# marcomistretta/incremental_multimodal_medical_learning_II

Measured on AMD Instinct MI355X. Metric: contrastive train-step images/sec at global batch 1024; 1/2/4/8-GPU scaling, higher is better.
Workload: dtype bf16x3

## Files before the change

### include/cxrk.h

```cpp
#ifndef CXRK_H
#define CXRK_H

#include <stddef.h>
#include <hip/hip_runtime_api.h>

#ifdef __cplusplus
extern "C" {
#endif

size_t cxrk_gemm_splitk_ws_bytes(int M, int N, int splitk);
int cxrk_gemm_wgrad_splitk(int M, int N, int K, int planes);
int cxrk_gemm_wide_tile(int M, int N, long K, int splitk, int kind);
int cxrk_gemm_f32(int transA, int transB, int M, int N, int K, const float* A, long lda, const float* B, long ldb,
                  float* C, long ldc, const float* bias, const float* R, long ldr, const float* aux, long ldaux,
                  int auxmode, float* C2, long ldc2, int act, float alpha, int accumulate, int splitk, float* ws,
                  size_t ws_bytes, hipStream_t stream);

int cxrk_gemm_pl(int transA, int transB, int M, int N, int K, const void* A, long lda, long aplane, const void* B, long ldb,
                 long bplane, float* C, void* Cp, long ldc, long cplane, const float* bias, const float* R, const void* Rp,
                 long ldr, long rplane, const float* aux, long ldaux, int auxmode, const unsigned char* maskin, long ldmaskin,
                 unsigned char* maskout, long ldmaskout, float* C2, long ldc2, int act, float alpha, int accumulate, int splitk,
                 float* colsum, int colsum_accumulate, float* ws, size_t ws_bytes, hipStream_t stream);
size_t cxrk_gemm_pl_colsum_ws_bytes(int M, int N);
int cxrk_split_planes(const float* x, long n, void* out, long plane, hipStream_t stream);
int cxrk_merge_planes(const void* x, long plane, long n, float* out, hipStream_t stream);

size_t cxrk_colsum_ws_bytes(long rows, int cols);
int cxrk_colsum(const float* X, long ldx, long rows, int cols, float* out, float alpha, int accumulate, float* ws,
                size_t ws_bytes, hipStream_t stream);
int cxrk_colsum_pl(const void* X, long ldx, long plane, long rows, int cols, float* out, float alpha, int accumulate, float* ws,
                   size_t ws_bytes, hipStream_t stream);
int cxrk_colvar(const void* X, long ldx, long plane, long rows, int cols, const float* mean, float* out, float alpha, float* ws,
                size_t ws_bytes, hipStream_t stream);

int cxrk_bn_fold(const float* w, const float* gamma, const float* beta, const float* rmean, const float* rvar,
                 float eps, int Ko, int taps, int C, int Cpad, float* w_scaled, float* scale, float* shift,
                 float* rstd, hipStream_t stream);
int cxrk_bn_fold_pl(const float* w, const float* gamma, const float* beta, const float* rmean, const float* rvar,
                    float eps, int Ko, int taps, int C, int Cpad, void* w_scaled, long wplane, float* scale, float* shift,
                    float* rstd, hipStream_t stream);
int cxrk_conv_bn_act_fwd(const float* x, const float* w_scaled, const float* shift, const float* residual, float* y,
                         int N, int H, int W, int C, int Ko, int R, int S, int stride, int pad, int relu,
                         hipStream_t stream);
int cxrk_conv_bn_act_fwd_pl(const void* x, long xplane, const void* w_scaled, long wplane, int in_planes, const float* shift,
                            const void* residual, long rplane, void* y, long yplane, unsigned char* maskout, int N, int H,
                            int W, int C, int Ko, int R, int S, int stride, int pad, int relu, hipStream_t stream);
size_t cxrk_conv_bwd_data_colsum_ws_bytes(int N, int H, int W, int C, int stride);
int cxrk_conv_bn_act_bwd_data(const float* dy, const float* w_scaled, const float* residual, const float* relu_src,
                              float* dx, int N, int H, int W, int C, int Ko, int R, int S, int stride, int pad,
                              float* sums, float* ws, size_t ws_bytes, hipStream_t stream);
int cxrk_conv_bn_act_bwd_data_pl(const void* dy, long dyplane, const void* w_scaled, long wplane, const void* residual,
                                 long rplane, const unsigned char* maskin, void* dx, long dxplane, int N, int H, int W, int C,
                                 int Ko, int R, int S, int stride, int pad, float* sums, float* ws, size_t ws_bytes,
                                 hipStream_t stream);
int cxrk_conv_bn_act_bwd_data_pl_s2res(const void* dy, long dyplane, const void* w_scaled, long wplane, const void* residual_s2,
                                 long rplane, const unsigned char* maskin, void* dx, long dxplane, int N, int H, int W, int C,
                                 int Ko, int R, int S, int stride, int pad, float* sums, float* ws, size_t ws_bytes,
                                 hipStream_t stream);
size_t cxrk_conv_wgrad_ws_bytes(int N, int H, int W, int Cpad, int Ko, int R, int S, int stride, int pad);
int cxrk_conv_bn_act_bwd_params(const float* x, const float* dy, const float* w, const float* scale, const float* rstd,
                                const float* rmean, const float* sumdy, float* dw, float* dgamma, float* dbeta,
                                int accumulate, int N, int H, int W, int C, int Cpad, int Ko, int R, int S, int stride,
                                int pad, float* ws, size_t ws_bytes, hipStream_t stream);
int cxrk_conv_bn_act_bwd_params_pl(const void* x, long xplane, const void* dy, long dyplane, const float* w, const float* scale,
                                   const float* rstd, const float* rmean, const float* sumdy, float* dw, float* dgamma,
                                   float* dbeta, int accumulate, int N, int H, int W, int C, int Ko, int R, int S, int stride,
                                   int pad, float* ws, size_t ws_bytes, hipStream_t stream);

int cxrk_nchw_to_nhwc(const float* x, float* y, int N, int C, int H, int W, int Cpad, hipStream_t stream);
int cxrk_nhwc_to_nchw(const float* x, float* y, int N, int C, int H, int W, hipStream_t stream);

int cxrk_maxpool_fwd(const float* x, float* y, unsigned char* idx, int N, int H, int W, int C, hipStream_t stream);
int cxrk_maxpool_bwd(const float* dy, const unsigned char* idx, const float* x, float* dx, int N, int H, int W, int C,
                     int relu_mask, hipStream_t stream);
int cxrk_maxpool_fwd_pl(const void* x, long xplane, void* y, long yplane, unsigned char* idx, int N, int H, int W, int C,
                        hipStream_t stream);
int cxrk_maxpool_bwd_pl(const void* dy, long dyplane, const unsigned char* idx, const void* pooled, float* dx, int N, int H,
                        int W, int C, hipStream_t stream);

int cxrk_spatial_mean_fwd(const float* x, float* y, int N, int P, int C, hipStream_t stream);
int cxrk_spatial_mean_bwd(const float* dy, float* dx, int N, int P, int C, hipStream_t stream);
int cxrk_spatial_mean_bwd_pl(const float* dy, const float* add, void* dx, long dxplane, int N, int P, int C, hipStream_t stream);

int cxrk_colstats(const void* x, long plane, long rows, int C, float* mean, float* var, float var_scale, float* ws, size_t ws_bytes,
                  hipStream_t stream);
int cxrk_bn_train_fwd_coeffs(const float* mean, const float* var, const float* gamma, const float* beta, float eps, long n, float momentum,
                             float* scale, float* shift, float* rstd, float* rmean, float* rvar, int C, hipStream_t stream);
int cxrk_bn_apply(const void* z, long zplane, const float* scale, const float* shift, const void* res, long rplane, void* y, long yplane,
                  unsigned char* mask, long rows, int C, int relu, hipStream_t stream);
size_t cxrk_coldot_ws_bytes(long rows, int C);
int cxrk_coldot(const void* a, long aplane, const void* b, long bplane, const float* bshift, long rows, int C, float* out, float* ws,
                size_t ws_bytes, hipStream_t stream);
int cxrk_bn_train_bwd_coeffs(const float* gamma, const float* mean, const float* rstd, const float* sumdy, const float* dot, long n, float* A,
                             float* B, float* Cc, float* dgamma, float* dbeta, int accumulate, int C, hipStream_t stream);
int cxrk_bn_train_dz(const void* dy, long dyplane, const void* z, long zplane, const float* A, const float* B, const float* Cc, void* dz,
                     long dzplane, long rows, int C, hipStream_t stream);

int cxrk_embed_ln_fwd(const long* ids, const float* word, const float* pos, const float* type, const float* gamma,
                      const float* beta, float eps, long T, int L, int H, void* y, long yplane, float* xhat, float* rstd,
                      hipStream_t stream);
int cxrk_residual_ln_fwd(const float* x, const float* res, const float* gamma, const float* beta, float eps, long rows,
                         int H, void* y, long yplane, float* xhat, float* rstd, hipStream_t stream);
size_t cxrk_residual_ln_bwd_ws_bytes(long rows, int H);
int cxrk_residual_ln_bwd(const float* dy, const float* xhat, const float* rstd, const float* gamma, long rows, int H,
                         const float* dx_add, void* dx, long dxplane, float* dgamma, float* dbeta, int accumulate, float* dxsum,
                         int dxsum_accumulate, float* ws, size_t ws_bytes, hipStream_t stream);
int cxrk_planes_add_rows(const void* src, long plane, long rows, int cols, float* dst, long ld, hipStream_t stream);
int cxrk_attn_fwd(const float* qkv, const long* mask, int B, int L, int nH, int dH, void* ctx, long ctxplane, float* probs,
                  hipStream_t stream);
size_t cxrk_attn_bwd_ws_bytes(int B, int L, int nH, int dH);
int cxrk_attn_bwd(const float* qkv, const float* probs, const float* dctx, int B, int L, int nH, int dH, void* dqkv,
                  long dqkvplane, float* ws, size_t ws_bytes, hipStream_t stream);
int cxrk_dropout_mask(unsigned long long seed, unsigned counter, int layer, int site, long row_offset, float p, int N, int L, int nH,
                      int C, unsigned char* keep, hipStream_t stream);
int cxrk_embed_ln_fwd_drop(const long* ids, const float* word, const float* pos, const float* type, const float* gamma,
                           const float* beta, float eps, long T, int L, int H, void* y, long yplane, float* xhat, float* rstd,
                           unsigned long long seed, unsigned counter, int layer, int site, long row_offset, float p,
                           hipStream_t stream);
int cxrk_residual_ln_fwd_drop(const float* x, const void* res, long resplane, long res_ld, const float* gamma, const float* beta,
                              float eps, long rows, int H, int rows_per_seq, void* y, long yplane, float* xhat, float* rstd,
                              unsigned long long seed, unsigned counter, int layer, int site, long row_offset, float p,
                              hipStream_t stream);
int cxrk_residual_ln_bwd_drop(const float* dy, const float* xhat, const float* rstd, const float* gamma, long rows, int H,
                              int rows_per_seq, int mode, const float* dx_add, void* dx, void* dxm, long dxplane, float* dgamma,
                              float* dbeta, int accumulate, float* dxsum, int dxsum_accumulate, float* ws, size_t ws_bytes,
                              unsigned long long seed, unsigned counter, int layer, int site, long row_offset, float p,
                              hipStream_t stream);
int cxrk_attn_fwd_drop(const float* qkv, const long* mask, int B, int L, int nH, int dH, void* ctx, long ctxplane, float* probs,
                       unsigned long long seed, unsigned counter, int layer, int site, long row_offset, float p, hipStream_t stream);
int cxrk_attn_bwd_drop(const float* qkv, const float* probs, const float* dctx, int B, int L, int nH, int dH, void* dqkv,
                       long dqkvplane, float* ws, size_t ws_bytes, unsigned long long seed, unsigned counter, int layer, int site,
                       long row_offset, float p, hipStream_t stream);
size_t cxrk_embed_bwd_ws_bytes(long T, int H);
int cxrk_embed_bwd(const long* ids, const float* dx, long T, int H, float* dword, float* ws, size_t ws_bytes, hipStream_t stream);
int cxrk_gelu_bwd(const float* dy, const float* pre, long n, float* dx, hipStream_t stream);

int cxrk_l2norm_fwd(const float* x, long rows, int D, float eps, float* xhat, long ldxhat, float* norm, hipStream_t stream);
int cxrk_l2norm_bwd(const float* dxhat, const float* xhat, long ldxhat, const float* norm, long rows, int D, float* dx,
                    hipStream_t stream);
int cxrk_infonce_row_lse(const float* S, long ld, int rows, int cols, int diag_off, float* lse, float* diag,
                         float* loss_out, float loss_scale, int loss_accumulate, hipStream_t stream);
int cxrk_infonce_grad_inplace(float* S, long ld, int rows, int cols, int diag_off, const float* lse_row,
                              const float* lse_col, hipStream_t stream);
int cxrk_multipos_row_stats(const float* S, long ld, int rows, int cols, const long long* keys_row,
                            const long long* keys_col, float* lse, float* posmean, float* npos, float* loss_out,
                            float loss_scale, int loss_accumulate, hipStream_t stream);
int cxrk_multipos_grad_inplace(float* S, long ld, int rows, int cols, const long long* keys_row,
                               const long long* keys_col, const float* n_row, const float* lse_row, const float* lse_col,
                               hipStream_t stream);
int cxrk_infonce_row_lse_scaled(const float* C, long ld, int rows, int cols, int diag_off, const float* log_scale, float* lse,
                                float* diag, float* loss_out, float loss_scale, int loss_accumulate, hipStream_t stream);
int cxrk_infonce_grad_scaled_inplace(float* C, long ld, int rows, int cols, int diag_off, const float* lse_row,
                                     const float* lse_col, const float* log_scale, float* partials, hipStream_t stream);
int cxrk_multipos_row_stats_scaled(const float* C, long ld, int rows, int cols, const long long* keys_row,
                                   const long long* keys_col, const float* log_scale, float* lse, float* posmean, float* npos,
                                   float* loss_out, float loss_scale, int loss_accumulate, hipStream_t stream);
int cxrk_multipos_grad_scaled_inplace(float* C, long ld, int rows, int cols, const long long* keys_row,
                                      const long long* keys_col, const float* n_row, const float* lse_row, const float* lse_col,
                                      const float* log_scale, float* partials, hipStream_t stream);
int cxrk_logit_scale_grad(const float* partials1, long n1, const float* partials2, long n2, const float* upstream, float scale,
                          float* dtheta, int accumulate, hipStream_t stream);
int cxrk_clamp_inplace(float* x, long n, float lo, float hi, hipStream_t stream);
int cxrk_pairwise_cosine_fwd(const float* x, const float* y, long B, int P, int D, float* cosv, float* xnorm,
                             float* ynorm, hipStream_t stream);
size_t cxrk_pairwise_cosine_bwd_ws_bytes(long B, int P, int D);
int cxrk_pairwise_cosine_bwd(const float* x, const float* y, const float* cosv, const float* dcos, const float* xnorm,
                             const float* ynorm, long B, int P, int D, float* dx, float* dy, int accumulate_dy,
                             float* ws, size_t ws_bytes, hipStream_t stream);
int cxrk_pairwise_cosine_max_fwd(const float* x, const float* y, long B, int G, int Pg, int D, float* cosv, float* xnorm,
                                 float* ynorm, float* maxv, float* meanv, int* argmax, hipStream_t stream);
int cxrk_pairwise_cosine_max_bwd(const float* x, const float* y, const float* cosv, const float* dmax, const int* argmax,
                                 const float* xnorm, const float* ynorm, long B, int G, int Pg, int D, float* dx, float* dy,
                                 int accumulate_dy, float* ws, size_t ws_bytes, hipStream_t stream);
int cxrk_patch_similarity(const float* patches, const float* text, long R, int D, float* sim, hipStream_t stream);
size_t cxrk_bce_posneg_ws_bytes(void);
int cxrk_bce_posneg_fwd_bwd(const float* cosv, const float* labels, long B, int C, int ldlab, int diff, float* logits,
                            float* dcos, float* loss, float* ws, size_t ws_bytes, hipStream_t stream);
int cxrk_eval_score(const float* cosv, long B, int C, int pred_diff, float* score, float* pred, hipStream_t stream);
int cxrk_group_mean_fwd(const float* in, int G, int n, int D, float* out, hipStream_t stream);
int cxrk_group_mean_bwd(const float* dout, int G, int n, int D, float* din, hipStream_t stream);
int cxrk_scale_mask(const float* x, const float* mask_src, const float* alpha_dev, float alpha, long n, float* out,
                    hipStream_t stream);

int cxrk_adam_fused(float* p, const float* g, float* m, float* v, long n, float lr, float beta1, float beta2,
                    float eps, float weight_decay, int step, float grad_scale, hipStream_t stream);
int cxrk_sgd(float* p, const float* g, long n, float lr, float weight_decay, float grad_scale, hipStream_t stream);
size_t cxrk_weight_reset_ws_bytes(void);
int cxrk_weight_reset(float* pnew, const float* pold, long n, float threshold, unsigned long long* counters, float* ws,
                      size_t ws_bytes, hipStream_t stream);

int cxrk_set_precision(int mode);
int cxrk_get_precision(void);
int cxrk_set_wide_mode(int mode);

const char* cxrk_version(void);

#ifdef __cplusplus
}
#endif
#endif
```

### incremental_multimodal_medical_learning_ii_amd/_lib.py

```python
from __future__ import annotations

import ctypes
import os
from ctypes import c_char_p, c_float, c_int, c_long, c_size_t, c_uint32, c_uint64, c_void_p
from typing import Dict, List, Tuple

_HERE = os.path.dirname(os.path.abspath(__file__))
LIB_PATH = os.path.join(_HERE, "libcxrk.so")

P, I, L, F, Z = c_void_p, c_int, c_long, c_float, c_size_t
DROP = [c_uint64, c_uint32, I, I, L, F]

SIGNATURES: Dict[str, Tuple[object, List[object]]] = {
    "cxrk_gemm_splitk_ws_bytes": (Z, [I, I, I]),
    "cxrk_gemm_f32": (I, [I, I, I, I, I, P, L, P, L, P, L, P, P, L, P, L, I, P, L, I, F, I, I, P, Z, P]),
    "cxrk_gemm_pl": (I, [I, I, I, I, I, P, L, L, P, L, L, P, P, L, L, P, P, P, L, L, P, L, I, P, L, P, L, P, L, I, F, I, I, P, I, P, Z, P]),
    "cxrk_gemm_pl_colsum_ws_bytes": (Z, [I, I]),
    "cxrk_split_planes": (I, [P, L, P, L, P]),
    "cxrk_merge_planes": (I, [P, L, L, P, P]),
    "cxrk_colsum_pl": (I, [P, L, L, L, I, P, F, I, P, Z, P]),
    "cxrk_colsum_ws_bytes": (Z, [L, I]),
    "cxrk_colsum": (I, [P, L, L, I, P, F, I, P, Z, P]),
    "cxrk_colvar": (I, [P, L, L, L, I, P, P, F, P, Z, P]),
    "cxrk_bn_fold": (I, [P, P, P, P, P, F, I, I, I, I, P, P, P, P, P]),
    "cxrk_conv_bn_act_fwd": (I, [P, P, P, P, P, I, I, I, I, I, I, I, I, I, I, P]),
    "cxrk_bn_fold_pl": (I, [P, P, P, P, P, F, I, I, I, I, P, L, P, P, P, P]),
    "cxrk_conv_bn_act_fwd_pl": (I, [P, L, P, L, I, P, P, L, P, L, P, I, I, I, I, I, I, I, I, I, I, P]),
    "cxrk_conv_bwd_data_colsum_ws_bytes": (Z, [I, I, I, I, I]),
    "cxrk_conv_bn_act_bwd_data": (I, [P, P, P, P, P, I, I, I, I, I, I, I, I, I, P, P, Z, P]),
    "cxrk_conv_bn_act_bwd_data_pl": (I, [P, L, P, L, P, L, P, P, L, I, I, I, I, I, I, I, I, I, P, P, Z, P]),
    "cxrk_conv_bn_act_bwd_data_pl_s2res": (I, [P, L, P, L, P, L, P, P, L, I, I, I, I, I, I, I, I, I, P, P, Z, P]),
    "cxrk_conv_wgrad_ws_bytes": (Z, [I, I, I, I, I, I, I, I, I]),
    "cxrk_conv_bn_act_bwd_params": (I, [P, P, P, P, P, P, P, P, P, P, I, I, I, I, I, I, I, I, I, I, I, P, Z, P]),
    "cxrk_conv_bn_act_bwd_params_pl": (I, [P, L, P, L, P, P, P, P, P, P, P, P, I, I, I, I, I, I, I, I, I, I, P, Z, P]),
    "cxrk_colstats": (I, [P, L, L, I, P, P, F, P, Z, P]),
    "cxrk_bn_train_fwd_coeffs": (I, [P, P, P, P, F, L, F, P, P, P, P, P, I, P]),
    "cxrk_bn_apply": (I, [P, L, P, P, P, L, P, L, P, L, I, I, P]),
    "cxrk_coldot_ws_bytes": (Z, [L, I]),
    "cxrk_coldot": (I, [P, L, P, L, P, L, I, P, P, Z, P]),
    "cxrk_bn_train_bwd_coeffs": (I, [P, P, P, P, P, L, P, P, P, P, P, I, I, P]),
    "cxrk_bn_train_dz": (I, [P, L, P, L, P, P, P, P, L, L, I, P]),
    "cxrk_nchw_to_nhwc": (I, [P, P, I, I, I, I, I, P]),
    "cxrk_nhwc_to_nchw": (I, [P, P, I, I, I, I, P]),
    "cxrk_maxpool_fwd": (I, [P, P, P, I, I, I, I, P]),
    "cxrk_maxpool_bwd": (I, [P, P, P, P, I, I, I, I, I, P]),
    "cxrk_maxpool_fwd_pl": (I, [P, L, P, L, P, I, I, I, I, P]),
    "cxrk_maxpool_bwd_pl": (I, [P, L, P, P, P, I, I, I, I, P]),
    "cxrk_spatial_mean_fwd": (I, [P, P, I, I, I, P]),
    "cxrk_spatial_mean_bwd": (I, [P, P, I, I, I, P]),
    "cxrk_spatial_mean_bwd_pl": (I, [P, P, P, L, I, I, I, P]),
    "cxrk_embed_ln_fwd": (I, [P, P, P, P, P, P, F, L, I, I, P, L, P, P, P]),
    "cxrk_residual_ln_fwd": (I, [P, P, P, P, F, L, I, P, L, P, P, P]),
    "cxrk_residual_ln_bwd_ws_bytes": (Z, [L, I]),
    "cxrk_residual_ln_bwd": (I, [P, P, P, P, L, I, P, P, L, P, P, I, P, I, P, Z, P]),
    "cxrk_planes_add_rows": (I, [P, L, L, I, P, L, P]),
    "cxrk_attn_fwd": (I, [P, P, I, I, I, I, P, L, P, P]),
    "cxrk_attn_bwd_ws_bytes": (Z, [I, I, I, I]),
    "cxrk_attn_bwd": (I, [P, P, P, I, I, I, I, P, L, P, Z, P]),
    "cxrk_dropout_mask": (I, DROP + [I, I, I, I, P, P]),
    "cxrk_embed_ln_fwd_drop": (I, [P, P, P, P, P, P, F, L, I, I, P, L, P, P] + DROP + [P]),
    "cxrk_residual_ln_fwd_drop": (I, [P, P, L, L, P, P, F, L, I, I, P, L, P, P] + DROP + [P]),
    "cxrk_residual_ln_bwd_drop": (I, [P, P, P, P, L, I, I, I, P, P, P, L, P, P, I, P, I, P, Z] + DROP + [P]),
    "cxrk_attn_fwd_drop": (I, [P, P, I, I, I, I, P, L, P] + DROP + [P]),
    "cxrk_attn_bwd_drop": (I, [P, P, P, I, I, I, I, P, L, P, Z] + DROP + [P]),
    "cxrk_embed_bwd_ws_bytes": (Z, [L, I]),
    "cxrk_embed_bwd": (I, [P, P, L, I, P, P, Z, P]),
    "cxrk_gelu_bwd": (I, [P, P, L, P, P]),
    "cxrk_l2norm_fwd": (I, [P, L, I, F, P, L, P, P]),
    "cxrk_l2norm_bwd": (I, [P, P, L, P, L, I, P, P]),
    "cxrk_infonce_row_lse": (I, [P, L, I, I, I, P, P, P, F, I, P]),
    "cxrk_infonce_grad_inplace": (I, [P, L, I, I, I, P, P, P]),
    "cxrk_multipos_row_stats": (I, [P, L, I, I, P, P, P, P, P, P, F, I, P]),
    "cxrk_multipos_grad_inplace": (I, [P, L, I, I, P, P, P, P, P, P]),
    "cxrk_infonce_row_lse_scaled": (I, [P, L, I, I, I, P, P, P, P, F, I, P]),
    "cxrk_infonce_grad_scaled_inplace": (I, [P, L, I, I, I, P, P, P, P, P]),
    "cxrk_multipos_row_stats_scaled": (I, [P, L, I, I, P, P, P, P, P, P, P, F, I, P]),
    "cxrk_multipos_grad_scaled_inplace": (I, [P, L, I, I, P, P, P, P, P, P, P, P]),
    "cxrk_logit_scale_grad": (I, [P, L, P, L, P, F, P, I, P]),
    "cxrk_clamp_inplace": (I, [P, L, F, F, P]),
    "cxrk_pairwise_cosine_fwd": (I, [P, P, L, I, I, P, P, P, P]),
    "cxrk_pairwise_cosine_bwd_ws_bytes": (Z, [L, I, I]),
    "cxrk_pairwise_cosine_bwd": (I, [P, P, P, P, P, P, L, I, I, P, P, I, P, Z, P]),
    "cxrk_pairwise_cosine_max_fwd": (I, [P, P, L, I, I, I, P, P, P, P, P, P, P]),
    "cxrk_pairwise_cosine_max_bwd": (I, [P, P, P, P, P, P, P, L, I, I, I, P, P, I, P, Z, P]),
    "cxrk_patch_similarity": (I, [P, P, L, I, P, P]),
    "cxrk_bce_posneg_ws_bytes": (Z, []),
    "cxrk_bce_posneg_fwd_bwd": (I, [P, P, L, I, I, I, P, P, P, P, Z, P]),
    "cxrk_eval_score": (I, [P, L, I, I, P, P, P]),
    "cxrk_group_mean_fwd": (I, [P, I, I, I, P, P]),
    "cxrk_group_mean_bwd": (I, [P, I, I, I, P, P]),
    "cxrk_scale_mask": (I, [P, P, P, F, L, P, P]),
    "cxrk_adam_fused": (I, [P, P, P, P, L, F, F, F, F, F, I, F, P]),
    "cxrk_sgd": (I, [P, P, L, F, F, F, P]),
    "cxrk_weight_reset_ws_bytes": (Z, []),
    "cxrk_weight_reset": (I, [P, P, L, F, P, P, Z, P]),
    "cxrk_gemm_wgrad_splitk": (I, [I, I, I, I]),
    "cxrk_gemm_wide_tile": (I, [I, I, L, I, I]),
    "cxrk_set_precision": (I, [I]),
    "cxrk_get_precision": (I, []),
    "cxrk_set_wide_mode": (I, [I]),
    "cxrk_version": (c_char_p, []),
}

_ERRORS = {-1: "bad argument / shape / alignment", -2: "workspace too small", -3: "kernel launch failed",
           -4: "unsupported shape"}


class CxrkError(RuntimeError):
    pass


_lib = None


def load() -> ctypes.CDLL:
    global _lib
    if _lib is not None:
        return _lib
    if not os.path.exists(LIB_PATH):
        raise CxrkError(f"{LIB_PATH} not found: build it with `python -c 'import __graft_entry__ as g; g.build()'` "
                        f"(hipcc --offload-arch=gfx950).  There is no CPU or PyTorch fallback for the hot path.")
    lib = ctypes.CDLL(LIB_PATH)
    for name, (res, args) in SIGNATURES.items():
        fn = getattr(lib, name)
        fn.restype = res
        fn.argtypes = args
    _lib = lib
    mode = os.environ.get("CXRK_PRECISION", "fp32")
    if mode not in PRECISIONS:
        raise CxrkError(f"CXRK_PRECISION={mode!r}: expected one of {sorted(PRECISIONS)}")
    lib.cxrk_set_precision(PRECISIONS[mode])
    return lib


PRECISIONS = {"fp32": 0, "split_bf16": 1}


def set_precision(mode: str) -> None:
    if mode not in PRECISIONS:
        raise ValueError(f"precision {mode!r}: expected one of {sorted(PRECISIONS)}")
    check(load().cxrk_set_precision(PRECISIONS[mode]), "cxrk_set_precision")


def get_precision() -> str:
    v = load().cxrk_get_precision()
    return {b: a for a, b in PRECISIONS.items()}[v]


def check(rc: int, what: str) -> None:
    if rc != 0:
        msg = _ERRORS.get(rc, "unknown error")
        if rc in (-1, -4):
            raise ValueError(f"{what}: {msg} (cxrk code {rc})")
        raise CxrkError(f"{what}: {msg} (cxrk code {rc})")
```

### incremental_multimodal_medical_learning_ii_amd/csrc/conv_fwd.hip

```cpp
#include "conv_common.h"
#include "conv_halo.h"

using namespace cxrk;

template <class FMT>
static int conv_fwd_impl(const typename FMT::T* x, long xplane, const typename FMT::T* w, long wplane, EpiParams ep, int N, int H,
                         int W, int C, int Ko, int R, int S, int stride, int pad, hipStream_t stream) {
  CXRK_CHECK_ARG(x && w && N > 0 && C % FMT::EPL == 0 && aligned16(x) && aligned16(w));
  CXRK_CHECK_ARG(stride == 1 || stride == 2);
  const ConvGeom g = make_geom(N, H, W, C, Ko, R, S, stride, pad);
  CXRK_CHECK_ARG(g.Ho > 0 && g.Wo > 0);
  const long Ml = (long)N * g.Ho * g.Wo;
  CXRK_CHECK_ARG(Ml < (1L << 31));
  const int M = (int)Ml, K = R * S * C;
  if (!tile_span_ok((long)g.Ho * g.Wo, (long)H * W * C)) return CXRK_ERR_UNSUPPORTED;
  int rc;
  const bool tapwise = (C % BK == 0) && R * S <= 32 && R <= 8;
  if (tapwise && use_wide256(M, Ko, K, 1, FMT::PLANES, WIDE_MINK_FPROP)) {
    if constexpr (FMT::PLANES) {
      DmaConvIm2colKC<256, 8>::P pa{x, g, M, K, xplane}; DmaDenseKC<256, 8>::P pb{w, (long)K, Ko, K, wplane};
      rc = launch_gemm_pw<Pw256, DmaConvIm2colKC<256, 8>, DmaDenseKC<256, 8>>(pa, pb, ep, M, Ko, K, 1, stream);
    } else return CXRK_ERR_UNSUPPORTED;
  } else if (tapwise) {
    if (FMT::PLANES && halo_applies(H, W, C, Ko, R, S, stride, pad)) {
      if constexpr (FMT::PLANES) {
        DmaDenseKC<64, 4>::P pb{w, (long)K, Ko, K, wplane};
        rc = launch_conv3x3_halo<DmaDenseKC<64, 4>, false>(x, xplane, pb, ep, M, Ko, H, W, stream);
      } else rc = CXRK_ERR_UNSUPPORTED;
    } else if (Ko <= 64) {
      if constexpr (FMT::PLANES) {
        DmaConvIm2colKC<256, 4>::P pa{x, g, M, K, xplane}; DmaDenseKC<64, 4>::P pb{w, (long)K, Ko, K, wplane};
        rc = launch_gemm_pw<Pw256x64, DmaConvIm2colKC<256, 4>, DmaDenseKC<64, 4>>(pa, pb, ep, M, Ko, K, 1, stream);
      } else {
        typename ConvIm2colKC<256, FMT>::P pa{x, g, M, K, xplane}; typename DenseKC<64, FMT>::P pb{w, (long)K, Ko, K, wplane};
        rc = launch_gemm<ConvIm2colKC<256, FMT>, DenseKC<64, FMT>, 4, 1>(pa, pb, ep, M, Ko, K, 1, stream);
      }
    } else if constexpr (FMT::PLANES) {
      DmaConvIm2colKC<128, 4>::P pa{x, g, M, K, xplane}; DmaDenseKC<128, 4>::P pb{w, (long)K, Ko, K, wplane};
      rc = launch_gemm_pw<Pw128, DmaConvIm2colKC<128, 4>, DmaDenseKC<128, 4>>(pa, pb, ep, M, Ko, K, 1, stream);
    } else {
      typename ConvIm2colKC<128, FMT>::P pa{x, g, M, K, xplane}; typename DenseKC<128, FMT>::P pb{w, (long)K, Ko, K, wplane};
      rc = launch_gemm<ConvIm2colKC<128, FMT>, DenseKC<128, FMT>, 2, 2>(pa, pb, ep, M, Ko, K, 1, stream);
    }
  } else {
    if constexpr (FMT::PLANES) return CXRK_ERR_UNSUPPORTED;
    else {
      if (Ko <= 64) {
        ConvIm2colKC<256, F32, false>::P pa{x, g, M, K, 0}; DenseKC<64>::P pb{w, (long)K, Ko, K, 0};
        rc = launch_gemm<ConvIm2colKC<256, F32, false>, DenseKC<64>, 4, 1>(pa, pb, ep, M, Ko, K, 1, stream);
      } else {
        ConvIm2colKC<128, F32, false>::P pa{x, g, M, K, 0}; DenseKC<128>::P pb{w, (long)K, Ko, K, 0};
        rc = launch_gemm<ConvIm2colKC<128, F32, false>, DenseKC<128>, 2, 2>(pa, pb, ep, M, Ko, K, 1, stream);
      }
    }
  }
  return rc < 0 ? rc : CXRK_OK;
}

extern "C" int cxrk_conv_bn_act_fwd(const float* x, const float* w_scaled, const float* shift, const float* residual,
                                    float* y, int N, int H, int W, int C, int Ko, int R, int S, int stride, int pad,
                                    int relu, hipStream_t stream) {
  CXRK_CHECK_ARG(y);
  EpiParams ep{};
  ep.C = y; ep.ldc = Ko; ep.bias = shift; ep.R = residual; ep.ldr = Ko; ep.act = relu ? 1 : 0; ep.alpha = 1.f;
  return conv_fwd_impl<F32>(x, 0, w_scaled, 0, ep, N, H, W, C, Ko, R, S, stride, pad, stream);
}

extern "C" int cxrk_conv_bn_act_fwd_pl(const void* x, long xplane, const void* w_scaled, long wplane, int in_planes,
                                       const float* shift, const void* residual, long rplane, void* y, long yplane,
                                       unsigned char* maskout, int N, int H, int W, int C, int Ko, int R, int S, int stride,
                                       int pad, int relu, hipStream_t stream) {
  CXRK_CHECK_ARG(y && (Ko % 8) == 0 && !(maskout && !relu));
  EpiParams ep{};
  ep.Cp = static_cast<unsigned short*>(y); ep.cplane = yplane; ep.ldc = Ko; ep.bias = shift;
  ep.Rp = static_cast<const unsigned short*>(residual); ep.rplane = rplane; ep.ldr = Ko; ep.act = relu ? 1 : 0; ep.alpha = 1.f;
  ep.maskout = maskout; ep.ldmaskout = Ko / 8;
  if (in_planes)
    return conv_fwd_impl<PL>(static_cast<const unsigned short*>(x), xplane, static_cast<const unsigned short*>(w_scaled), wplane, ep, N, H,
                             W, C, Ko, R, S, stride, pad, stream);
  return conv_fwd_impl<F32>(static_cast<const float*>(x), 0, static_cast<const float*>(w_scaled), 0, ep, N, H, W, C, Ko, R, S, stride,
                            pad, stream);
}
```

### incremental_multimodal_medical_learning_ii_amd/csrc/conv_misc.hip

```cpp
#include "conv_common.h"

using namespace cxrk;

namespace {
__global__ void bn_fold_kernel(const float* __restrict__ w, const float* __restrict__ gamma, const float* __restrict__ beta,
                               const float* __restrict__ rmean, const float* __restrict__ rvar, float eps, int Ko, int taps,
                               int C, int Cpad, float* __restrict__ ws, unsigned short* __restrict__ wp, long wplane,
                               float* __restrict__ scale, float* __restrict__ shift, float* __restrict__ rstd) {
  const int ko = blockIdx.x;
  const float rs = 1.0f / sqrtf(rvar[ko] + eps);
  const float sc = gamma[ko] * rs;
  if (threadIdx.x == 0) { scale[ko] = sc; shift[ko] = beta[ko] - rmean[ko] * sc; rstd[ko] = rs; }
  const int n = taps * Cpad;
  if (wp) {
    for (int i8 = threadIdx.x; i8 < n / 8; i8 += blockDim.x) {
      const int i = i8 * 8, tap = i / Cpad, c = i - tap * Cpad;
      float v[8];
#pragma unroll
      for (int q = 0; q < 8; ++q) v[q] = c + q < C ? w[((long)ko * taps + tap) * C + c + q] * sc : 0.f;
      planes_store8(wp, wplane, (long)ko * n + i, v);
    }
    return;
  }
  for (int i = threadIdx.x; i < n; i += blockDim.x) {
    const int tap = i / Cpad, c = i - tap * Cpad;
    ws[(long)ko * n + i] = c < C ? w[((long)ko * taps + tap) * C + c] * sc : 0.f;
  }
}

__global__ void nchw_to_nhwc_kernel(const float* __restrict__ x, float* __restrict__ y, int C, int H, int W, int Cpad) {
  const long nh = blockIdx.x;
  const long n = nh / H; const int hh = (int)(nh - n * H);
  for (int i = threadIdx.x; i < W * Cpad; i += blockDim.x) {
    const int wv = i / Cpad, c = i - wv * Cpad;
    y[(nh * W + wv) * Cpad + c] = c < C ? x[((n * C + c) * H + hh) * W + wv] : 0.f;
  }
}
__global__ void nhwc_to_nchw_kernel(const float* __restrict__ x, float* __restrict__ y, int C, int H, int W) {
  const long nh = blockIdx.x;
  const long n = nh / H; const int hh = (int)(nh - n * H);
  for (int i = threadIdx.x; i < W * C; i += blockDim.x) {
    const int c = i / W, wv = i - c * W;
    y[((n * C + c) * H + hh) * W + wv] = x[(nh * W + wv) * C + c];
  }
}

__global__ void maxpool_fwd_kernel(const float* __restrict__ x, float* __restrict__ y, unsigned char* __restrict__ idx,
                                   int N, int H, int W, int C, int Ho, int Wo) {
  const long t = (long)blockIdx.x * blockDim.x + threadIdx.x;
  const int C4 = C / 4;
  const long total = (long)N * Ho * Wo * C4;
  if (t >= total) return;
  const int c4 = (int)(t % C4); long p = t / C4;
  const int wo = (int)(p % Wo); p /= Wo; const int ho = (int)(p % Ho); const long n = p / Ho;
  float4 best = make_float4(-INFINITY, -INFINITY, -INFINITY, -INFINITY);
  uchar4 bi = make_uchar4(0, 0, 0, 0);
  bool first = true;
  for (int r = 0; r < 3; ++r) {
    const int hi = ho * 2 - 1 + r;
    if ((unsigned)hi >= (unsigned)H) continue;
    for (int s = 0; s < 3; ++s) {
      const int wi = wo * 2 - 1 + s;
      if ((unsigned)wi >= (unsigned)W) continue;
      const float4 v = *reinterpret_cast<const float4*>(x + ((n * H + hi) * W + wi) * C + c4 * 4);
      const unsigned char tap = (unsigned char)(r * 3 + s);
      if (first || v.x > best.x) { best.x = v.x; bi.x = tap; }
      if (first || v.y > best.y) { best.y = v.y; bi.y = tap; }
      if (first || v.z > best.z) { best.z = v.z; bi.z = tap; }
      if (first || v.w > best.w) { best.w = v.w; bi.w = tap; }
      first = false;
    }
  }
  *reinterpret_cast<float4*>(y + t * 4) = best;
  *reinterpret_cast<uchar4*>(idx + t * 4) = bi;
}

__global__ void maxpool_bwd_kernel(const float* __restrict__ dy, const unsigned char* __restrict__ idx,
                                   const float* __restrict__ x, float* __restrict__ dx, int N, int H, int W, int C, int Ho,
                                   int Wo, int relu_mask) {
  const long t = (long)blockIdx.x * blockDim.x + threadIdx.x;
  const int C4 = C / 4;
  const long total = (long)N * H * W * C4;
  if (t >= total) return;
  const int c4 = (int)(t % C4); long p = t / C4;
  const int wi = (int)(p % W); p /= W; const int hi = (int)(p % H); const long n = p / H;
  float4 g = make_float4(0.f, 0.f, 0.f, 0.f);
  for (int r = 0; r < 3; ++r) {
    const int hn = hi + 1 - r;
    if (hn < 0 || (hn & 1)) continue;
    const int ho = hn >> 1;
    if (ho >= Ho) continue;
    for (int s = 0; s < 3; ++s) {
      const int wn = wi + 1 - s;
      if (wn < 0 || (wn & 1)) continue;
      const int wo = wn >> 1;
      if (wo >= Wo) continue;
      const long o = (((n * Ho + ho) * Wo + wo) * C4 + c4) * 4;
      const uchar4 bi = *reinterpret_cast<const uchar4*>(idx + o);
      const float4 d = *reinterpret_cast<const float4*>(dy + o);
      const unsigned char tap = (unsigned char)(r * 3 + s);
      if (bi.x == tap) g.x += d.x;
      if (bi.y == tap) g.y += d.y;
      if (bi.z == tap) g.z += d.z;
      if (bi.w == tap) g.w += d.w;
    }
  }
  if (relu_mask) {
    const float4 xv = *reinterpret_cast<const float4*>(x + t * 4);
    g.x = xv.x > 0.f ? g.x : 0.f; g.y = xv.y > 0.f ? g.y : 0.f; g.z = xv.z > 0.f ? g.z : 0.f; g.w = xv.w > 0.f ? g.w : 0.f;
  }
  *reinterpret_cast<float4*>(dx + t * 4) = g;
}

__global__ void spatial_mean_fwd_kernel(const float* __restrict__ x, float* __restrict__ y, int P, int C) {
  const int n = blockIdx.x;
  for (int c = threadIdx.x; c < C; c += blockDim.x) {
    float s = 0.f;
    for (int p = 0; p < P; ++p) s += x[((long)n * P + p) * C + c];
    y[(long)n * C + c] = s / (float)P;
  }
}
__global__ void spatial_mean_bwd_kernel(const float* __restrict__ dy, float* __restrict__ dx, int P, int C) {
  const int n = blockIdx.x;
  const float inv = 1.0f / (float)P;
  for (int i = threadIdx.x; i < P * C; i += blockDim.x) dx[(long)n * P * C + i] = dy[(long)n * C + (i % C)] * inv;
}

__global__ void maxpool_fwd_pl_kernel(const unsigned short* __restrict__ x, long xplane, unsigned short* __restrict__ y, long yplane,
                                      unsigned char* __restrict__ idx, int N, int H, int W, int C, int Ho, int Wo) {
  const long t = (long)blockIdx.x * blockDim.x + threadIdx.x;
  const int C8 = C / 8;
  const long total = (long)N * Ho * Wo * C8;
  if (t >= total) return;
  const int c8 = (int)(t % C8); long p = t / C8;
  const int wo = (int)(p % Wo); p /= Wo; const int ho = (int)(p % Ho); const long n = p / Ho;
  float best[8]; unsigned char bi[8];
  bool first = true;
  for (int r = 0; r < 3; ++r) {
    const int hi = ho * 2 - 1 + r;
    if ((unsigned)hi >= (unsigned)H) continue;
    for (int s = 0; s < 3; ++s) {
      const int wi = wo * 2 - 1 + s;
      if ((unsigned)wi >= (unsigned)W) continue;
      float v[8]; planes_load8(x, xplane, ((n * H + hi) * W + wi) * C + c8 * 8, v);
      const unsigned char tap = (unsigned char)(r * 3 + s);
#pragma unroll
      for (int q = 0; q < 8; ++q) if (first || v[q] > best[q]) { best[q] = v[q]; bi[q] = tap; }
      first = false;
    }
  }
  planes_store8(y, yplane, t * 8, best);
  *reinterpret_cast<uint2*>(idx + t * 8) = make_uint2(bi[0] | (bi[1] << 8) | (bi[2] << 16) | (bi[3] << 24),
                                                      bi[4] | (bi[5] << 8) | (bi[6] << 16) | (bi[7] << 24));
}
struct PoolWin { float d[8]; unsigned tap[8]; };
__device__ __forceinline__ void pool_win_load(PoolWin& w, bool valid, const unsigned short* __restrict__ dy, long dyplane,
                                              const unsigned char* __restrict__ idx, const unsigned short* __restrict__ pooled, long o) {
  if (!valid) {
#pragma unroll
    for (int q = 0; q < 8; ++q) { w.d[q] = 0.f; w.tap[q] = 0xffu; }
    return;
  }
  const uint2 bw = *reinterpret_cast<const uint2*>(idx + o);
  const uint4 ph = *reinterpret_cast<const uint4*>(pooled + o);
  planes_load8(dy, dyplane, o, w.d);
  const unsigned pw[4] = {ph.x, ph.y, ph.z, ph.w};
#pragma unroll
  for (int q = 0; q < 8; ++q) {
    w.tap[q] = ((q < 4 ? bw.x : bw.y) >> (8 * (q & 3))) & 0xffu;
    const float pv = __builtin_bit_cast(float, (q & 1) ? (pw[q >> 1] & 0xffff0000u) : (pw[q >> 1] << 16));
    if (!(pv > 0.f)) w.tap[q] = 0xffu;
  }
}
__device__ __forceinline__ void pool_acc(float (&g)[8], const PoolWin& w, unsigned tap) {
#pragma unroll
  for (int q = 0; q < 8; ++q) if (w.tap[q] == tap) g[q] += w.d[q];
}
__device__ __forceinline__ void pool_store(float* __restrict__ dx, long e, const float (&g)[8]) {
  *reinterpret_cast<float4*>(dx + e) = make_float4(g[0], g[1], g[2], g[3]);
  *reinterpret_cast<float4*>(dx + e + 4) = make_float4(g[4], g[5], g[6], g[7]);
}
__global__ __launch_bounds__(256) void maxpool_bwd_pl_kernel(const unsigned short* __restrict__ dy, long dyplane, const unsigned char* __restrict__ idx,
                                                             const unsigned short* __restrict__ pooled, float* __restrict__ dx, int N, int H,
                                                             int W, int C, int Ho, int Wo) {
  const long t = (long)blockIdx.x * blockDim.x + threadIdx.x;
  const int C8 = C / 8, H2 = (H + 1) / 2, W2 = (W + 1) / 2;
  const long total = (long)N * H2 * W2 * C8;
  if (t >= total) return;
  const int c8 = (int)(t % C8); long p = t / C8;
  const int b = (int)(p % W2); p /= W2; const int a = (int)(p % H2); const long n = p / H2;
  PoolWin w00, w01, w10, w11;
  const bool va = a < Ho, va1 = a + 1 < Ho, vb = b < Wo, vb1 = b + 1 < Wo;
  const long o00 = (((n * Ho + a) * Wo + b) * C8 + c8) * 8;
  pool_win_load(w00, va && vb, dy, dyplane, idx, pooled, o00);
  pool_win_load(w01, va && vb1, dy, dyplane, idx, pooled, o00 + (long)C);
  pool_win_load(w10, va1 && vb, dy, dyplane, idx, pooled, o00 + (long)Wo * C);
  pool_win_load(w11, va1 && vb1, dy, dyplane, idx, pooled, o00 + (long)(Wo + 1) * C);
  const int hi = 2 * a, wi = 2 * b;
  const long e = (((n * H + hi) * W + wi) * C8 + c8) * 8;
  {
    float g[8] = {0.f, 0.f, 0.f, 0.f, 0.f, 0.f, 0.f, 0.f};
    pool_acc(g, w00, 4u);
    pool_store(dx, e, g);
  }
  if (wi + 1 < W) {
    float g[8] = {0.f, 0.f, 0.f, 0.f, 0.f, 0.f, 0.f, 0.f};
    pool_acc(g, w01, 3u); pool_acc(g, w00, 5u);
    pool_store(dx, e + C, g);
  }
  if (hi + 1 < H) {
    float g[8] = {0.f, 0.f, 0.f, 0.f, 0.f, 0.f, 0.f, 0.f};
    pool_acc(g, w10, 1u); pool_acc(g, w00, 7u);
    pool_store(dx, e + (long)W * C, g);
  }
  if (hi + 1 < H && wi + 1 < W) {
    float g[8] = {0.f, 0.f, 0.f, 0.f, 0.f, 0.f, 0.f, 0.f};
    pool_acc(g, w11, 0u); pool_acc(g, w10, 2u); pool_acc(g, w01, 6u); pool_acc(g, w00, 8u);
    pool_store(dx, e + (long)(W + 1) * C, g);
  }
}
__global__ void spatial_mean_bwd_pl_kernel(const float* __restrict__ dy, const float* __restrict__ add, unsigned short* __restrict__ dx,
                                           long dxplane, int P, int C) {
  const int n = blockIdx.x;
  const float inv = 1.0f / (float)P;
  const int C8 = C / 8;
  for (int i = threadIdx.x; i < P * C8; i += blockDim.x) {
    const int c = (i % C8) * 8;
    float v[8];
#pragma unroll
    for (int q = 0; q < 8; ++q) v[q] = dy[(long)n * C + c + q] * inv;
    const long o = ((long)n * P + i / C8) * C + c;
    if (add) {
#pragma unroll
      for (int q = 0; q < 8; ++q) v[q] += add[o + q];
    }
    planes_store8(dx, dxplane, o, v);
  }
}

}

extern "C" int cxrk_bn_fold(const float* w, const float* gamma, const float* beta, const float* rmean, const float* rvar,
                            float eps, int Ko, int taps, int C, int Cpad, float* w_scaled, float* scale, float* shift,
                            float* rstd, hipStream_t stream) {
  CXRK_CHECK_ARG(w && gamma && beta && rmean && rvar && w_scaled && scale && shift && rstd && Ko > 0 && taps > 0 && C > 0 && Cpad >= C);
  hipLaunchKernelGGL(bn_fold_kernel, dim3(Ko), dim3(256), 0, stream, w, gamma, beta, rmean, rvar, eps, Ko, taps, C, Cpad,
                     w_scaled, (unsigned short*)nullptr, 0L, scale, shift, rstd);
  CXRK_LAUNCH_CHECK();
  return CXRK_OK;
}
extern "C" int cxrk_bn_fold_pl(const float* w, const float* gamma, const float* beta, const float* rmean, const float* rvar,
                               float eps, int Ko, int taps, int C, int Cpad, void* w_scaled, long wplane, float* scale,
                               float* shift, float* rstd, hipStream_t stream) {
  CXRK_CHECK_ARG(w && gamma && beta && rmean && rvar && w_scaled && scale && shift && rstd && Ko > 0 && taps > 0 && C > 0 && Cpad >= C);
  CXRK_CHECK_ARG((Cpad % 8) == 0 && (wplane % 8) == 0 && aligned16(w_scaled));
  hipLaunchKernelGGL(bn_fold_kernel, dim3(Ko), dim3(256), 0, stream, w, gamma, beta, rmean, rvar, eps, Ko, taps, C, Cpad,
                     (float*)nullptr, static_cast<unsigned short*>(w_scaled), wplane, scale, shift, rstd);
  CXRK_LAUNCH_CHECK();
  return CXRK_OK;
}

extern "C" int cxrk_nchw_to_nhwc(const float* x, float* y, int N, int C, int H, int W, int Cpad, hipStream_t stream) {
  CXRK_CHECK_ARG(x && y && N > 0 && C > 0 && Cpad >= C);
  hipLaunchKernelGGL(nchw_to_nhwc_kernel, dim3((unsigned)((long)N * H)), dim3(256), 0, stream, x, y, C, H, W, Cpad);
  CXRK_LAUNCH_CHECK();
  return CXRK_OK;
}
extern "C" int cxrk_nhwc_to_nchw(const float* x, float* y, int N, int C, int H, int W, hipStream_t stream) {
  CXRK_CHECK_ARG(x && y && N > 0 && C > 0);
  hipLaunchKernelGGL(nhwc_to_nchw_kernel, dim3((unsigned)((long)N * H)), dim3(256), 0, stream, x, y, C, H, W);
  CXRK_LAUNCH_CHECK();
  return CXRK_OK;
}

extern "C" int cxrk_maxpool_fwd(const float* x, float* y, unsigned char* idx, int N, int H, int W, int C, hipStream_t stream) {
  CXRK_CHECK_ARG(x && y && idx && C % 4 == 0 && aligned16(x) && aligned16(y));
  const int Ho = (H + 2 - 3) / 2 + 1, Wo = (W + 2 - 3) / 2 + 1;
  const long total = (long)N * Ho * Wo * (C / 4);
  hipLaunchKernelGGL(maxpool_fwd_kernel, dim3((unsigned)((total + 255) / 256)), dim3(256), 0, stream, x, y, idx, N, H, W, C, Ho, Wo);
  CXRK_LAUNCH_CHECK();
  return CXRK_OK;
}
extern "C" int cxrk_maxpool_bwd(const float* dy, const unsigned char* idx, const float* x, float* dx, int N, int H, int W,
                                int C, int relu_mask, hipStream_t stream) {
  CXRK_CHECK_ARG(dy && idx && dx && C % 4 == 0 && (!relu_mask || x));
  const int Ho = (H + 2 - 3) / 2 + 1, Wo = (W + 2 - 3) / 2 + 1;
  const long total = (long)N * H * W * (C / 4);
  hipLaunchKernelGGL(maxpool_bwd_kernel, dim3((unsigned)((total + 255) / 256)), dim3(256), 0, stream, dy, idx, x, dx, N, H, W, C,
                     Ho, Wo, relu_mask);
  CXRK_LAUNCH_CHECK();
  return CXRK_OK;
}
extern "C" int cxrk_maxpool_fwd_pl(const void* x, long xplane, void* y, long yplane, unsigned char* idx, int N, int H, int W, int C,
                                   hipStream_t stream) {
  CXRK_CHECK_ARG(x && y && idx && C % 8 == 0 && aligned16(x) && aligned16(y) && (xplane % 8) == 0 && (yplane % 8) == 0 && (((uintptr_t)idx) & 7) == 0);
  const int Ho = (H + 2 - 3) / 2 + 1, Wo = (W + 2 - 3) / 2 + 1;
  const long total = (long)N * Ho * Wo * (C / 8);
  hipLaunchKernelGGL(maxpool_fwd_pl_kernel, dim3((unsigned)((total + 255) / 256)), dim3(256), 0, stream, static_cast<const unsigned short*>(x),
                     xplane, static_cast<unsigned short*>(y), yplane, idx, N, H, W, C, Ho, Wo);
  CXRK_LAUNCH_CHECK();
  return CXRK_OK;
}
extern "C" int cxrk_maxpool_bwd_pl(const void* dy, long dyplane, const unsigned char* idx, const void* pooled, float* dx, int N, int H,
                                   int W, int C, hipStream_t stream) {
  CXRK_CHECK_ARG(dy && idx && pooled && dx && C % 8 == 0 && aligned16(dy) && aligned16(pooled) && aligned16(dx) && (dyplane % 8) == 0);
  const int Ho = (H + 2 - 3) / 2 + 1, Wo = (W + 2 - 3) / 2 + 1;
  const long total = (long)N * ((H + 1) / 2) * ((W + 1) / 2) * (C / 8);
  hipLaunchKernelGGL(maxpool_bwd_pl_kernel, dim3((unsigned)((total + 255) / 256)), dim3(256), 0, stream, static_cast<const unsigned short*>(dy),
                     dyplane, idx, static_cast<const unsigned short*>(pooled), dx, N, H, W, C, Ho, Wo);
  CXRK_LAUNCH_CHECK();
  return CXRK_OK;
}

extern "C" int cxrk_spatial_mean_fwd(const float* x, float* y, int N, int P, int C, hipStream_t stream) {
  CXRK_CHECK_ARG(x && y && N > 0 && P > 0 && C > 0);
  hipLaunchKernelGGL(spatial_mean_fwd_kernel, dim3(N), dim3(128), 0, stream, x, y, P, C);
  CXRK_LAUNCH_CHECK();
  return CXRK_OK;
}
extern "C" int cxrk_spatial_mean_bwd(const float* dy, float* dx, int N, int P, int C, hipStream_t stream) {
  CXRK_CHECK_ARG(dy && dx && N > 0 && P > 0 && C > 0);
  hipLaunchKernelGGL(spatial_mean_bwd_kernel, dim3(N), dim3(256), 0, stream, dy, dx, P, C);
  CXRK_LAUNCH_CHECK();
  return CXRK_OK;
}
extern "C" int cxrk_spatial_mean_bwd_pl(const float* dy, const float* add, void* dx, long dxplane, int N, int P, int C, hipStream_t stream) {
  CXRK_CHECK_ARG(dy && dx && N > 0 && P > 0 && C > 0 && (C % 8) == 0 && aligned16(dx) && (dxplane % 8) == 0);
  hipLaunchKernelGGL(spatial_mean_bwd_pl_kernel, dim3(N), dim3(256), 0, stream, dy, add, static_cast<unsigned short*>(dx), dxplane, P, C);
  CXRK_LAUNCH_CHECK();
  return CXRK_OK;
}
```

### incremental_multimodal_medical_learning_ii_amd/csrc/conv_wgrad.hip

```cpp
#include "conv_common.h"

using namespace cxrk;

namespace {
__global__ __launch_bounds__(256) void wgrad_reduce_bn_kernel(const float* __restrict__ slabs, int nslab, long slab_stride,
                                                              int taps, int C, int Cpad, const float* __restrict__ w,
                                                              const float* __restrict__ scale, float* __restrict__ dw,
                                                              float* __restrict__ dotpart, int accumulate, int sg_log2) {
  __shared__ float sh[16];
  __shared__ float4 red[256];
  const int ko = blockIdx.x;
  const int n = taps * Cpad;
  const float sc = scale ? scale[ko] : 1.f;
  const int SG = 1 << sg_log2, QPB = 256 >> sg_log2;
  const int ql = threadIdx.x & (QPB - 1), grp = threadIdx.x >> (8 - sg_log2);
  const int i4 = (blockIdx.y * QPB + ql) * 4;
  float4 s = make_float4(0.f, 0.f, 0.f, 0.f);
  if (i4 < n) {
    const float* src = slabs + (long)ko * n + i4;
    int z = grp;
    for (; z + 3 * SG < nslab; z += 4 * SG) {
      const float4 t0 = *reinterpret_cast<const float4*>(src + (long)z * slab_stride);
      const float4 t1 = *reinterpret_cast<const float4*>(src + (long)(z + SG) * slab_stride);
      const float4 t2 = *reinterpret_cast<const float4*>(src + (long)(z + 2 * SG) * slab_stride);
      const float4 t3 = *reinterpret_cast<const float4*>(src + (long)(z + 3 * SG) * slab_stride);
      s.x += (t0.x + t1.x) + (t2.x + t3.x); s.y += (t0.y + t1.y) + (t2.y + t3.y);
      s.z += (t0.z + t1.z) + (t2.z + t3.z); s.w += (t0.w + t1.w) + (t2.w + t3.w);
    }
    for (; z < nslab; z += SG) {
      const float4 t = *reinterpret_cast<const float4*>(src + (long)z * slab_stride);
      s.x += t.x; s.y += t.y; s.z += t.z; s.w += t.w;
    }
  }
  if (SG > 1) {
    red[threadIdx.x] = s;
    __syncthreads();
    if (grp == 0) {
      for (int g2 = 1; g2 < SG; ++g2) { const float4 t = red[g2 * QPB + ql]; s.x += t.x; s.y += t.y; s.z += t.z; s.w += t.w; }
    }
  }
  float dot = 0.f;
  if (i4 < n && grp == 0) {
    const int tap = i4 / Cpad, c = i4 - tap * Cpad;
    const float sv[4] = {s.x, s.y, s.z, s.w};
#pragma unroll
    for (int q = 0; q < 4; ++q) {
      if (c + q < C) {
        const long o = ((long)ko * taps + tap) * C + c + q;
        if (dotpart) dot += w[o] * sv[q];
        dw[o] = accumulate ? dw[o] + sc * sv[q] : sc * sv[q];
      }
    }
  }
  if (dotpart) {
    dot = block_sum(dot, sh);
    if (threadIdx.x == 0) dotpart[(long)ko * gridDim.y + blockIdx.y] = dot;
  }
}
__global__ void bn_param_grad_kernel(const float* __restrict__ dotpart, int nparts, const float* __restrict__ rstd,
                                     const float* __restrict__ rmean, const float* __restrict__ sumdy, int Ko,
                                     float* __restrict__ dgamma, float* __restrict__ dbeta, int accumulate) {
  const int ko = blockIdx.x * blockDim.x + threadIdx.x;
  if (ko >= Ko) return;
  float dot = 0.f;
  for (int p = 0; p < nparts; ++p) dot += dotpart[(long)ko * nparts + p];
  const float g = rstd[ko] * (dot - rmean[ko] * sumdy[ko]);
  dgamma[ko] = accumulate ? dgamma[ko] + g : g;
  dbeta[ko] = accumulate ? dbeta[ko] + sumdy[ko] : sumdy[ko];
}

}

static int wgrad_splitk(int Ko, int Ncols, long Kred, bool planes) { return wgrad_splitk_policy(Ko, Ncols, (int)Kred, planes); }
static int wgrad_dot_parts(int Nc) { return ceil_div(Nc, 64); }

extern "C" size_t cxrk_conv_wgrad_ws_bytes(int N, int H, int W, int C, int Ko, int R, int S, int stride, int pad) {
  const ConvGeom g = make_geom(N, H, W, C, Ko, R, S, stride, pad);
  int sk = wgrad_splitk(Ko, R * S * C, (long)N * g.Ho * g.Wo, false);
  const int sk2 = wgrad_splitk(Ko, R * S * C, (long)N * g.Ho * g.Wo, true);
  if (sk2 > sk) sk = sk2;
  return ((size_t)sk * (size_t)Ko * (size_t)(R * S * C) + (size_t)Ko * wgrad_dot_parts(R * S * C)) * sizeof(float);
}

template <class FMT>
static int conv_bwd_params_impl(const typename FMT::T* x, long xplane, const typename FMT::T* dy, long dyplane, const float* w,
                                const float* scale, const float* rstd, const float* rmean, const float* sumdy, float* dw,
                                float* dgamma, float* dbeta, int accumulate, int N, int H, int W, int C, int Cpad, int Ko, int R,
                                int S, int stride, int pad, float* ws, size_t ws_bytes, hipStream_t stream) {
  CXRK_CHECK_ARG(x && dy && dw && N > 0 && Cpad % FMT::EPL == 0 && Ko % FMT::EPL == 0 && aligned16(x) && aligned16(dy));
  CXRK_CHECK_ARG(!(dgamma && !(w && rstd && rmean && sumdy && dbeta)));
  const ConvGeom g = make_geom(N, H, W, Cpad, Ko, R, S, stride, pad);
  const long Kl = (long)N * g.Ho * g.Wo;
  CXRK_CHECK_ARG(Kl < (1L << 31));
  const int Kred = (int)Kl, Nc = R * S * Cpad;
  if ((long)H * W * Cpad * 4 * 3 >= (1L << 31)) return CXRK_ERR_UNSUPPORTED;
  int sk = wgrad_splitk(Ko, Nc, Kl, FMT::PLANES);
  const size_t slab_floats = (size_t)sk * Ko * Nc;
  CXRK_CHECK_WS(ws, ws_bytes, (slab_floats + (size_t)Ko * wgrad_dot_parts(Nc)) * sizeof(float));
  EpiParams ep{};
  ep.C = ws; ep.ldc = Nc; ep.alpha = 1.f; ep.slab_stride = (long)Ko * Nc;
  int rc;
  const bool exact = false;
  if (use_wide256(Ko, Nc, Kred, sk, FMT::PLANES)) {
    if constexpr (FMT::PLANES) {
      DmaDenseMC<256, 8>::P pa{dy, (long)Ko, Ko, Kred, dyplane}; DmaConvIm2colMC<256, 8>::P pb{x, g, Nc, Kred, xplane};
      rc = launch_gemm_pw<Pw256, DmaDenseMC<256, 8>, DmaConvIm2colMC<256, 8>>(pa, pb, ep, Ko, Nc, Kred, sk, stream);
    } else return CXRK_ERR_UNSUPPORTED;
  } else if (Ko <= 64) {
    if constexpr (FMT::PLANES) {
      DmaDenseMC<64, 4>::P pa{dy, (long)Ko, Ko, Kred, dyplane}; DmaConvIm2colMC<256, 4>::P pb{x, g, Nc, Kred, xplane};
      rc = launch_gemm_pw<Pw64x256, DmaDenseMC<64, 4>, DmaConvIm2colMC<256, 4>>(pa, pb, ep, Ko, Nc, Kred, sk, stream);
    } else {
      typename DenseMC<64, FMT>::P pa{dy, (long)Ko, Ko, Kred, dyplane}; typename ConvIm2colMC<256, FMT>::P pb{x, g, Nc, Kred, xplane};
      rc = launch_gemm<DenseMC<64, FMT>, ConvIm2colMC<256, FMT>, 1, 4>(pa, pb, ep, Ko, Nc, Kred, sk, stream, exact);
    }
  } else if constexpr (FMT::PLANES) {
    DmaDenseMC<128, 4>::P pa{dy, (long)Ko, Ko, Kred, dyplane}; DmaConvIm2colMC<128, 4>::P pb{x, g, Nc, Kred, xplane};
    rc = launch_gemm_pw<Pw128, DmaDenseMC<128, 4>, DmaConvIm2colMC<128, 4>>(pa, pb, ep, Ko, Nc, Kred, sk, stream);
  } else {
    typename DenseMC<128, FMT>::P pa{dy, (long)Ko, Ko, Kred, dyplane}; typename ConvIm2colMC<128, FMT>::P pb{x, g, Nc, Kred, xplane};
    rc = launch_gemm<DenseMC<128, FMT>, ConvIm2colMC<128, FMT>, 2, 2>(pa, pb, ep, Ko, Nc, Kred, sk, stream, exact);
  }
  if (rc < 0) return rc;
  const int sg_log2 = rc >= 64 ? 4 : (rc >= 8 ? 2 : 0);
  const int ny = ceil_div(Nc, 4 * (256 >> sg_log2));
  float* dotpart = dgamma ? ws + slab_floats : nullptr;
  hipLaunchKernelGGL(wgrad_reduce_bn_kernel, dim3(Ko, ny), dim3(256), 0, stream, ws, rc, (long)Ko * Nc, R * S, C, Cpad, w, scale, dw,
                     dotpart, accumulate, sg_log2);
  CXRK_LAUNCH_CHECK();
  if (dgamma) {
    hipLaunchKernelGGL(bn_param_grad_kernel, dim3(ceil_div(Ko, 256)), dim3(256), 0, stream, dotpart, ny, rstd, rmean, sumdy, Ko, dgamma,
                       dbeta, accumulate);
    CXRK_LAUNCH_CHECK();
  }
  return CXRK_OK;
}

extern "C" int cxrk_conv_bn_act_bwd_params(const float* x, const float* dy, const float* w, const float* scale,
                                           const float* rstd, const float* rmean, const float* sumdy, float* dw,
                                           float* dgamma, float* dbeta, int accumulate, int N, int H, int W, int C,
                                           int Cpad, int Ko, int R, int S, int stride, int pad, float* ws, size_t ws_bytes,
                                           hipStream_t stream) {
  return conv_bwd_params_impl<F32>(x, 0, dy, 0, w, scale, rstd, rmean, sumdy, dw, dgamma, dbeta, accumulate, N, H, W, C, Cpad, Ko, R, S,
                                   stride, pad, ws, ws_bytes, stream);
}
extern "C" int cxrk_conv_bn_act_bwd_params_pl(const void* x, long xplane, const void* dy, long dyplane, const float* w,
                                              const float* scale, const float* rstd, const float* rmean, const float* sumdy,
                                              float* dw, float* dgamma, float* dbeta, int accumulate, int N, int H, int W, int C,
                                              int Ko, int R, int S, int stride, int pad, float* ws, size_t ws_bytes,
                                              hipStream_t stream) {
  return conv_bwd_params_impl<PL>(static_cast<const unsigned short*>(x), xplane, static_cast<const unsigned short*>(dy), dyplane, w, scale,
                                  rstd, rmean, sumdy, dw, dgamma, dbeta, accumulate, N, H, W, C, C, Ko, R, S, stride, pad, ws, ws_bytes,
                                  stream);
}
```

### incremental_multimodal_medical_learning_ii_amd/csrc/gemm_core.h

```cpp
#pragma once
#include "cxrk_common.h"
#include <cstdlib>

namespace cxrk {

constexpr int BK = 32;
constexpr int NTHREADS = 256;
constexpr int LPAD = 4;

struct EpiParams {
  float* C; long ldc;
  const float* bias;
  const float* R; long ldr;
  const float* aux; long ldaux;
  int auxmode;
  float* C2; long ldc2;
  int act;
  float alpha;
  long slab_stride;
  int rm_on, rm_Hs, rm_Ws, rm_H, rm_W, rm_ph, rm_pw;
  int vec;
  int nt;
  float* colsum_part;
  unsigned short* Cp; long cplane;
// ... 193 lines not shown
  constexpr int BM = WM * 64, BN = WN * 64;
  constexpr int LDA = LA::LD, LDB = LB::LD;
  constexpr int ASZ = BK * LDA, BSZ = BK * LDB;
  __shared__ __attribute__((aligned(16))) float smem[ASZ + BSZ];
  float* const As0 = smem;
  float* const Bs0 = smem + ASZ;

  int mt, nt, z;
  tile_coords(nMt, nNt, nZ, mt, nt, z);
  const int m0 = mt * BM, n0 = nt * BN;
  const int kbeg = z * kchunk;
  const int kend = min(K, kbeg + kchunk);

  const int tid = threadIdx.x;
  const int lane = tid & 63, wave = tid >> 6;
  const int wm = wave / WN, wn = wave % WN;
  const int r = lane & 31, h = lane >> 5;

  LA la; LB lb;
  la.init(pa, m0, tid);
  lb.init(pb, n0, tid);

  f32x16 acc[2][2];
#pragma unroll
  for (int i = 0; i < 2; ++i)
#pragma unroll
    for (int j = 0; j < 2; ++j)
#pragma unroll
      for (int e = 0; e < 16; ++e) acc[i][j][e] = 0.f;

  static_assert(!LA::FMT_PLANES && !LB::FMT_PLANES, "the exact-fp32 mainloop reads fp32 operands");
  float4 ra[LA::NV], rb[LB::NV];
  if (kbeg < kend) {
    la.load(kbeg, ra); lb.load(kbeg, rb);
    la.store(As0, ra); lb.store(Bs0, rb);
  }
  __syncthreads();
  if (kbeg + BK < kend) { la.load(kbeg + BK, ra); lb.load(kbeg + BK, rb); }

  for (int k0 = kbeg; k0 < kend; k0 += BK) {
    const float* Ap = As0 + wm * 64 + r + h * LDA;
    const float* Bp = Bs0 + wn * 64 + r + h * LDB;
    const bool has1 = k0 + BK < kend, has2 = k0 + 2 * BK < kend;
    float a0 = Ap[0], a1 = Ap[32], b0 = Bp[0], b1 = Bp[32];
#pragma unroll
    for (int kk = 0; kk < BK / 2; ++kk) {
      float a0n = 0.f, a1n = 0.f, b0n = 0.f, b1n = 0.f;
      if (kk + 1 < BK / 2) {
        a0n = Ap[(2 * kk + 2) * LDA]; a1n = Ap[(2 * kk + 2) * LDA + 32];
        b0n = Bp[(2 * kk + 2) * LDB]; b1n = Bp[(2 * kk + 2) * LDB + 32];
      }
      acc[0][0] = __builtin_amdgcn_mfma_f32_32x32x2f32(a0, b0, acc[0][0], 0, 0, 0);
      acc[0][1] = __builtin_amdgcn_mfma_f32_32x32x2f32(a0, b1, acc[0][1], 0, 0, 0);
      acc[1][0] = __builtin_amdgcn_mfma_f32_32x32x2f32(a1, b0, acc[1][0], 0, 0, 0);
      acc[1][1] = __builtin_amdgcn_mfma_f32_32x32x2f32(a1, b1, acc[1][1], 0, 0, 0);
      a0 = a0n; a1 = a1n; b0 = b0n; b1 = b1n;
    }
    __syncthreads();
    if (has1) { la.store(As0, ra); lb.store(Bs0, rb); }
    __syncthreads();
    if (has2) { la.load(k0 + 2 * BK, ra); lb.load(k0 + 2 * BK, rb); }
  }

  static_assert(BK * (LDA + LDB) >= 4 * 32 * 64, "operand LDS too small to stage the epilogue");
  __syncthreads();
  gemm_epilogue<WM, WN>(acc, ep, smem, M, N, m0, n0, mt, z, wave, lane);
}

template <class LA, class LB, int WM, int WN>
__global__ __launch_bounds__(NTHREADS, (WM == 2 && WN == 2) ? 3 : 2) void gemm_x3_kernel(typename LA::P pa, typename LB::P pb, EpiParams ep,
                                                              int M, int N, int K, int nMt, int nNt, int nZ, int kchunk) {
  constexpr int BM = WM * 64, BN = WN * 64;
  constexpr int PLANE_A = LA::PLANE, PLANE_B = LB::PLANE;
  static_assert(2 * (PLANE_A + PLANE_B) * 2 >= 4 * 32 * 64 * 4, "operand LDS too small to stage the epilogue");
  __shared__ __attribute__((aligned(16))) unsigned short smem16[2 * (PLANE_A + PLANE_B)];
  unsigned short* const Ahi = smem16;
  unsigned short* const Alo = Ahi + PLANE_A;
  unsigned short* const Bhi = Alo + PLANE_A;
  unsigned short* const Blo = Bhi + PLANE_B;

  int mt, nt, z;
  tile_coords(nMt, nNt, nZ, mt, nt, z);
  const int m0 = mt * BM, n0 = nt * BN;
  const int kbeg = z * kchunk;
  const int kend = min(K, kbeg + kchunk);

  const int tid = threadIdx.x;
  const int lane = tid & 63, wave = tid >> 6;
  const int wm = wave / WN, wn = wave % WN;

  LA la; LB lb;
  la.init(pa, m0, tid);
  lb.init(pb, n0, tid);

  f32x16 acc[2][2];
#pragma unroll
  for (int i = 0; i < 2; ++i)
#pragma unroll
    for (int j = 0; j < 2; ++j)
#pragma unroll
      for (int e = 0; e < 16; ++e) acc[i][j][e] = 0.f;

  typename LA::V ra[LA::NV]; typename LB::V rb[LB::NV];
  if (kbeg < kend) {
    la.load(kbeg, ra); lb.load(kbeg, rb);
    la.store2(Ahi, Alo, ra); lb.store2(Bhi, Blo, rb);
  }
  __syncthreads();
  if (kbeg + BK < kend) { la.load(kbeg + BK, ra); lb.load(kbeg + BK, rb); }

  for (int k0 = kbeg; k0 < kend; k0 += BK) {
#pragma unroll
    for (int kc = 0; kc < BK / 16; ++kc) {
      bf16x8 ah[2], al[2], bh[2], bl[2];
#pragma unroll
      for (int i = 0; i < 2; ++i) {
        if constexpr (LA::KC) {
          ah[i] = frag_kc(Ahi, wm * 64 + i * 32, kc, lane); al[i] = frag_kc(Alo, wm * 64 + i * 32, kc, lane);
        } else {
          ah[i] = frag_mc<LA::LDT>(Ahi, wm * 64 + i * 32, kc, lane); al[i] = frag_mc<LA::LDT>(Alo, wm * 64 + i * 32, kc, lane);
        }
        if constexpr (LB::KC) {
          bh[i] = frag_kc(Bhi, wn * 64 + i * 32, kc, lane); bl[i] = frag_kc(Blo, wn * 64 + i * 32, kc, lane);
        } else {
          bh[i] = frag_mc<LB::LDT>(Bhi, wn * 64 + i * 32, kc, lane); bl[i] = frag_mc<LB::LDT>(Blo, wn * 64 + i * 32, kc, lane);
        }
      }
#pragma unroll
      for (int i = 0; i < 2; ++i)
#pragma unroll
        for (int j = 0; j < 2; ++j) {
          acc[i][j] = __builtin_amdgcn_mfma_f32_32x32x16_bf16(al[i], bh[j], acc[i][j], 0, 0, 0);
          acc[i][j] = __builtin_amdgcn_mfma_f32_32x32x16_bf16(ah[i], bl[j], acc[i][j], 0, 0, 0);
          acc[i][j] = __builtin_amdgcn_mfma_f32_32x32x16_bf16(ah[i], bh[j], acc[i][j], 0, 0, 0);
        }
    }
    __syncthreads();
    if (k0 + BK < kend) { la.store2(Ahi, Alo, ra); lb.store2(Bhi, Blo, rb); }
    __syncthreads();
    if (k0 + 2 * BK < kend) { la.load(k0 + 2 * BK, ra); lb.load(k0 + 2 * BK, rb); }
  }
  __syncthreads();
  gemm_epilogue<WM, WN>(acc, ep, reinterpret_cast<float*>(smem16), M, N, m0, n0, mt, z, wave, lane);
}

inline int& gemm_precision_mode() { static int mode = 0; return mode; }

static inline int stream_output(int M, int N, int splitk) {
  static const double thr = [] { const char* e = getenv("CXRK_NT_MB"); return (e ? atof(e) : 64.0) * 1048576.0; }();
  return (double)M * N * 4.0 * (splitk > 1 ? splitk : 1) >= thr;
}

int wgrad_splitk_policy(int M, int N, int K, bool planes);

inline int& wide_mode_ref() { static int m = [] { const char* e = getenv("CXRK_WIDE"); return e ? atoi(e) : 1; }(); return m; }
inline int wide_mode() { return wide_mode_ref(); }
static inline long env_long(const char* name, long dflt) { const char* e = getenv(name); return e ? atol(e) : dflt; }
#define WIDE_MINK_PLAIN (wide_mink(0))
#define WIDE_MINK_FPROP (wide_mink(1))
#define WIDE_MINK_DGRAD (wide_mink(2))
inline long wide_mink(int kind) {
  static const long v[3] = {env_long("CXRK_MINK_PLAIN", 512), env_long("CXRK_MINK_FPROP", 512), env_long("CXRK_MINK_DGRAD", 64)};
  return v[kind];
}
static inline bool use_wide256(int M, int N, long K, int splitk, bool planes, long min_k = WIDE_MINK_PLAIN) {
  if (!planes) return false;
  const int mode = wide_mode();
  if (mode == 2) return true;
  if (2.0 * M * N * (double)K < 1073741824.0) return false;
  if (mode == 0 || M < 256 || N < 256) return false;
  const long kper = splitk > 1 ? K / splitk : K;
  if (kper < min_k) return false;
  const long tiles = (long)ceil_div(M, 256) * ceil_div(N, 256) * (splitk > 1 ? splitk : 1);
  const long rounds = (tiles + 255) / 256;
  static const long eff_pct = env_long("CXRK_WIDE_EFF", 60);
  return tiles * 100 >= rounds * 256 * eff_pct;
}

static inline bool prep_epilogue(EpiParams& e, int M, int N, int splitk) {
  auto ok16 = [](const void* p_, long ld) { return p_ == nullptr || (aligned16(p_) && (ld % 4) == 0); };
  auto ok8 = [](const void* p_, long ld) { return p_ == nullptr || (aligned16(p_) && (ld % 8) == 0); };
  e.vec = (N % 4 == 0) && ok16(e.C, e.ldc) && ((e.slab_stride % 4) == 0) && ok16(e.R, e.ldr) && ok16(e.aux, e.ldaux) &&
          ok16(e.C2, e.ldc2) && (e.bias == nullptr || aligned16(e.bias));
  e.pl = (e.Cp || e.Rp || e.maskin || e.maskout || e.auxmode == 3) ? 1 : 0;
  e.fast = e.vec && (N % 8) == 0 && ok8(e.Cp, e.ldc) && ok8(e.Rp, e.ldr) && (e.cplane % 8) == 0 && (e.rplane % 8) == 0 &&
           (!e.maskout || ((N % 64) == 0 && (e.ldmaskout % 8) == 0 && (((uintptr_t)e.maskout) & 7) == 0));
  e.kind = epi_kind(epi_flags(e));
  if (e.kind >= 0 && (EPI_KINDS[e.kind] & (EF_OUTPL | EF_AUX_MASK | EF_MASKOUT)) == 0u && (N % 64) != 0) e.kind = -1;
  if (e.rs2_on && !(e.Rp && e.Cp && e.rs2_H > 0 && e.rs2_W > 0 && (long)e.rs2_Ho * e.rs2_Wo > 0)) return false;
  if (e.pl) {
    if (!e.fast) return false;
    if ((e.C != nullptr) == (e.Cp != nullptr)) return false;
    if (e.R && e.Rp) return false;
    if (e.auxmode == 3 && !e.maskin) return false;
    if (e.maskout && e.act != 1) return false;
    if (e.Cp && splitk > 1) return false;
  }
  e.nt = stream_output(M, N, splitk);
  return true;
}

template <class LA, class LB, int WM, int WN>
static int launch_gemm(const typename LA::P& pa, const typename LB::P& pb, const EpiParams& ep, int M, int N, int K,
                       int splitk, hipStream_t stream, bool force_fp32 = false) {
  constexpr int BM = WM * 64, BN = WN * 64;
  if (M <= 0 || N <= 0 || K <= 0) return CXRK_ERR_ARG;
  const int nMt = ceil_div(M, BM), nNt = ceil_div(N, BN);
  int kchunk = K;
  if (splitk > 1) { kchunk = ceil_div(ceil_div(K, splitk), BK) * BK; splitk = ceil_div(K, kchunk); }
  else splitk = 1;
  dim3 grid((unsigned)(nMt * nNt * splitk), 1, 1);
  EpiParams e = ep;
  if (!prep_epilogue(e, M, N, splitk)) return CXRK_ERR_ARG;
  if (e.rs2_on) return CXRK_ERR_UNSUPPORTED;
  constexpr bool planes_in = LA::FMT_PLANES || LB::FMT_PLANES;
  const bool split = planes_in || (gemm_precision_mode() == 1 && !force_fp32 && 2.0 * M * N * (double)K >= 1073741824.0);
  if constexpr (planes_in) {
    static_assert(LA::FMT_PLANES && LB::FMT_PLANES, "both operands must share the storage format");
    hipLaunchKernelGGL((gemm_x3_kernel<LA, LB, WM, WN>), grid, dim3(NTHREADS), 0, stream, pa, pb, e, M, N, K, nMt, nNt, splitk, kchunk);
  } else if (split)
    hipLaunchKernelGGL((gemm_x3_kernel<LA, LB, WM, WN>), grid, dim3(NTHREADS), 0, stream, pa, pb, e, M, N, K, nMt, nNt, splitk, kchunk);
  else
    hipLaunchKernelGGL((gemm_f32_kernel<LA, LB, WM, WN>), grid, dim3(NTHREADS), 0, stream, pa, pb, e, M, N, K, nMt, nNt, splitk, kchunk);
  CXRK_LAUNCH_CHECK();
  return splitk;
}

}
#include "gemm_pw.h"
```

### incremental_multimodal_medical_learning_ii_amd/csrc/gemm_loaders.h

```cpp
#pragma once

namespace cxrk {

constexpr unsigned VOFF_OOB = 0x80000000u;

struct F32 {
  static constexpr bool PLANES = false;
  static constexpr int ESZ = 4;
  static constexpr int EPL = 4;
  static constexpr int NPL = 1;
  typedef float T;
  typedef float4 V;
};
struct PL {
  static constexpr bool PLANES = true;
  static constexpr int ESZ = 2;
  static constexpr int EPL = 8;
  static constexpr int NPL = 2;
  typedef unsigned short T;
  typedef uint4 V;
};

__device__ __forceinline__ __amdgpu_buffer_rsrc_t tile_rsrc(const void* p, bool live = true) {
  return __builtin_amdgcn_make_buffer_rsrc(const_cast<void*>(p), 0, live ? (int)0x80000000 : 0, 0x00020000);
}
__device__ __forceinline__ float4 bload4(__amdgpu_buffer_rsrc_t r, unsigned voff) {
  const auto q = __builtin_amdgcn_raw_buffer_load_b128(r, (int)voff, 0, 0);
  static_assert(sizeof(q) == 16, "raw_buffer_load_b128 must return 16 bytes");
  const f32x4 f = __builtin_bit_cast(f32x4, q);
  return make_float4(f[0], f[1], f[2], f[3]);
}
__device__ __forceinline__ uint4 bloadu4(__amdgpu_buffer_rsrc_t r, unsigned voff) {
  const auto q = __builtin_amdgcn_raw_buffer_load_b128(r, (int)voff, 0, 0);
  typedef unsigned u32x4 __attribute__((ext_vector_type(4)));
  const u32x4 u = __builtin_bit_cast(u32x4, q);
  return make_uint4(u[0], u[1], u[2], u[3]);
}
template <class FMT> __device__ __forceinline__ typename FMT::V bloadv(__amdgpu_buffer_rsrc_t r, unsigned voff);
template <> __device__ __forceinline__ float4 bloadv<F32>(__amdgpu_buffer_rsrc_t r, unsigned voff) { return bload4(r, voff); }
template <> __device__ __forceinline__ uint4 bloadv<PL>(__amdgpu_buffer_rsrc_t r, unsigned voff) { return bloadu4(r, voff); }

__device__ __forceinline__ unsigned masked_off(unsigned off, unsigned inv, int t) {
  return (__builtin_amdgcn_ubfe(inv, (unsigned)t, 1u) << 31) | off;
}

__device__ __forceinline__ unsigned low_bits(int k) { return k >= 32 ? 0xffffffffu : ((1u << k) - 1u); }
__device__ __forceinline__ unsigned outside_bits(int lo, int hi, int n) {
  lo = min(max(lo, 0), n); hi = min(max(hi, 0), n);
  return low_bits(lo) | (low_bits(n) & ~low_bits(hi));
}
__device__ __forceinline__ unsigned tap_mask(unsigned badr, unsigned bads, int R, int S) {
  const unsigned full = low_bits(S);
  unsigned m = 0;
#pragma unroll
  for (int r = 0; r < 8; ++r)
    if (r < R) m |= (((badr >> r) & 1u) ? full : bads) << (r * S);
  return m;
}

template <int NV, int LD, int RP>
__device__ __forceinline__ void stage_kc(float* S, int r0, int k4, const float4 (&v)[NV]) {
#pragma unroll
  for (int j = 0; j < NV; ++j) {
    float* d = S + (k4 * 4) * LD + r0 + j * RP;
    d[0] = v[j].x; d[LD] = v[j].y; d[2 * LD] = v[j].z; d[3 * LD] = v[j].w;
  }
}
template <int NV, int RP>
__device__ __forceinline__ void stage2_kc(unsigned short* hi, unsigned short* lo, int r0, int kq, const float4 (&v)[NV]) {
#pragma unroll
  for (int j = 0; j < NV; ++j) store2_kc(hi, lo, r0 + j * RP, kq * 4, v[j]);
}
template <int NV, int RP>
__device__ __forceinline__ void stage2_kc(unsigned short* hi, unsigned short* lo, int r0, int kq, const uint4 (&v)[NV]) {
#pragma unroll
  for (int j = 0; j < NV / 2; ++j) {
    *reinterpret_cast<uint4*>(hi + (r0 + j * RP) * LDH + kq * 8) = v[j];
    *reinterpret_cast<uint4*>(lo + (r0 + j * RP) * LDH + kq * 8) = v[NV / 2 + j];
  }
}
template <int NV, int LD, int RPP>
__device__ __forceinline__ void stage_mc(float* S, int kr0, int c4, const float4 (&v)[NV]) {
#pragma unroll
  for (int j = 0; j < NV; ++j) *reinterpret_cast<float4*>(S + (kr0 + j * RPP) * LD + c4 * 4) = v[j];
}
template <int NV, int LDT, int RPP>
__device__ __forceinline__ void stage2_mc(unsigned short* hi, unsigned short* lo, int kr0, int cq, const float4 (&v)[NV]) {
#pragma unroll
  for (int j = 0; j < NV; ++j) store2_mc<LDT>(hi, lo, cq * 4, kr0 + j * RPP, v[j]);
}
template <int NV, int LDT, int RPP>
__device__ __forceinline__ void stage2_mc(unsigned short* hi, unsigned short* lo, int kr0, int cq, const uint4 (&v)[NV]) {
#pragma unroll
  for (int j = 0; j < NV / 2; ++j) {
    *reinterpret_cast<uint4*>(hi + (kr0 + j * RPP) * LDT + cq * 8) = v[j];
    *reinterpret_cast<uint4*>(lo + (kr0 + j * RPP) * LDT + cq * 8) = v[NV / 2 + j];
  }
}

template <int TILE, class FMT, int NT>
struct KCGeom {
  static constexpr bool KC = true;
  static constexpr bool FMT_PLANES = FMT::PLANES;
  static constexpr int PLANE = TILE * LDH;
  static constexpr int KQ = BK / FMT::EPL;
  static constexpr int RP = NT / KQ;
  static constexpr int NVR = TILE / RP;
  static constexpr int NV = NVR * FMT::NPL;
  static constexpr int LD = TILE + 1;
  static_assert(NVR >= 1 && NVR * RP == TILE, "tile / thread-count mismatch");
};
template <int TILE, class FMT, int NT>
struct MCGeom {
  static constexpr bool KC = false;
  static constexpr bool FMT_PLANES = FMT::PLANES;
  static constexpr int LDT = TILE + 32;
  static constexpr int PLANE = BK * LDT;
  static constexpr int LD = TILE + 4;
  static constexpr int VPR = TILE / FMT::EPL;
  static constexpr int RPP = NT / VPR;
  static constexpr int NVR = BK / RPP;
  static constexpr int NV = NVR * FMT::NPL;
  static_assert(NVR >= 1 && NVR * RPP == BK, "tile / thread-count mismatch");
};

template <int TILE, class FMT = F32, int NT = NTHREADS>
struct DenseKC : KCGeom<TILE, FMT, NT> {
  typedef KCGeom<TILE, FMT, NT> G;
  typedef typename FMT::T T; typedef typename FMT::V V;
  using G::NV; using G::NVR; using G::RP; using G::KQ; using G::LD;
  struct P { const T* ptr; long ld; int rows; int K; long plane; };
  const T* bp; long plane; unsigned voff[NVR]; int kq, r0, K;
  __device__ __forceinline__ void init(const P& p, int idx0, int tid) {
    kq = tid % KQ; r0 = tid / KQ; K = p.K; plane = p.plane;
    bp = p.ptr + (long)idx0 * p.ld;
    const int ld = (int)p.ld;
#pragma unroll
    for (int j = 0; j < NVR; ++j)
      voff[j] = idx0 + r0 + j * RP < p.rows ? (unsigned)(((r0 + j * RP) * ld + kq * FMT::EPL) * FMT::ESZ) : VOFF_OOB;
  }
  __device__ __forceinline__ void load(int k0, V (&v)[NV]) {
    const unsigned t = (k0 + BK <= K || k0 + kq * FMT::EPL < K) ? 0u : VOFF_OOB;
#pragma unroll
    for (int pl = 0; pl < FMT::NPL; ++pl) {
      const __amdgpu_buffer_rsrc_t rs = tile_rsrc(bp + pl * plane + k0);
#pragma unroll
      for (int j = 0; j < NVR; ++j) v[pl * NVR + j] = bloadv<FMT>(rs, voff[j] | t);
    }
  }
  __device__ __forceinline__ void store2(unsigned short* hi, unsigned short* lo, const V (&v)[NV]) const { stage2_kc<NV, RP>(hi, lo, r0, kq, v); }
  __device__ __forceinline__ void store(float* S, const float4 (&v)[NV]) const { stage_kc<NV, LD, RP>(S, r0, kq, v); }
};

template <int TILE, class FMT = F32, int NT = NTHREADS>
struct DenseMC : MCGeom<TILE, FMT, NT> {
  typedef MCGeom<TILE, FMT, NT> G;
  typedef typename FMT::T T; typedef typename FMT::V V;
  using G::NV; using G::NVR; using G::RPP; using G::VPR; using G::LD; using G::LDT;
  struct P { const T* ptr; long ld; int cols; int K; long plane; };
  const T* bp; long ld_, plane; unsigned voff[NVR];
  int cq, kr0, K;
  __device__ __forceinline__ void init(const P& p, int idx0, int tid) {
    cq = tid % VPR; kr0 = tid / VPR; K = p.K; ld_ = p.ld; plane = p.plane;
    bp = p.ptr + idx0;
    const bool ok = idx0 + cq * FMT::EPL < p.cols;
    const int ld = (int)p.ld;
#pragma unroll
    for (int j = 0; j < NVR; ++j) voff[j] = ok ? (unsigned)(((kr0 + j * RPP) * ld + cq * FMT::EPL) * FMT::ESZ) : VOFF_OOB;
  }
  __device__ __forceinline__ void load(int k0, V (&v)[NV]) {
    const bool full = k0 + BK <= K;
#pragma unroll
    for (int pl = 0; pl < FMT::NPL; ++pl) {
      const __amdgpu_buffer_rsrc_t rs = tile_rsrc(bp + pl * plane + (long)k0 * ld_);
#pragma unroll
      for (int j = 0; j < NVR; ++j) v[pl * NVR + j] = bloadv<FMT>(rs, (full || k0 + kr0 + j * RPP < K) ? voff[j] : VOFF_OOB);
    }
  }
  __device__ __forceinline__ void store2(unsigned short* hi, unsigned short* lo, const V (&v)[NV]) const { stage2_mc<NV, LDT, RPP>(hi, lo, kr0, cq, v); }
  __device__ __forceinline__ void store(float* S, const float4 (&v)[NV]) const { stage_mc<NV, LD, RPP>(S, kr0, cq, v); }
};

struct ConvGeom {
  int N, H, W, C;
  int Ho, Wo, Ko;
  int R, S, stride, pad;
};

template <int TILE, class FMT = F32, bool TAPWISE = true, int NT = NTHREADS>
struct ConvIm2colKC : KCGeom<TILE, FMT, NT> {
  typedef KCGeom<TILE, FMT, NT> G;
  typedef typename FMT::T T; typedef typename FMT::V V;
  using G::NV; using G::NVR; using G::RP; using G::KQ; using G::LD;
  static_assert(TAPWISE || !FMT::PLANES, "the per-lane-tap gather exists for the fp32 stem only");
  struct P { const T* x; ConvGeom g; int rows; int K; long plane; };
  const T* bp; long plane;
  unsigned off[NVR];
  unsigned inv[NVR];
  int hi0[NVR], wi0[NVR];
  int kq, r0, K, H, W, C, S;
  int tr, ts, tc, knext;
  __device__ __forceinline__ void init(const P& p, int idx0, int tid) {
    kq = tid % KQ; r0 = tid / KQ; K = p.K; H = p.g.H; W = p.g.W; C = p.g.C; S = p.g.S; plane = p.plane;
    const int HoWo = p.g.Ho * p.g.Wo;
    const int n_first = idx0 / HoWo;
    const int bias = TAPWISE ? (p.g.pad * W + p.g.pad) * C : 0;
    bp = p.x + (long)n_first * H * W * C - bias;
    knext = -1; tr = ts = tc = 0;
#pragma unroll
    for (int j = 0; j < NVR; ++j) {
      const int row = idx0 + r0 + j * RP;
      const bool in = row < p.rows;
      const int rowc = in ? row : 0;
      const int wo = rowc % p.g.Wo; const int t = rowc / p.g.Wo; const int ho = t % p.g.Ho; const int n = t / p.g.Ho;
      const int h0 = ho * p.g.stride - p.g.pad, w0 = wo * p.g.stride - p.g.pad;
      const unsigned o = (unsigned)(((((n - n_first) * H + h0) * W + w0) * C + bias + (TAPWISE ? kq * FMT::EPL : 0)) * FMT::ESZ);
      off[j] = in ? o : 0u;
      if constexpr (TAPWISE) {
        const unsigned m = tap_mask(outside_bits(-h0, H - h0, p.g.R), outside_bits(-w0, W - w0, S), p.g.R, S);
        inv[j] = in ? m : 0xffffffffu;
      } else {
        hi0[j] = in ? h0 : -(1 << 28); wi0[j] = in ? w0 : 0;
      }
    }
  }
  __device__ __forceinline__ void load(int k0, V (&v)[NV]) {
    if constexpr (TAPWISE) {
      if (k0 != knext) { const int tap = k0 / C; tc = k0 - tap * C; tr = tap / S; ts = tap - tr * S; }
      const int t = tr * S + ts;
#pragma unroll
      for (int pl = 0; pl < FMT::NPL; ++pl) {
        const __amdgpu_buffer_rsrc_t rs = tile_rsrc(bp + pl * plane + ((long)(tr * W + ts) * C + tc));
#pragma unroll
        for (int j = 0; j < NVR; ++j) v[pl * NVR + j] = bloadv<FMT>(rs, masked_off(off[j], inv[j], t));
      }
      tc += BK;
      if (tc >= C) { tc = 0; if (++ts == S) { ts = 0; ++tr; } }
      knext = k0 + BK;
    } else {
      const __amdgpu_buffer_rsrc_t rs = tile_rsrc(bp);
      const int k = k0 + kq * 4;
      const int tap = k / C, c = k - tap * C;
      const int r = tap / S, s = tap - r * S;
      const unsigned toff = (unsigned)(((r * W + s) * C + c) * 4);
#pragma unroll
      for (int j = 0; j < NVR; ++j) {
        const bool ok = (k < K) && ((unsigned)(hi0[j] + r) < (unsigned)H) && ((unsigned)(wi0[j] + s) < (unsigned)W);
        v[j] = bloadv<FMT>(rs, ok ? off[j] + toff : VOFF_OOB);
      }
    }
  }
  __device__ __forceinline__ void store2(unsigned short* hi, unsigned short* lo, const V (&v)[NV]) const { stage2_kc<NV, RP>(hi, lo, r0, kq, v); }
  __device__ __forceinline__ void store(float* Sm, const float4 (&v)[NV]) const { stage_kc<NV, LD, RP>(Sm, r0, kq, v); }
};

template <int TILE, class FMT = F32, int NT = NTHREADS>
struct ConvDgradKC : KCGeom<TILE, FMT, NT> {
  typedef KCGeom<TILE, FMT, NT> G;
  typedef typename FMT::T T; typedef typename FMT::V V;
  using G::NV; using G::NVR; using G::RP; using G::KQ; using G::LD;
  struct P { const T* dy; ConvGeom g; int rows; int K; long plane; };
  const T* bp; long plane; unsigned off[NVR], inv[NVR];
  int kq, r0, Wo, Ko, R, S;
  int tr, ts, tk, knext;
  __device__ __forceinline__ void init(const P& p, int idx0, int tid) {
    kq = tid % KQ; r0 = tid / KQ; Wo = p.g.Wo; Ko = p.g.Ko; R = p.g.R; S = p.g.S; plane = p.plane;
    const int Ho = p.g.Ho, H = p.g.H, W = p.g.W, pad = p.g.pad;
    const int n_first = idx0 / (H * W);
    bp = p.dy + ((long)n_first * Ho * Wo - ((R - 1) * Wo + (S - 1))) * Ko;
    knext = -1; tr = ts = tk = 0;
#pragma unroll
    for (int j = 0; j < NVR; ++j) {
      const int row = idx0 + r0 + j * RP;
      if (row < p.rows) {
        const int wi = row % W; const int t = row / W; const int hi = t % H; const int n = t / H;
        off[j] = (unsigned)(((((n - n_first) * Ho + hi + pad) * Wo + wi + pad) * Ko + kq * FMT::EPL) * FMT::ESZ);
        inv[j] = tap_mask(outside_bits(hi + pad - Ho + 1, hi + pad + 1, R), outside_bits(wi + pad - Wo + 1, wi + pad + 1, S), R, S);
      } else { off[j] = 0; inv[j] = 0xffffffffu; }
    }
  }
  __device__ __forceinline__ void load(int k0, V (&v)[NV]) {
    if (k0 != knext) { const int tap = k0 / Ko; tk = k0 - tap * Ko; tr = tap / S; ts = tap - tr * S; }
    const int t = tr * S + ts;
#pragma unroll
    for (int pl = 0; pl < FMT::NPL; ++pl) {
      const __amdgpu_buffer_rsrc_t rs = tile_rsrc(bp + pl * plane + ((long)((R - 1 - tr) * Wo + (S - 1 - ts)) * Ko + tk));
#pragma unroll
      for (int j = 0; j < NVR; ++j) v[pl * NVR + j] = bloadv<FMT>(rs, masked_off(off[j], inv[j], t));
    }
    tk += BK;
    if (tk >= Ko) { tk = 0; if (++ts == S) { ts = 0; ++tr; } }
    knext = k0 + BK;
  }
  __device__ __forceinline__ void store2(unsigned short* hi, unsigned short* lo, const V (&v)[NV]) const { stage2_kc<NV, RP>(hi, lo, r0, kq, v); }
  __device__ __forceinline__ void store(float* Sm, const float4 (&v)[NV]) const { stage_kc<NV, LD, RP>(Sm, r0, kq, v); }
};

template <int TILE, class FMT = F32, int NT = NTHREADS>
struct ConvFilterMC : MCGeom<TILE, FMT, NT> {
  typedef MCGeom<TILE, FMT, NT> G;
  typedef typename FMT::T T; typedef typename FMT::V V;
  using G::NV; using G::NVR; using G::RPP; using G::VPR; using G::LD; using G::LDT;
  struct P { const T* w; ConvGeom g; int cols; int K; long plane; };
  const T* bp; long plane; unsigned voff[NVR]; int cq, kr0, Ko, C; long RSC;
  int tap, tk, knext;
  __device__ __forceinline__ void init(const P& p, int idx0, int tid) {
    cq = tid % VPR; kr0 = tid / VPR; Ko = p.g.Ko; C = p.g.C; RSC = (long)p.g.R * p.g.S * p.g.C; plane = p.plane;
    bp = p.w + idx0;
    const bool ok = idx0 + cq * FMT::EPL < p.cols;
    knext = -1; tap = tk = 0;
#pragma unroll
    for (int j = 0; j < NVR; ++j) voff[j] = ok ? (unsigned)(((kr0 + j * RPP) * (int)RSC + cq * FMT::EPL) * FMT::ESZ) : VOFF_OOB;
  }
  __device__ __forceinline__ void load(int k0, V (&v)[NV]) {
    if (k0 != knext) { tap = k0 / Ko; tk = k0 - tap * Ko; }
#pragma unroll
    for (int pl = 0; pl < FMT::NPL; ++pl) {
      const __amdgpu_buffer_rsrc_t rs = tile_rsrc(bp + pl * plane + ((long)tk * RSC + (long)tap * C));
#pragma unroll
      for (int j = 0; j < NVR; ++j) v[pl * NVR + j] = bloadv<FMT>(rs, voff[j]);
    }
    tk += BK;
    if (tk >= Ko) { tk = 0; ++tap; }
    knext = k0 + BK;
  }
  __device__ __forceinline__ void store2(unsigned short* hi, unsigned short* lo, const V (&v)[NV]) const { stage2_mc<NV, LDT, RPP>(hi, lo, kr0, cq, v); }
  __device__ __forceinline__ void store(float* Sm, const float4 (&v)[NV]) const { stage_mc<NV, LD, RPP>(Sm, kr0, cq, v); }
};

struct S2Taps { int nr, ns; int r[2], s[2]; int dr[2], ds[2]; };

template <int TILE, class FMT = F32, int NT = NTHREADS>
struct ConvDgradS2KC : KCGeom<TILE, FMT, NT> {
  typedef KCGeom<TILE, FMT, NT> G;
  typedef typename FMT::T T; typedef typename FMT::V V;
  using G::NV; using G::NVR; using G::RP; using G::KQ; using G::LD;
  struct P { const T* dy; ConvGeom g; S2Taps t; int Hs, Ws; int rows; int K; long plane; };
  const T* bp; long plane; unsigned off[NVR], inv[NVR];
  int kq, r0, Wo, Ko; S2Taps t;
  int ti, tk, knext;
  __device__ __forceinline__ void init(const P& p, int idx0, int tid) {
    kq = tid % KQ; r0 = tid / KQ; Wo = p.g.Wo; Ko = p.g.Ko; t = p.t; plane = p.plane;
    const int Ho = p.g.Ho;
    const int n_first = idx0 / (p.Hs * p.Ws);
    bp = p.dy + (long)n_first * Ho * Wo * Ko;
    knext = -1; ti = tk = 0;
#pragma unroll
// ... 165 lines not shown
```

### incremental_multimodal_medical_learning_ii_amd/csrc/gemm_misc.hip

```cpp
#include "cxrk.h"
#include "gemm_core.h"

using namespace cxrk;

namespace {
__global__ __launch_bounds__(256) void colsum_partial_vec_kernel(const float* __restrict__ X, long ldx, long rows, int cols,
                                                                 int rows_per, float* __restrict__ part) {
  __shared__ float4 sh[4][64];
  const int cq = threadIdx.x & 63, rl = threadIdx.x >> 6;
  const int col = blockIdx.x * 256 + cq * 4;
  const long r0 = (long)blockIdx.y * rows_per;
  const long r1 = min(rows, r0 + rows_per);
  float4 s = make_float4(0.f, 0.f, 0.f, 0.f);
  if (col < cols) {
    const float* p = X + col;
    long r = r0 + rl;
    for (; r + 28 < r1; r += 32) {
      float4 t[8];
#pragma unroll
      for (int u = 0; u < 8; ++u) t[u] = *reinterpret_cast<const float4*>(p + (r + 4 * u) * ldx);
#pragma unroll
      for (int u = 0; u < 8; ++u) { s.x += t[u].x; s.y += t[u].y; s.z += t[u].z; s.w += t[u].w; }
    }
    for (; r < r1; r += 4) { const float4 t = *reinterpret_cast<const float4*>(p + r * ldx); s.x += t.x; s.y += t.y; s.z += t.z; s.w += t.w; }
  }
  sh[rl][cq] = s;
  __syncthreads();
  if (rl == 0 && col < cols) {
    const float4 a = sh[1][cq], b = sh[2][cq], c = sh[3][cq];
    s.x = (s.x + a.x) + (b.x + c.x); s.y = (s.y + a.y) + (b.y + c.y); s.z = (s.z + a.z) + (b.z + c.z); s.w = (s.w + a.w) + (b.w + c.w);
    *reinterpret_cast<float4*>(part + (long)blockIdx.y * cols + col) = s;
  }
}
__global__ __launch_bounds__(256) void colsum_partial_pl_kernel(const unsigned short* __restrict__ X, long ldx, long plane, long rows,
                                                                int cols, int rows_per, float* __restrict__ part) {
  __shared__ float sh[8][32][8];
  const int cq = threadIdx.x & 31, rl = threadIdx.x >> 5;
  const int col = blockIdx.x * 256 + cq * 8;
  const long r0 = (long)blockIdx.y * rows_per;
  const long r1 = min(rows, r0 + rows_per);
  float s[8] = {0.f, 0.f, 0.f, 0.f, 0.f, 0.f, 0.f, 0.f};
  if (col < cols) {
    long r = r0 + rl;
    for (; r + 24 < r1; r += 32) {
      uint4 h[4], l[4];
#pragma unroll
      for (int u = 0; u < 4; ++u) {
        h[u] = *reinterpret_cast<const uint4*>(X + (r + 8 * u) * ldx + col);
        l[u] = *reinterpret_cast<const uint4*>(X + plane + (r + 8 * u) * ldx + col);
      }
#pragma unroll
      for (int u = 0; u < 4; ++u) {
        float v[8]; planes_unpack8(h[u], l[u], v);
#pragma unroll
        for (int q = 0; q < 8; ++q) s[q] += v[q];
      }
    }
    for (; r < r1; r += 8) {
      float v[8]; planes_load8(X, plane, r * ldx + col, v);
#pragma unroll
      for (int q = 0; q < 8; ++q) s[q] += v[q];
    }
  }
#pragma unroll
  for (int q = 0; q < 8; ++q) sh[rl][cq][q] = s[q];
  __syncthreads();
  if (rl == 0 && col < cols) {
#pragma unroll
    for (int q = 0; q < 8; ++q) {
      float t = s[q];
#pragma unroll
      for (int i = 1; i < 8; ++i) t += sh[i][cq][q];
      part[(long)blockIdx.y * cols + col + q] = t;
    }
  }
}
__global__ __launch_bounds__(256) void split_planes_kernel(const float* __restrict__ x, long n8, unsigned short* __restrict__ out, long plane) {
  for (long i = (long)blockIdx.x * blockDim.x + threadIdx.x; i < n8; i += (long)gridDim.x * blockDim.x) {
    const float4 a = *reinterpret_cast<const float4*>(x + i * 8), b = *reinterpret_cast<const float4*>(x + i * 8 + 4);
    const float v[8] = {a.x, a.y, a.z, a.w, b.x, b.y, b.z, b.w};
    planes_store8(out, plane, i * 8, v);
  }
}
__global__ __launch_bounds__(256) void merge_planes_kernel(const unsigned short* __restrict__ x, long plane, long n8, float* __restrict__ out) {
  for (long i = (long)blockIdx.x * blockDim.x + threadIdx.x; i < n8; i += (long)gridDim.x * blockDim.x) {
    float v[8]; planes_load8(x, plane, i * 8, v);
    *reinterpret_cast<float4*>(out + i * 8) = make_float4(v[0], v[1], v[2], v[3]);
    *reinterpret_cast<float4*>(out + i * 8 + 4) = make_float4(v[4], v[5], v[6], v[7]);
  }
}

__global__ void colsum_partial_kernel(const float* __restrict__ X, long ldx, long rows, int cols, int rows_per,
                                      float* __restrict__ part) {
  const int col = blockIdx.x * 256 + threadIdx.x;
  if (col >= cols) return;
  const long r0 = (long)blockIdx.y * rows_per;
  const long r1 = min(rows, r0 + rows_per);
  float s0 = 0.f, s1 = 0.f, s2 = 0.f, s3 = 0.f;
  long r = r0;
  for (; r + 3 < r1; r += 4) {
    s0 += X[r * ldx + col]; s1 += X[(r + 1) * ldx + col]; s2 += X[(r + 2) * ldx + col]; s3 += X[(r + 3) * ldx + col];
  }
  for (; r < r1; ++r) s0 += X[r * ldx + col];
  part[(long)blockIdx.y * cols + col] = (s0 + s1) + (s2 + s3);
}
__global__ void colvar_partial_kernel(const float* __restrict__ X, const unsigned short* __restrict__ Xp, long ldx, long plane, long rows,
                                      int cols, int rows_per, const float* __restrict__ mean, float* __restrict__ part) {
  const int col = blockIdx.x * 256 + threadIdx.x;
  if (col >= cols) return;
  const long r0 = (long)blockIdx.y * rows_per;
  const long r1 = min(rows, r0 + rows_per);
  const float m = mean[col];
  auto val = [&](long r) {
    if (Xp) return __builtin_bit_cast(float, (unsigned)Xp[r * ldx + col] << 16) + __builtin_bit_cast(float, (unsigned)Xp[plane + r * ldx + col] << 16);
    return X[r * ldx + col];
  };
  float s0 = 0.f, s1 = 0.f, s2 = 0.f, s3 = 0.f;
  long r = r0;
  for (; r + 3 < r1; r += 4) {
    const float a = val(r) - m, b = val(r + 1) - m, c = val(r + 2) - m, d = val(r + 3) - m;
    s0 = fmaf(a, a, s0); s1 = fmaf(b, b, s1); s2 = fmaf(c, c, s2); s3 = fmaf(d, d, s3);
  }
  for (; r < r1; ++r) { const float a = val(r) - m; s0 = fmaf(a, a, s0); }
  part[(long)blockIdx.y * cols + col] = (s0 + s1) + (s2 + s3);
}
__global__ void colsum_final_kernel(const float* __restrict__ part, int nparts, int cols, float* __restrict__ out,
                                    float alpha, int accumulate) {
  const int col = blockIdx.x * 256 + threadIdx.x;
  if (col >= cols) return;
  float s = 0.f;
  for (int p = 0; p < nparts; ++p) s += part[(long)p * cols + col];
  out[col] = accumulate ? out[col] + alpha * s : alpha * s;
}

}

int cxrk::wgrad_splitk_policy(int M, int N, int K, bool planes) {
  const long maxk = K / (8 * BK) > 0 ? K / (8 * BK) : 1;
  if (planes && wide_mode() != 0 && M >= 256 && N >= 256) {
    const long tiles = (long)ceil_div(M, 256) * ceil_div(N, 256);
    static const long blocks = env_long("CXRK_WGRAD_BLOCKS", 256);
    long sk = blocks / tiles;
    if (sk > maxk) sk = maxk;
    if (sk < 1) sk = 1;
    if (sk > 512) sk = 512;
    if (use_wide256(M, N, K, (int)sk, true)) return (int)sk;
  }
  const long tiles = (long)ceil_div(M, 128) * ceil_div(N, 128);
  static const long blocks128 = env_long("CXRK_WGRAD_BLOCKS128", 1536);
  long sk = (blocks128 + tiles - 1) / tiles;
  if (sk > K / 256) sk = K / 256;
  if (sk > 512) sk = 512;
  if (sk < 1) sk = 1;
  return (int)sk;
}
extern "C" int cxrk_gemm_wgrad_splitk(int M, int N, int K, int planes) { return wgrad_splitk_policy(M, N, K, planes != 0); }

extern "C" int cxrk_gemm_wide_tile(int M, int N, long K, int splitk, int kind) {
  return use_wide256(M, N, K, splitk, true, kind == 1 ? WIDE_MINK_FPROP : (kind == 2 ? WIDE_MINK_DGRAD : WIDE_MINK_PLAIN));
}

extern "C" size_t cxrk_gemm_splitk_ws_bytes(int M, int N, int splitk) {
  return splitk > 1 ? (size_t)splitk * (size_t)M * (size_t)N * sizeof(float) : 0;
}

extern "C" size_t cxrk_colsum_ws_bytes(long rows, int cols) {
  int nparts = (int)((rows + 511) / 512);
  if (nparts > 512) nparts = 512;
  if (nparts < 1) nparts = 1;
  return (size_t)nparts * (size_t)cols * sizeof(float);
}

extern "C" int cxrk_split_planes(const float* x, long n, void* out, long plane, hipStream_t stream) {
  CXRK_CHECK_ARG(x && out && n > 0 && (n % 8) == 0 && aligned16(x) && aligned16(out) && (plane % 8) == 0 && plane >= n);
  const long n8 = n / 8;
  long nb = (n8 + 255) / 256; if (nb > 4096) nb = 4096;
  hipLaunchKernelGGL(split_planes_kernel, dim3((unsigned)nb), dim3(256), 0, stream, x, n8, static_cast<unsigned short*>(out), plane);
  CXRK_LAUNCH_CHECK();
  return CXRK_OK;
}
extern "C" int cxrk_merge_planes(const void* x, long plane, long n, float* out, hipStream_t stream) {
  CXRK_CHECK_ARG(x && out && n > 0 && (n % 8) == 0 && aligned16(x) && aligned16(out) && (plane % 8) == 0);
  const long n8 = n / 8;
  long nb = (n8 + 255) / 256; if (nb > 4096) nb = 4096;
  hipLaunchKernelGGL(merge_planes_kernel, dim3((unsigned)nb), dim3(256), 0, stream, static_cast<const unsigned short*>(x), plane, n8, out);
  CXRK_LAUNCH_CHECK();
  return CXRK_OK;
}

extern "C" int cxrk_colsum_pl(const void* X, long ldx, long plane, long rows, int cols, float* out, float alpha, int accumulate,
                              float* ws, size_t ws_bytes, hipStream_t stream) {
  CXRK_CHECK_ARG(X && out && rows > 0 && cols > 0 && (cols % 8) == 0 && (ldx % 8) == 0 && (plane % 8) == 0 && aligned16(X));
  int nparts = (int)((rows + 511) / 512);
  if (nparts > 512) nparts = 512;
  if (nparts < 1) nparts = 1;
  CXRK_CHECK_WS(ws, ws_bytes, (size_t)nparts * cols * sizeof(float));
  const int rows_per = (int)((rows + nparts - 1) / nparts);
  nparts = (int)((rows + rows_per - 1) / rows_per);
  hipLaunchKernelGGL(colsum_partial_pl_kernel, dim3(ceil_div(cols, 256), nparts), dim3(256), 0, stream,
                     static_cast<const unsigned short*>(X), ldx, plane, rows, cols, rows_per, ws);
  CXRK_LAUNCH_CHECK();
  hipLaunchKernelGGL(colsum_final_kernel, dim3(ceil_div(cols, 256)), dim3(256), 0, stream, ws, nparts, cols, out, alpha, accumulate);
  CXRK_LAUNCH_CHECK();
  return CXRK_OK;
}

extern "C" int cxrk_colvar(const void* X, long ldx, long plane, long rows, int cols, const float* mean, float* out, float alpha,
                           float* ws, size_t ws_bytes, hipStream_t stream) {
  CXRK_CHECK_ARG(X && mean && out && rows > 0 && cols > 0 && plane >= 0);
  int nparts = (int)((rows + 511) / 512);
  if (nparts > 512) nparts = 512;
  if (nparts < 1) nparts = 1;
  CXRK_CHECK_WS(ws, ws_bytes, (size_t)nparts * cols * sizeof(float));
  const int rows_per = (int)((rows + nparts - 1) / nparts);
  nparts = (int)((rows + rows_per - 1) / rows_per);
  hipLaunchKernelGGL(colvar_partial_kernel, dim3(ceil_div(cols, 256), nparts), dim3(256), 0, stream,
                     plane ? nullptr : static_cast<const float*>(X), plane ? static_cast<const unsigned short*>(X) : nullptr, ldx, plane, rows,
                     cols, rows_per, mean, ws);
  CXRK_LAUNCH_CHECK();
  hipLaunchKernelGGL(colsum_final_kernel, dim3(ceil_div(cols, 256)), dim3(256), 0, stream, ws, nparts, cols, out, alpha, 0);
  CXRK_LAUNCH_CHECK();
  return CXRK_OK;
}

extern "C" int cxrk_colsum(const float* X, long ldx, long rows, int cols, float* out, float alpha, int accumulate,
                           float* ws, size_t ws_bytes, hipStream_t stream) {
  CXRK_CHECK_ARG(X && out && rows > 0 && cols > 0);
  int nparts = (int)((rows + 511) / 512);
  if (nparts > 512) nparts = 512;
  if (nparts < 1) nparts = 1;
  CXRK_CHECK_WS(ws, ws_bytes, (size_t)nparts * cols * sizeof(float));
  const int rows_per = (int)((rows + nparts - 1) / nparts);
  nparts = (int)((rows + rows_per - 1) / rows_per);
  if (cols % 4 == 0 && ldx % 4 == 0 && aligned16(X) && aligned16(ws))
    hipLaunchKernelGGL(colsum_partial_vec_kernel, dim3(ceil_div(cols, 256), nparts), dim3(256), 0, stream, X, ldx, rows, cols,
                       rows_per, ws);
  else
    hipLaunchKernelGGL(colsum_partial_kernel, dim3(ceil_div(cols, 256), nparts), dim3(256), 0, stream, X, ldx, rows, cols,
                       rows_per, ws);
  CXRK_LAUNCH_CHECK();
  hipLaunchKernelGGL(colsum_final_kernel, dim3(ceil_div(cols, 256)), dim3(256), 0, stream, ws, nparts, cols, out, alpha,
                     accumulate);
  CXRK_LAUNCH_CHECK();
  return CXRK_OK;
}
```

### incremental_multimodal_medical_learning_ii_amd/image_encoder.py

```python
from __future__ import annotations

import os

from typing import List, Optional, Sequence, Tuple

import torch

from . import _lib
from . import kernels as K
from .gradsink import GradSink
from .kernels import Planes

LAYERS = (3, 4, 6, 3)
PLANES = (64, 128, 256, 512)
BN_EPS = 1e-5


class ConvSpec:
    __slots__ = ("conv", "bn", "cin", "cpad", "cout", "k", "stride", "pad", "widx", "off")

    def __init__(self, conv, bn, cin, cout, k, stride, pad):
        self.conv, self.bn, self.cin, self.cout, self.k, self.stride, self.pad = conv, bn, cin, cout, k, stride, pad
        self.cpad = (cin + 3) // 4 * 4


def resnet50_specs(prefix: str = "encoder.encoder.", joint: int = 128) -> Tuple[List[ConvSpec], List[dict]]:
    specs: List[ConvSpec] = [ConvSpec(prefix + "conv1", prefix + "bn1", 3, 64, 7, 2, 3)]
    blocks: List[dict] = []
    inpl = 64
    for li, (nblk, planes) in enumerate(zip(LAYERS, PLANES), start=1):
        for b in range(nblk):
            pre = f"{prefix}layer{li}.{b}."
            stride = 2 if (b == 0 and li > 1) else 1
            blk = {"c1": len(specs)}
            specs.append(ConvSpec(pre + "conv1", pre + "bn1", inpl, planes, 1, 1, 0))
            blk["c2"] = len(specs)
            specs.append(ConvSpec(pre + "conv2", pre + "bn2", planes, planes, 3, stride, 1))
            blk["c3"] = len(specs)
            specs.append(ConvSpec(pre + "conv3", pre + "bn3", planes, planes * 4, 1, 1, 0))
            blk["ds"] = None
            if b == 0:
                blk["ds"] = len(specs)
                specs.append(ConvSpec(pre + "downsample.0", pre + "downsample.1", inpl, planes * 4, 1, stride, 0))
            blocks.append(blk)
            inpl = planes * 4
    specs.append(ConvSpec("projector.model.0", "projector.model.1", 2048, joint, 1, 1, 0))
    return specs, blocks


def param_names(specs: Sequence[ConvSpec]) -> List[str]:
    names: List[str] = []
    for s in specs:
        names += [s.conv + ".weight", s.bn + ".weight", s.bn + ".bias"]
    return names + ["projector.model.3.weight", "projector.model.3.bias"]


def buffer_names(specs: Sequence[ConvSpec]) -> List[str]:
    names: List[str] = []
    for s in specs:
        names += [s.bn + ".running_mean", s.bn + ".running_var"]
    return names


def _planes_mode() -> bool:
    return _lib.get_precision() == "split_bf16"


class _Fold:

    def __init__(self, specs: Sequence[ConvSpec], device, pl: bool):
        self.pl = pl
        sizes = [s.cout * s.k * s.k * s.cpad for s in specs]
        tot_c = sum(s.cout for s in specs)
        self.vec = torch.empty(3, tot_c, dtype=torch.float32, device=device)
        self.woff, self.coff = [], []
        a = b = 0
        for s, n in zip(specs, sizes):
            self.woff.append(a)
            self.coff.append(b)
            a += (n + 7) // 8 * 8
            b += s.cout
        self.sizes = sizes
        self.train = False
        self.tstate = None
        if pl:
            self.wp = torch.empty(2, a, dtype=torch.bfloat16, device=device)
            self.w = torch.empty(sizes[0], dtype=torch.float32, device=device)
        else:
            self.w = torch.empty(a, dtype=torch.float32, device=device)

    def ws(self, i, s):
        n = self.sizes[i]
        if self.pl and i > 0:
            return Planes(self.wp[:, self.woff[i]: self.woff[i] + n].view(2, s.cout, n // s.cout))
        return self.w[:n] if self.pl else self.w[self.woff[i]: self.woff[i] + n]

    def scale(self, i, s):
        return self.vec[0, self.coff[i]: self.coff[i] + s.cout]

    def shift(self, i, s):
        return self.vec[1, self.coff[i]: self.coff[i] + s.cout]

    def rstd(self, i, s):
        return self.vec[2, self.coff[i]: self.coff[i] + s.cout]


def _filter_rsc(w: torch.Tensor) -> torch.Tensor:
    v = w.permute(0, 2, 3, 1)
    return v if v.is_contiguous() else v.contiguous()


def _out_hw(s, H, W):
    return (H + 2 * s.pad - s.k) // s.stride + 1, (W + 2 * s.pad - s.k) // s.stride + 1


def _conv(i, s, fold, x, residual, relu, N, H, W, pl, want_mask=True):
    Ho, Wo = _out_hw(s, H, W)
    dev = fold.vec.device
    if not pl:
        y = torch.empty(N, Ho, Wo, s.cout, dtype=torch.float32, device=dev)
        K.conv_fwd(x, fold.ws(i, s), fold.shift(i, s), residual, y, N, H, W, s.cpad, s.cout, s.k, s.k, s.stride, s.pad, relu)
        return y, None
    y = Planes.empty(N, Ho, Wo, s.cout, device=dev)
    mask = torch.empty(N * Ho * Wo, s.cout // 8, dtype=torch.uint8, device=dev) if (relu and want_mask) else None
    K.conv_fwd_pl(x, fold.ws(i, s), fold.shift(i, s), residual, y, mask, N, H, W, s.cpad, s.cout, s.k, s.k, s.stride, s.pad, relu)
    return y, mask


def _conv_bn_train(i, s, fold, p, bufs, x, residual, relu, N, H, W, pl, want_mask, momentum):
    z, _ = _conv(i, s, fold, x, None, False, N, H, W, pl, want_mask=False)
    C = s.cout
    rows = z.numel() // C
    mean, var = K.colstats(z)
    scale, shift, rstd = K.bn_train_fwd_coeffs(mean, var, p[3 * i + 1], p[3 * i + 2], BN_EPS, rows, momentum, bufs[2 * i], bufs[2 * i + 1])
    y, mask = K.bn_apply(z, scale, shift, residual, relu, want_mask and pl)
    if fold.tstate is not None:
        fold.tstate[i] = (z, mean, rstd)
    return y, mask


def _forward(specs, blocks, p: Sequence[torch.Tensor], bufs: Sequence[torch.Tensor], x: torch.Tensor, save: bool,
             want_patch: bool, stages: Optional[list] = None, keep_stem: bool = False, bn_momentum: Optional[float] = None):
    N, C, H, W = x.shape
    if C != 3:
        raise ValueError(f"ImageModel expects 3-channel input (ExpandChannels, transforms.py:12-38), got {C}")
    dev = x.device
    pl = _planes_mode()
    fold = _Fold(specs, dev, pl)
    train = bn_momentum is not None
    fold.train = train
    if train and save:
        fold.tstate = {}
    ident = {}
    for i, s in enumerate(specs):
        if train:
            if s.cout not in ident:
                one, zero = torch.ones(s.cout, device=dev), torch.zeros(s.cout, device=dev)
                ident[s.cout] = (one, zero, zero, one - BN_EPS)
            bn = ident[s.cout]
        else:
            bn = (p[3 * i + 1], p[3 * i + 2], bufs[2 * i], bufs[2 * i + 1])
        args = (_filter_rsc(p[3 * i]), *bn, BN_EPS, s.cout, s.k * s.k, s.cin, s.cpad)
        if pl and i > 0:
            K.bn_fold_pl(*args, fold.ws(i, s), fold.scale(i, s), fold.shift(i, s), fold.rstd(i, s))
        else:
            K.bn_fold(*args, fold.ws(i, s), fold.scale(i, s), fold.shift(i, s), fold.rstd(i, s))

    def unit(i, s, fold, x, residual, relu, N, H, W, pl, want_mask=True):
        if train:
            return _conv_bn_train(i, s, fold, p, bufs, x, residual, relu, N, H, W, pl, want_mask, bn_momentum)
        return _conv(i, s, fold, x, residual, relu, N, H, W, pl, want_mask)

    x0 = K.nchw_to_nhwc(x, 4)
    stem, _ = unit(0, specs[0], fold, x0, None, True, N, H, W, pl, want_mask=False)
    Hs, Ws = stem.shape[1], stem.shape[2]
    pooled, idx = K.maxpool_fwd_pl(stem) if pl else K.maxpool_fwd(stem)
    if pl and not keep_stem:
        stem = None
    cur = pooled
    h, w = cur.shape[1], cur.shape[2]
    if stages is not None:
        stages.append(cur)
    binfo = []
    for bi, blk in enumerate(blocks):
        s1, s2, s3 = specs[blk["c1"]], specs[blk["c2"]], specs[blk["c3"]]
        o1, m1 = unit(blk["c1"], s1, fold, cur, None, True, N, h, w, pl)
        o2, m2 = unit(blk["c2"], s2, fold, o1, None, True, N, h, w, pl)
        h2, w2 = o2.shape[1], o2.shape[2]
        if blk["ds"] is not None:
            idt, _ = unit(blk["ds"], specs[blk["ds"]], fold, cur, None, False, N, h, w, pl)
        else:
            idt = cur
        out, m3 = unit(blk["c3"], s3, fold, o2, idt, True, N, h2, w2, pl)
        if save:
            binfo.append((cur, o1, o2, out if not pl else None, h, w, h2, w2, m1, m2, m3))
        cur, h, w = out, h2, w2
        if stages is not None and (bi + 1 == len(blocks) or blocks[bi + 1]["ds"] is not None):
            stages.append(cur)
    ip = len(specs) - 1
    pj1, mp = unit(ip, specs[ip], fold, cur, None, True, N, h, w, pl)
    w3, b3 = p[3 * len(specs)], p[3 * len(specs) + 1]
    w3m = w3.reshape(w3.shape[0], -1)
    if pl:
        w3p = K.split_planes(w3m)
        pj2 = K.linear_fwd_pl(pj1.view(N * h * w, pj1.shape[-1]), w3p, b3)
    else:
        w3p = None
        pj2 = K.linear_fwd(pj1.view(N * h * w, -1), w3m, b3)
    emb = K.spatial_mean_fwd(pj2.view(N, h * w, -1))
    patch = pj2.view(N, h, w, -1) if want_patch else None
    state = (fold, x0, stem, idx, pooled, binfo, cur, pj1, mp, w3p, (N, H, W, Hs, Ws, h, w), pl) if save else None
    return emb, patch, state


def _unit_params_bwd(i, s, fold, p, bufs, x, dy, sumdy, N, H, W, sink: GradSink, pl):
    w = _filter_rsc(p[3 * i])
    if fold.train:
        gw, acc = sink.dst(3 * i)
        dg = torch.empty(s.cout, dtype=torch.float32, device=w.device)
        db = torch.empty(s.cout, dtype=torch.float32, device=w.device)
    else:
        trip = [sink.dst(3 * i + k) for k in range(3)]
        if len({acc for _, acc in trip}) > 1:
            trip = [sink.dst(3 * i + k, force_fresh=True) for k in range(3)]
        (gw, acc), (dg, _), (db, _) = trip
    if not acc and not gw.permute(0, 2, 3, 1).is_contiguous():
        gw = torch.empty_like(w).permute(0, 3, 1, 2)
        sink.ret[3 * i] = gw
    dw = gw.permute(0, 2, 3, 1)
    args = (w, fold.scale(i, s), fold.rstd(i, s), bufs[2 * i], sumdy, dw, dg, db, acc, N, H, W)
    if pl and i > 0:
        K.conv_bwd_params_pl(x, dy, *args, s.cpad, s.cout, s.k, s.k, s.stride, s.pad)
    else:
        K.conv_bwd_params(x, dy, *args, s.cin, s.cpad, s.cout, s.k, s.k, s.stride, s.pad)


def _dgrad(i, s, fold, dy, residual, relu, N, H, W, pl, want_sums, residual_s2=False):
    dev = fold.vec.device
    sums = torch.empty(s.cpad, dtype=torch.float32, device=dev) if want_sums else None
    if pl:
        dx = Planes.empty(N, H, W, s.cpad, device=dev)
        K.conv_bwd_data_pl(dy, fold.ws(i, s), residual, relu, dx, N, H, W, s.cpad, s.cout, s.k, s.k, s.stride, s.pad, sums,
                           residual_s2=residual_s2)
    else:
        dx = torch.empty(N, H, W, s.cpad, dtype=torch.float32, device=dev)
        K.conv_bwd_data(dy, fold.ws(i, s), residual, relu, dx, N, H, W, s.cpad, s.cout, s.k, s.k, s.stride, s.pad, sums)
    return (dx, sums) if want_sums else dx


def stage_of_param(name: str) -> str:
    if name.startswith("projector.") or ".layer4." in name:
        return "head"
    if ".layer3." in name:
        return "layer3"
    if ".layer2." in name:
        return "layer2"
    return "stem"


def _backward(specs, blocks, p, bufs, state, demb: Optional[torch.Tensor], dpatch: Optional[torch.Tensor], sink: GradSink,
              on_grads_ready=None):
    fold, x0, stem, idx, pooled, binfo, last, pj1, mp, w3p, (N, H, W, Hs, Ws, h, w), pl = state
    def params_bwd(i, s_, x_, dy_, sum_, N_, H_, W_, pl_):
        _unit_params_bwd(i, s_, fold, p, bufs, x_, dy_, sum_, N_, H_, W_, sink, pl_)

    def report(stage):
        if on_grads_ready is not None:
            on_grads_ready(stage)

    tstate = fold.tstate

    def through_bn(i, s_, dy_, sum_):
        if tstate is None:
            return dy_, sum_
        z, mean, rstd = tstate.pop(i)
        C = s_.cout
        rows = z.numel() // C
        (dg, a1), (db, a2) = sink.dst(3 * i + 1), sink.dst(3 * i + 2)
        if a1 != a2:
            (dg, a1), (db, a2) = sink.dst(3 * i + 1, True), sink.dst(3 * i + 2, True)
        dot = K.coldot(dy_, z, mean)
        A, B, Cc = K.bn_train_bwd_coeffs(p[3 * i + 1], mean, rstd, sum_, dot, rows, dg, db, a1)
        return K.bn_train_dz(dy_, z, A, B, Cc), torch.zeros(C, dtype=torch.float32, device=dev)

    ns = len(specs)
    ip = ns - 1
    w3 = p[3 * ns]
    w3m = w3.reshape(w3.shape[0], -1)
    J = w3m.shape[0]
    dev = w3.device
    P = h * w
    gw3, acc3 = sink.dst(3 * ns)
    gb3, accb3 = sink.dst(3 * ns + 1)
    gw3m = gw3.permute(0, 2, 3, 1).reshape(J, -1) if gw3.dim() == 4 else gw3.reshape(J, -1)
    assert gw3m.data_ptr() == gw3.data_ptr()
    if pl:
        if demb is not None:
            dpj2 = K.spatial_mean_bwd_pl(demb.contiguous(), P, add=dpatch.reshape(N, P, J) if dpatch is not None else None).view(N * P, J)
        else:
            dpj2 = K.split_planes(dpatch.reshape(N * P, J).contiguous())
        pj1m = pj1.view(N * P, pj1.shape[-1])
        K.linear_bwd_weight_pl(dpj2, pj1m, gw3m, accumulate=acc3)
        K.colsum_pl(dpj2, gb3, accumulate=accb3)
        g = K.linear_bwd_data_pl(dpj2, w3p, maskin=mp, out_planes=True)
        sum_p = K.colsum_pl(g, torch.empty(g.shape[1], dtype=torch.float32, device=dev))
        g = g.view(N, h, w, g.shape[1])
    else:
        if demb is not None:
            dpj2 = K.spatial_mean_bwd(demb.contiguous(), P).view(N * P, J)
            if dpatch is not None:
                dpj2 = dpj2 + dpatch.reshape(N * P, J)
        else:
            dpj2 = dpatch.reshape(N * P, J).contiguous()
        pj1m = pj1.view(N * P, -1)
        K.linear_bwd_weight(dpj2, pj1m, gw3m, accumulate=acc3)
        K.colsum(dpj2, gb3, accumulate=accb3)
        g = K.linear_bwd_data(dpj2, w3m, aux=pj1m, auxmode=K.AUX_RELU_MASK)
        sum_p = K.colsum(g, torch.empty(g.shape[1], dtype=torch.float32, device=dev))
        g = g.view(N, h, w, -1)
    g, sum_p = through_bn(ip, specs[ip], g, sum_p)
    params_bwd(ip, specs[ip], last, g, sum_p, N, h, w, pl)

    nb = len(blocks)

    def relu_of_block_out(bi):
        return binfo[bi][10] if pl else binfo[bi][3]

    g, gs = _dgrad(ip, specs[ip], fold, g, None, relu_of_block_out(nb - 1), N, h, w, pl, True)
    for bi in reversed(range(nb)):
        blk = blocks[bi]
        cur, o1, o2, out, hi, wi, h2, w2, m1, m2, m3 = binfo[bi]
        s1, s2, s3 = specs[blk["c1"]], specs[blk["c2"]], specs[blk["c3"]]
        g3, gs3 = through_bn(blk["c3"], s3, g, gs)
        params_bwd(blk["c3"], s3, o2, g3, gs3, N, h2, w2, pl)
        d2, q2 = _dgrad(blk["c3"], s3, fold, g3, None, m2 if pl else o2, N, h2, w2, pl, True)
        del g3
        d2, q2 = through_bn(blk["c2"], s2, d2, q2)
        params_bwd(blk["c2"], s2, o1, d2, q2, N, hi, wi, pl)
        d1, q1 = _dgrad(blk["c2"], s2, fold, d2, None, m1 if pl else o1, N, hi, wi, pl, True)
        del d2
        d1, q1 = through_bn(blk["c1"], s1, d1, q1)
        params_bwd(blk["c1"], s1, cur, d1, q1, N, hi, wi, pl)
        if blk["ds"] is not None:
            sd = specs[blk["ds"]]
            gd, gsd = through_bn(blk["ds"], sd, g, gs)
            params_bwd(blk["ds"], sd, cur, gd, gsd, N, hi, wi, pl)
            res = None
            if pl and sd.k == 1 and sd.stride == 2 and sd.pad == 0 and os.environ.get("CXRK_S2RES", "1") != "0":
                res = K.conv1x1_s2_bwd_data_compact_pl(gd, fold.ws(blk["ds"], sd), N, hi, wi, sd.cpad, sd.cout)
                res_s2 = res is not None
            if res is None:
                res = _dgrad(blk["ds"], sd, fold, gd, None, None, N, hi, wi, pl, False)
                res_s2 = False
            del gd
        else:
            res, res_s2 = g, False
        if bi > 0:
            g, gs = _dgrad(blk["c1"], s1, fold, d1, res, relu_of_block_out(bi - 1), N, hi, wi, pl, True, residual_s2=res_s2)
        else:
            g, gs = _dgrad(blk["c1"], s1, fold, d1, res, None, N, hi, wi, pl, False, residual_s2=res_s2), None
        del d1, res
        binfo[bi] = None
        if on_grads_ready is not None and blk["ds"] is not None and bi > 0:
            stage = {LAYERS[0] + LAYERS[1] + LAYERS[2]: "head", LAYERS[0] + LAYERS[1]: "layer3", LAYERS[0]: "layer2"}[bi]
            if all(r is None for r in sink.ret[3 * blk["c1"]:]):
                report(stage)
    if pl:
        ds = K.maxpool_bwd_pl(g, idx, pooled, Hs, Ws)
    else:
        ds = K.maxpool_bwd(g, idx, stem, True)
    if _debug is not None:
        _debug["ds"], _debug["x0"] = ds, x0
    sum_s = K.colsum(ds.view(-1, ds.shape[-1]), torch.empty(ds.shape[-1], dtype=torch.float32, device=dev))
    ds, sum_s = through_bn(0, specs[0], ds, sum_s)
    params_bwd(0, specs[0], x0, ds, sum_s, N, H, W, False)
    if on_grads_ready is not None and all(r is None for r in sink.ret):
        report("stem")
    return sink.ret


class Decisions(list):
    pool_taps: Optional[torch.Tensor] = None


def relu_decisions(state) -> List[torch.Tensor]:
    fold, x0, stem, idx, pooled, binfo, cur, pj1, mp, w3p, dims, pl = state
    N, H, W, Hs, Ws, h, w = dims

    def nchw(t):
        return (t > 0).permute(0, 3, 1, 2).contiguous().cpu()

    taps = idx.permute(0, 3, 1, 2).contiguous().cpu()
    if not pl:
        acts = [stem]
        for b in binfo:
            acts += [b[1], b[2], b[3]]
        acts.append(pj1)
        out = Decisions(nchw(a) for a in acts)
        out.pool_taps = taps
        return out
    if stem is None:
        raise RuntimeError("relu_decisions: the stem output was not kept (run the forward inside capture_relu_decisions())")
    out = Decisions([nchw(stem.float())])
    out.pool_taps = taps
    for b in binfo:
        _, _, _, _, hi, wi, h2, w2, m1, m2, m3 = b
        for m, hh, ww in ((m1, hi, wi), (m2, h2, w2), (m3, h2, w2)):
            C = m.shape[1] * 8
            out.append(K.unpack_mask(m, C).view(N, hh, ww, C).permute(0, 3, 1, 2).contiguous())
    C = mp.shape[1] * 8
    out.append(K.unpack_mask(mp, C).view(N, h, w, C).permute(0, 3, 1, 2).contiguous())
    return out


def _pack_bits(a: torch.Tensor) -> torch.Tensor:
    rows, C = a.shape
    w = 1 << torch.arange(8, device=a.device, dtype=torch.int32)
    return (a.view(rows, C // 8, 8).to(torch.int32) * w).sum(-1).to(torch.uint8)


def device_decisions(state) -> dict:
    fold, x0, stem, idx, pooled, binfo, cur, pj1, mp, w3p, dims, pl = state
    if pl:
        blocks = [(b[8], b[9], b[10]) for b in binfo]
        proj = mp
        stem_pos = pooled.t[0].float() > 0
    else:
        blocks = [tuple(_pack_bits((b[k] > 0).view(-1, b[k].shape[-1])) for k in (1, 2, 3)) for b in binfo]
        proj = _pack_bits((pj1 > 0).view(-1, pj1.shape[-1]))
        stem_pos = pooled > 0
    return {"blocks": [tuple(m.clone() for m in t) for t in blocks], "proj": proj.clone(), "pool_taps": idx.clone(), "stem_pos": stem_pos}


def count_decision_differences(a: dict, b: dict) -> dict:
    def bits(x, y):
        d = (x ^ y).to(torch.int32)
        n = 0
        for k in range(8):
            n += int(((d >> k) & 1).sum())
        return n
    relu = sum(bits(x, y) for ta, tb in zip(a["blocks"], b["blocks"]) for x, y in zip(ta, tb)) + bits(a["proj"], b["proj"])
    total = sum(x.numel() * 8 for ta in a["blocks"] for x in ta) + a["proj"].numel() * 8
    return {"relu": relu + int((a["stem_pos"] != b["stem_pos"]).sum()), "relu_total": total + a["stem_pos"].numel(),
            "pool_taps": int((a["pool_taps"] != b["pool_taps"]).sum()), "pool_total": a["pool_taps"].numel()}


def impose_decisions_(node, dec: dict) -> None:
    fold, x0, stem, idx, pooled, binfo, cur, pj1, mp, w3p, dims, pl = node.state
    if not pl:
        raise RuntimeError("impose_decisions_: only the planes (split_bf16) backward reads stored decisions")
    for b, t in zip(binfo, dec["blocks"]):
        for m, src in zip((b[8], b[9], b[10]), t):
            m.copy_(src)
    mp.copy_(dec["proj"])
    idx.copy_(dec["pool_taps"])
    sign = Planes(torch.zeros_like(pooled.t))
    sign.t[0].copy_(dec["stem_pos"].to(torch.bfloat16))
    node.state = (fold, x0, stem, idx, sign, binfo, cur, pj1, mp, w3p, dims, pl)


@torch.no_grad()
def calibrate_batchnorm_(specs, blocks, params, bufs, x: torch.Tensor) -> None:
    import math
    N, C, H, W = x.shape
    dev = x.device
    pl = _planes_mode()
    fold = _Fold(specs, dev, pl)
    p = [t.detach() for t in params]
    b = [t.detach() for t in bufs]
    k = math.sqrt(1.0 + BN_EPS)

    def fold_unit(i, s, gamma, beta, mean, var):
        args = (_filter_rsc(p[3 * i]), gamma, beta, mean, var, BN_EPS, s.cout, s.k * s.k, s.cin, s.cpad)
        fn = K.bn_fold_pl if (pl and i > 0) else K.bn_fold
        fn(*args, fold.ws(i, s), fold.scale(i, s), fold.shift(i, s), fold.rstd(i, s))

    def unit(i, xin, residual, relu, h, w, want_mask=True):
        s = specs[i]
        one, zero = torch.ones(s.cout, device=dev), torch.zeros(s.cout, device=dev)
        fold_unit(i, s, one, zero, zero, one)
        raw, _ = _conv(i, s, fold, xin, None, False, N, h, w, pl, want_mask=False)
        r = raw.view(-1, s.cout)
        rows = r.shape[0]
        K.colsum(r, b[2 * i], alpha=1.0 / rows)
        K.colvar(r, b[2 * i], b[2 * i + 1], alpha=k * k / max(1, rows - 1))
        K.scale_mask(b[2 * i], alpha=k, out=b[2 * i])
        del raw, r
        fold_unit(i, s, p[3 * i + 1], p[3 * i + 2], b[2 * i], b[2 * i + 1])
        return _conv(i, s, fold, xin, residual, relu, N, h, w, pl, want_mask=want_mask)[0]

    stem = unit(0, K.nchw_to_nhwc(x, 4), None, True, H, W, want_mask=False)
    cur = (K.maxpool_fwd_pl(stem) if pl else K.maxpool_fwd(stem))[0]
    del stem
    h, w = cur.shape[1], cur.shape[2]
    for blk in blocks:
        o1 = unit(blk["c1"], cur, None, True, h, w)
        o2 = unit(blk["c2"], o1, None, True, h, w)
        h2, w2 = o2.shape[1], o2.shape[2]
        idt = unit(blk["ds"], cur, None, False, h, w) if blk["ds"] is not None else cur
        cur, h, w = unit(blk["c3"], o2, idt, True, h2, w2), h2, w2
    unit(len(specs) - 1, cur, None, True, h, w)


_capture: Optional[list] = None
_debug: Optional[dict] = None


class capture_relu_decisions:

    def __enter__(self):
        global _capture
        self._old, _capture = _capture, []
        return _capture

    def __exit__(self, *exc):
        global _capture
        _capture = self._old
        return False


class ImageEncodeFn(torch.autograd.Function):

    @staticmethod
    def forward(ctx, x, meta, *tensors):
        specs, blocks, n_params, want_patch = meta[:4]
        ctx.set_materialize_grads(False)
# ... 61 lines not shown
```

### incremental_multimodal_medical_learning_ii_amd/kernels.py

```python
from __future__ import annotations

from typing import NamedTuple, Optional, Tuple

import torch

from . import _lib
from ._lib import check

ACT_NONE, ACT_RELU, ACT_GELU = 0, 1, 2
AUX_NONE, AUX_RELU_MASK, AUX_GELU_GRAD, AUX_MASK_BITS = 0, 1, 2, 3


def _stream() -> int:
    return torch.cuda.current_stream().cuda_stream


def _p(t: Optional[torch.Tensor]) -> Optional[int]:
    return None if t is None else t.data_ptr()


def _chk(t: torch.Tensor, name: str, dtype=torch.float32) -> torch.Tensor:
    if not isinstance(t, torch.Tensor) or not t.is_cuda:
        raise ValueError(f"{name}: expected a tensor on the GPU (the cxrk path has no CPU fallback), got "
                         f"{type(t).__name__} on {getattr(t, 'device', None)}")
# ... 525 lines not shown
def _dgrad_label(N, H, W, Ko, R, S, stride):
    if stride == 1:
        return "ConvDgradKC", "ConvFilterMC", N * H * W, R * S * Ko, 1
    classes = 4 if R > 1 else 1
    return "ConvDgradS2KC", "ConvFilterS2MC", N * ((H + 1) // 2) * ((W + 1) // 2), Ko * max(1, (R * S) // 4), classes


def conv_bwd_data(dy, w_scaled, residual, relu_src, dx, N, H, W, C, Ko, R, S, stride, pad, sums=None):
    lib = _lib.load()
    ws = workspace(lib.cxrk_conv_bwd_data_colsum_ws_bytes(N, H, W, C, stride), dy.device) if sums is not None else None
    ev = None
    if profiler.on:
        Ho, Wo = _conv_out(H, W, R, S, stride, pad)
        fl = 2.0 * N * Ho * Wo * Ko * R * S * C
        la, lb, Ml, Kl, sub = _dgrad_label(N, H, W, Ko, R, S, stride)
        ev = profiler.bracket(_label(la, lb, "4,1" if C <= 64 else "2,2", Ml, C, Kl, 1, 2), fl,
                              4.0 * (N * Ho * Wo * Ko + Ko * R * S * C + N * H * W * C * (1 + (residual is not None) + (relu_src is not None))), sub)
    rc = lib.cxrk_conv_bn_act_bwd_data(_p(_chk(dy, "conv.dy")), _p(w_scaled), _p(residual), _p(relu_src), _p(dx), N, H,
                                       W, C, Ko, R, S, stride, pad, _p(sums), _p(ws), ws.numel() * 4 if ws is not None else 0, _stream())
    if ev is not None:
        ev.record()
    check(rc, f"cxrk_conv_bn_act_bwd_data(N={N},H={H},W={W},C={C},Ko={Ko},R={R},s={stride})")
    return dx


def conv_bwd_params(x, dy, w, scale, rstd, rmean, sumdy, dw, dgamma, dbeta, accumulate, N, H, W, C, Cpad, Ko, R, S, stride, pad):
    lib = _lib.load()
    wsb = lib.cxrk_conv_wgrad_ws_bytes(N, H, W, Cpad, Ko, R, S, stride, pad)
    ws = workspace(wsb, x.device)
    ev = None
    if profiler.on:
        Ho, Wo = _conv_out(H, W, R, S, stride, pad)
        fl = 2.0 * N * Ho * Wo * Ko * R * S * Cpad
        sk = lib.cxrk_gemm_wgrad_splitk(Ko, R * S * Cpad, N * Ho * Wo, 0)
        ev = profiler.bracket(_label("DenseMC", "ConvIm2colMC", "1,4" if Ko <= 64 else "2,2", Ko, R * S * Cpad, N * Ho * Wo, sk, 0,
                                     False), fl, 4.0 * (N * H * W * Cpad + N * Ho * Wo * Ko + Ko * R * S * Cpad))
    check(lib.cxrk_conv_bn_act_bwd_params(_p(_chk(x, "conv.x")), _p(_chk(dy, "conv.dy")), _p(w), _p(scale), _p(rstd),
                                          _p(rmean), _p(sumdy), _p(dw), _p(dgamma), _p(dbeta), int(accumulate), N, H, W,
                                          C, Cpad, Ko, R, S, stride, pad, _p(ws), ws.numel() * 4, _stream()),
          f"cxrk_conv_bn_act_bwd_params(N={N},H={H},W={W},C={C},Ko={Ko},R={R},s={stride})")
    if ev is not None:
        ev.record()



def bn_fold_pl(w, gamma, beta, rmean, rvar, eps, Ko, taps, C, Cpad, w_scaled: Planes, scale, shift, rstd):
    lib = _lib.load()
    for n, t in (("w", w), ("gamma", gamma), ("beta", beta), ("rmean", rmean), ("rvar", rvar)):
        _chk(t, "bn_fold." + n)
    check(lib.cxrk_bn_fold_pl(_p(w), _p(gamma), _p(beta), _p(rmean), _p(rvar), float(eps), Ko, taps, C, Cpad, w_scaled.ptr(),
                              w_scaled.plane, _p(scale), _p(shift), _p(rstd), _stream()), "cxrk_bn_fold_pl")


def conv_fwd_pl(x, w_scaled, shift, residual: Optional[Planes], y: Planes, maskout, N, H, W, C, Ko, R, S, stride, pad, relu):
    lib = _lib.load()
    in_planes = isinstance(x, Planes)
    if in_planes != isinstance(w_scaled, Planes):
        raise ValueError("conv_fwd_pl: x and w_scaled must share the storage format")
    ev = None
    if profiler.on:
        Ho, Wo = _conv_out(H, W, R, S, stride, pad)
        fl = 2.0 * N * Ho * Wo * Ko * R * S * C
        nb = 4.0 * (N * H * W * C + Ko * R * S * C + N * Ho * Wo * Ko * (1 + (residual is not None))) + (N * Ho * Wo * Ko / 8.0 if maskout is not None else 0.0)
        if in_planes:
            key = _label("ConvIm2colKC", "DenseKC", "4,1" if Ko <= 64 else "2,2", N * Ho * Wo, Ko, R * S * C, 1, 1, planes=True)
        else:
            key = _label("ConvIm2colKC", "DenseKC", "4,1" if Ko <= 64 else "2,2", N * Ho * Wo, Ko, R * S * C, 1, 3)
        ev = profiler.bracket(key, fl, nb)
    if maskout is not None:
        _chk(maskout, "conv.maskout", torch.uint8)
    xp, xpl = (x.ptr(), x.plane) if in_planes else (_p(_chk(x, "conv.x")), 0)
    wp, wpl = (w_scaled.ptr(), w_scaled.plane) if in_planes else (_p(_chk(w_scaled, "conv.w")), 0)
    rc = lib.cxrk_conv_bn_act_fwd_pl(xp, xpl, wp, wpl, int(in_planes), _p(shift), residual.ptr() if residual is not None else None,
                                     residual.plane if residual is not None else 0, y.ptr(), y.plane, _p(maskout), N, H, W, C, Ko, R, S,
                                     stride, pad, int(relu), _stream())
    if ev is not None:
        ev.record()
    check(rc, f"cxrk_conv_bn_act_fwd_pl(N={N},H={H},W={W},C={C},Ko={Ko},R={R},s={stride})")
    return y


def conv_bwd_data_pl(dy: Planes, w_scaled: Planes, residual: Optional[Planes], maskin, dx: Planes, N, H, W, C, Ko, R, S, stride, pad,
                     sums=None, residual_s2: bool = False):
    lib = _lib.load()
    if residual_s2:
        if residual is None or tuple(residual.shape) != (N, (H + 1) // 2, (W + 1) // 2, C):
            raise ValueError(f"conv_bwd_data_pl: compact residual must be [N, (H+1)//2, (W+1)//2, C], got {None if residual is None else tuple(residual.shape)}")
    ws = workspace(lib.cxrk_conv_bwd_data_colsum_ws_bytes(N, H, W, C, stride), dy.device) if sums is not None else None
    ev = None
    if profiler.on:
        Ho, Wo = _conv_out(H, W, R, S, stride, pad)
        fl = 2.0 * N * Ho * Wo * Ko * R * S * C
        la, lb, Ml, Kl, sub = _dgrad_label(N, H, W, Ko, R, S, stride)
        ev = profiler.bracket(_label(la, lb, "4,1" if C <= 64 else "2,2", Ml, C, Kl, 1, 2, planes=True), fl,
                              4.0 * (N * Ho * Wo * Ko + Ko * R * S * C + N * H * W * C * (1 + (0.0 if residual is None else 0.25 if residual_s2 else 1.0)))
                              + (N * H * W * C / 8.0 if maskin is not None else 0.0), sub)
    fn = lib.cxrk_conv_bn_act_bwd_data_pl_s2res if residual_s2 else lib.cxrk_conv_bn_act_bwd_data_pl
    rc = fn(dy.ptr(), dy.plane, w_scaled.ptr(), w_scaled.plane, residual.ptr() if residual is not None else None,
                                          residual.plane if residual is not None else 0, _p(maskin), dx.ptr(), dx.plane, N, H, W, C, Ko, R, S,
                                          stride, pad, _p(sums), _p(ws), ws.numel() * 4 if ws is not None else 0, _stream())
    if ev is not None:
        ev.record()
    check(rc, f"cxrk_conv_bn_act_bwd_data_pl{'_s2res' if residual_s2 else ''}(N={N},H={H},W={W},C={C},Ko={Ko},R={R},s={stride})")
    return dx


def conv1x1_s2_bwd_data_compact_pl(dy: Planes, w_scaled: Planes, N, H, W, C, Ko) -> Optional[Planes]:
    Ho, Wo = (H + 1) // 2, (W + 1) // 2
    if N * Ho * Wo * C * 2 >= (1 << 31):
        return None
    if tuple(dy.shape) not in ((N, Ho, Wo, Ko), (N * Ho * Wo, Ko)) or tuple(w_scaled.shape) != (Ko, C):
        raise ValueError(f"conv1x1_s2_bwd_data_compact_pl: dy {tuple(dy.shape)}, w {tuple(w_scaled.shape)} for N={N},H={H},W={W},C={C},Ko={Ko}")
    out = Planes.empty(N * Ho * Wo, C, device=dy.device)
    linear_bwd_data_pl(dy.view(N * Ho * Wo, Ko), w_scaled, out=out)
    return out.view(N, Ho, Wo, C)


def conv_bwd_params_pl(x: Planes, dy: Planes, w, scale, rstd, rmean, sumdy, dw, dgamma, dbeta, accumulate, N, H, W, C, Ko, R, S, stride, pad):
    lib = _lib.load()
    ws = workspace(lib.cxrk_conv_wgrad_ws_bytes(N, H, W, C, Ko, R, S, stride, pad), x.device)
    ev = None
    if profiler.on:
        Ho, Wo = _conv_out(H, W, R, S, stride, pad)
        fl = 2.0 * N * Ho * Wo * Ko * R * S * C
        sk = lib.cxrk_gemm_wgrad_splitk(Ko, R * S * C, N * Ho * Wo, 1)
        ev = profiler.bracket(_label("DenseMC", "ConvIm2colMC", "1,4" if Ko <= 64 else "2,2", Ko, R * S * C, N * Ho * Wo, sk, 0, planes=True),
                              fl, 4.0 * (N * H * W * C + N * Ho * Wo * Ko + Ko * R * S * C))
    check(lib.cxrk_conv_bn_act_bwd_params_pl(x.ptr(), x.plane, dy.ptr(), dy.plane, _p(w), _p(scale), _p(rstd), _p(rmean), _p(sumdy),
                                             _p(dw), _p(dgamma), _p(dbeta), int(accumulate), N, H, W, C, Ko, R, S, stride, pad, _p(ws),
                                             ws.numel() * 4, _stream()),
          f"cxrk_conv_bn_act_bwd_params_pl(N={N},H={H},W={W},C={C},Ko={Ko},R={R},s={stride})")
    if ev is not None:
        ev.record()


def maxpool_fwd_pl(x: Planes):
    lib = _lib.load()
    N, H, W, C = x.shape
    Ho, Wo = (H - 1) // 2 + 1, (W - 1) // 2 + 1
    y = Planes.empty(N, Ho, Wo, C, device=x.device)
    idx = torch.empty(N, Ho, Wo, C, dtype=torch.uint8, device=x.device)
    check(lib.cxrk_maxpool_fwd_pl(x.ptr(), x.plane, y.ptr(), y.plane, _p(idx), N, H, W, C, _stream()), "cxrk_maxpool_fwd_pl")
    return y, idx


def maxpool_bwd_pl(dy: Planes, idx, pooled: Planes, H: int, W: int) -> torch.Tensor:
    lib = _lib.load()
    N, _, _, C = pooled.shape
    dx = torch.empty(N, H, W, C, dtype=torch.float32, device=dy.device)
    check(lib.cxrk_maxpool_bwd_pl(dy.ptr(), dy.plane, _p(idx), pooled.ptr(), _p(dx), N, H, W, C, _stream()), "cxrk_maxpool_bwd_pl")
    return dx


def spatial_mean_bwd_pl(dy: torch.Tensor, Pn: int, add: Optional[torch.Tensor] = None) -> Planes:
    lib = _lib.load()
    N, C = dy.shape
    dx = Planes.empty(N, Pn, C, device=dy.device)
    if add is not None:
        add = _chk(add, "spatial_mean.add").contiguous()
    check(lib.cxrk_spatial_mean_bwd_pl(_p(_chk(dy.contiguous(), "spatial_mean.dy")), _p(add), dx.ptr(), dx.plane, N, Pn, C, _stream()),
          "cxrk_spatial_mean_bwd_pl")
    return dx


def unpack_mask(mask: torch.Tensor, C: int) -> torch.Tensor:
    m = mask.cpu().reshape(-1, C // 8).to(torch.int32)
    bits = (m.unsqueeze(-1) >> torch.arange(8, dtype=torch.int32)) & 1
    return bits.reshape(-1, C).bool()


def nchw_to_nhwc(x: torch.Tensor, cpad: int) -> torch.Tensor:
    lib = _lib.load()
    _chk(x, "nchw_to_nhwc.x")
    x = x.contiguous()
    N, C, H, W = x.shape
    y = torch.empty(N, H, W, cpad, dtype=torch.float32, device=x.device)
    check(lib.cxrk_nchw_to_nhwc(_p(x), _p(y), N, C, H, W, cpad, _stream()), "cxrk_nchw_to_nhwc")
    return y


def nhwc_to_nchw(x: torch.Tensor) -> torch.Tensor:
    lib = _lib.load()
    _chk(x, "nhwc_to_nchw.x")
    N, H, W, C = x.shape
    y = torch.empty(N, C, H, W, dtype=torch.float32, device=x.device)
    check(lib.cxrk_nhwc_to_nchw(_p(x), _p(y), N, C, H, W, _stream()), "cxrk_nhwc_to_nchw")
    return y


def maxpool_fwd(x: torch.Tensor):
    lib = _lib.load()
    N, H, W, C = x.shape
    Ho, Wo = (H - 1) // 2 + 1, (W - 1) // 2 + 1
    y = torch.empty(N, Ho, Wo, C, dtype=torch.float32, device=x.device)
    idx = torch.empty(N, Ho, Wo, C, dtype=torch.uint8, device=x.device)
    check(lib.cxrk_maxpool_fwd(_p(_chk(x, "maxpool.x")), _p(y), _p(idx), N, H, W, C, _stream()), "cxrk_maxpool_fwd")
    return y, idx


def maxpool_bwd(dy, idx, x, relu_mask: bool):
    lib = _lib.load()
    N, H, W, C = x.shape
    dx = torch.empty_like(x)
    check(lib.cxrk_maxpool_bwd(_p(_chk(dy, "maxpool.dy")), _p(idx), _p(x), _p(dx), N, H, W, C, int(relu_mask), _stream()),
          "cxrk_maxpool_bwd")
    return dx


def spatial_mean_fwd(x: torch.Tensor) -> torch.Tensor:
    lib = _lib.load()
    N, Pn, C = x.shape
    y = torch.empty(N, C, dtype=torch.float32, device=x.device)
    check(lib.cxrk_spatial_mean_fwd(_p(_chk(x, "spatial_mean.x")), _p(y), N, Pn, C, _stream()), "cxrk_spatial_mean_fwd")
    return y


def spatial_mean_bwd(dy: torch.Tensor, Pn: int) -> torch.Tensor:
    lib = _lib.load()
    N, C = dy.shape
    dx = torch.empty(N, Pn, C, dtype=torch.float32, device=dy.device)
    check(lib.cxrk_spatial_mean_bwd(_p(_chk(dy.contiguous(), "spatial_mean.dy")), _p(dx), N, Pn, C, _stream()),
          "cxrk_spatial_mean_bwd")
    return dx



def _new_out(rows, cols, device, planes: bool):
    if planes:
        o = Planes.empty(rows, cols, device=device)
        return o, o.ptr(), o.plane
    o = torch.empty(rows, cols, dtype=torch.float32, device=device)
    return o, o.data_ptr(), 0


class Drop(NamedTuple):
    seed: int
    counter: int
    layer: int
    site: int
    row_offset: int
    p: float

    def args(self):
        return (self.seed & (2 ** 64 - 1), self.counter & 0xFFFFFFFF, self.layer, self.site, self.row_offset, float(self.p))


DROP_EMBED, DROP_ATTN_PROBS, DROP_ATTN_OUT, DROP_FFN_OUT = 0, 1, 2, 3


def dropout_mask(drop: Drop, N: int, L: int, C: int, nH: int = 1, device="cuda") -> torch.Tensor:
    keep = torch.empty(N, nH, L, C, dtype=torch.uint8, device=device)
    check(_lib.load().cxrk_dropout_mask(*drop.args(), N, L, nH, C, _p(keep), _stream()), "cxrk_dropout_mask")
    return keep


def embed_ln_fwd(ids, word, pos, type_row, gamma, beta, eps, L, out_planes: bool = False, drop: Optional[Drop] = None):
    lib = _lib.load()
    _chk(ids, "embed.ids", torch.int64)
    ids = ids.contiguous()
    T = ids.numel()
    H = word.shape[1]
    y, yp, ypl = _new_out(T, H, word.device, out_planes)
    xhat = torch.empty(T, H, dtype=torch.float32, device=word.device)
    rstd = torch.empty(T, dtype=torch.float32, device=word.device)
    if drop is not None:
        check(lib.cxrk_embed_ln_fwd_drop(_p(ids), _p(_chk(word, "embed.word")), _p(pos), _p(type_row), _p(gamma), _p(beta),
                                         float(eps), T, L, H, yp, ypl, _p(xhat), _p(rstd), *drop.args(), _stream()),
              "cxrk_embed_ln_fwd_drop")
        return y, xhat, rstd
    check(lib.cxrk_embed_ln_fwd(_p(ids), _p(_chk(word, "embed.word")), _p(pos), _p(type_row), _p(gamma), _p(beta),
                                float(eps), T, L, H, yp, ypl, _p(xhat), _p(rstd), _stream()), "cxrk_embed_ln_fwd")
    return y, xhat, rstd


def residual_ln_fwd(x, res, gamma, beta, eps, save: bool = True, out_planes: bool = False, drop: Optional[Drop] = None,
                    rows_per_seq: int = 1):
    lib = _lib.load()
    rows, H = x.shape
    y, yp, ypl = _new_out(rows, H, x.device, out_planes)
    xhat = torch.empty_like(x) if save else None
    rstd = torch.empty(rows, dtype=torch.float32, device=x.device) if save else None
    if drop is not None:
        if res is None:
            raise ValueError("residual_ln_fwd(drop=...): the residual is required")
        if isinstance(res, Planes):
            rp, rld, rpl = _pl2d(res, "ln.res")
        else:
            _chk(res, "ln.res")
            if res.stride(1) != 1:
                raise ValueError("ln.res: columns must be contiguous")
            rp, rld, rpl = res.data_ptr(), res.stride(0), 0
        check(lib.cxrk_residual_ln_fwd_drop(_p(_chk(x, "ln.x")), rp, rpl, rld, _p(gamma), _p(beta), float(eps), rows, H, int(rows_per_seq),
                                            yp, ypl, _p(xhat), _p(rstd), *drop.args(), _stream()), "cxrk_residual_ln_fwd_drop")
        return y, xhat, rstd
    check(lib.cxrk_residual_ln_fwd(_p(_chk(x, "ln.x")), _p(res), _p(gamma), _p(beta), float(eps), rows, H, yp, ypl,
                                   _p(xhat), _p(rstd), _stream()), "cxrk_residual_ln_fwd")
    return y, xhat, rstd


def residual_ln_bwd(dy, xhat, rstd, gamma, dgamma, dbeta, dx_add=None, accumulate: bool = False, out=None, out_planes: bool = False,
                    dxsum=None, dxsum_accumulate: bool = False):
    lib = _lib.load()
    rows, H = dy.shape
    if out is None:
        dx, dxp, dxpl = _new_out(rows, H, dy.device, out_planes)
    elif isinstance(out, Planes):
        dx, dxp, dxpl = out, out.ptr(), out.plane
    else:
        dx, dxp, dxpl = out, out.data_ptr(), 0
    wsb = lib.cxrk_residual_ln_bwd_ws_bytes(rows, H)
    ws = workspace(wsb, dy.device)
    check(lib.cxrk_residual_ln_bwd(_p(_chk(dy, "ln.dy")), _p(xhat), _p(rstd), _p(gamma), rows, H, _p(dx_add), dxp, dxpl,
                                   _p(dgamma), _p(dbeta), int(accumulate), _p(dxsum), int(dxsum_accumulate), _p(ws), ws.numel() * 4,
                                   _stream()),
          "cxrk_residual_ln_bwd")
    return dx


def residual_ln_bwd_drop(dy, xhat, rstd, gamma, dgamma, dbeta, drop: Drop, rows_per_seq: int, accumulate: bool = False,
                         out_planes: bool = False, dxsum=None, dxsum_accumulate: bool = False, mask_dy: bool = False, out=None):
    lib = _lib.load()
    rows, H = dy.shape
    if out is not None:
        dx, dxm = out
        _chk_out(dx, (rows, H), "ln.out[0]")
        if (dxm is None) != bool(mask_dy):
            raise ValueError("residual_ln_bwd_drop: out = (dx, dxm), dxm None exactly when mask_dy")
        dxp, dxpl = (dx.ptr(), dx.plane) if isinstance(dx, Planes) else (dx.data_ptr(), 0)
        dxmp = None
        if dxm is not None:
            _chk_out(dxm, (rows, H), "ln.out[1]")
# ... 400 lines not shown
```

Measured before the change: 6737.

## Pre-split stem image into bf16 planes and fuse maxpool backward with column sums

The stem image is converted once from NCHW fp32 into a packed NHWC4 layout already split into bf16 hi/lo planes. Dedicated stem forward-conv and weight-gradient kernels then read that pre-split input directly instead of re-splitting fp32 inside every GEMM tile load. Separately, the maxpool backward kernel now also accumulates per-channel gradient sums through block partials, which removes the separate colsum pass over the stem gradient. The risks are extra code paths gated by precision mode and problem size, and a slightly different summation order for the BN reductions.

New measurement: 6798, median of 6. No clear change (+0.9%).

```diff
diff --git a/include/cxrk.h b/include/cxrk.h
--- a/include/cxrk.h
+++ b/include/cxrk.h
@@ -67,7 +67,15 @@
                                    float* dbeta, int accumulate, int N, int H, int W, int C, int Ko, int R, int S, int stride,
                                    int pad, float* ws, size_t ws_bytes, hipStream_t stream);
 
+int cxrk_conv_bn_act_fwd_pl_stem(const void* x, int presplit, const float* w_scaled, const float* shift, void* y, long yplane, int N,
+                                 int H, int W, int Ko, int R, int S, int stride, int pad, int relu, hipStream_t stream);
+int cxrk_conv_bn_act_bwd_params_stem(const void* x, int presplit, const float* dy, const float* w, const float* scale,
+                                     const float* rstd, const float* rmean, const float* sumdy, float* dw, float* dgamma,
+                                     float* dbeta, int accumulate, int N, int H, int W, int C, int Ko, int R, int S, int stride,
+                                     int pad, float* slabs, size_t slabs_bytes, hipStream_t stream);
+
 int cxrk_nchw_to_nhwc(const float* x, float* y, int N, int C, int H, int W, int Cpad, hipStream_t stream);
+int cxrk_nchw_to_nhwc4_split(const float* x, void* y, int N, int H, int W, hipStream_t stream);
 int cxrk_nhwc_to_nchw(const float* x, float* y, int N, int C, int H, int W, hipStream_t stream);
 
 int cxrk_maxpool_fwd(const float* x, float* y, unsigned char* idx, int N, int H, int W, int C, hipStream_t stream);
@@ -77,6 +85,8 @@
                         hipStream_t stream);
 int cxrk_maxpool_bwd_pl(const void* dy, long dyplane, const unsigned char* idx, const void* pooled, float* dx, int N, int H,
                         int W, int C, hipStream_t stream);
+int cxrk_maxpool_bwd_pl_sums(const void* dy, long dyplane, const unsigned char* idx, const void* pooled, float* dx, float* sums,
+                             int accumulate, int N, int H, int W, int C, float* partials, size_t partials_bytes, hipStream_t stream);
 
 int cxrk_spatial_mean_fwd(const float* x, float* y, int N, int P, int C, hipStream_t stream);
 int cxrk_spatial_mean_bwd(const float* dy, float* dx, int N, int P, int C, hipStream_t stream);
diff --git a/incremental_multimodal_medical_learning_ii_amd/_lib.py b/incremental_multimodal_medical_learning_ii_amd/_lib.py
--- a/incremental_multimodal_medical_learning_ii_amd/_lib.py
+++ b/incremental_multimodal_medical_learning_ii_amd/_lib.py
@@ -41,11 +41,15 @@
     "cxrk_bn_train_bwd_coeffs": (I, [P, P, P, P, P, L, P, P, P, P, P, I, I, P]),
     "cxrk_bn_train_dz": (I, [P, L, P, L, P, P, P, P, L, L, I, P]),
     "cxrk_nchw_to_nhwc": (I, [P, P, I, I, I, I, I, P]),
+    "cxrk_nchw_to_nhwc4_split": (I, [P, P, I, I, I, P]),
+    "cxrk_conv_bn_act_fwd_pl_stem": (I, [P, I, P, P, P, L, I, I, I, I, I, I, I, I, I, P]),
+    "cxrk_conv_bn_act_bwd_params_stem": (I, [P, I, P, P, P, P, P, P, P, P, P, I, I, I, I, I, I, I, I, I, I, P, Z, P]),
     "cxrk_nhwc_to_nchw": (I, [P, P, I, I, I, I, P]),
     "cxrk_maxpool_fwd": (I, [P, P, P, I, I, I, I, P]),
     "cxrk_maxpool_bwd": (I, [P, P, P, P, I, I, I, I, I, P]),
     "cxrk_maxpool_fwd_pl": (I, [P, L, P, L, P, I, I, I, I, P]),
     "cxrk_maxpool_bwd_pl": (I, [P, L, P, P, P, I, I, I, I, P]),
+    "cxrk_maxpool_bwd_pl_sums": (I, [P, L, P, P, P, P, I, I, I, I, I, P, Z, P]),
     "cxrk_spatial_mean_fwd": (I, [P, P, I, I, I, P]),
     "cxrk_spatial_mean_bwd": (I, [P, P, I, I, I, P]),
     "cxrk_spatial_mean_bwd_pl": (I, [P, P, P, L, I, I, I, P]),
diff --git a/incremental_multimodal_medical_learning_ii_amd/csrc/conv_fwd.hip b/incremental_multimodal_medical_learning_ii_amd/csrc/conv_fwd.hip
--- a/incremental_multimodal_medical_learning_ii_amd/csrc/conv_fwd.hip
+++ b/incremental_multimodal_medical_learning_ii_amd/csrc/conv_fwd.hip
@@ -81,3 +81,30 @@
   return conv_fwd_impl<F32>(static_cast<const float*>(x), 0, static_cast<const float*>(w_scaled), 0, ep, N, H, W, C, Ko, R, S, stride,
                             pad, stream);
 }
+
+extern "C" int cxrk_conv_bn_act_fwd_pl_stem(const void* x, int presplit, const float* w_scaled, const float* shift, void* y, long yplane,
+                                            int N, int H, int W, int Ko, int R, int S, int stride, int pad, int relu,
+                                            hipStream_t stream) {
+  constexpr int C = 4;
+  CXRK_CHECK_ARG(x && w_scaled && y && N > 0 && Ko > 0 && (Ko % 8) == 0 && aligned16(x) && aligned16(w_scaled));
+  CXRK_CHECK_ARG(stride == 1 || stride == 2);
+  if (Ko > 64) return CXRK_ERR_UNSUPPORTED;
+  const ConvGeom g = make_geom(N, H, W, C, Ko, R, S, stride, pad);
+  CXRK_CHECK_ARG(g.Ho > 0 && g.Wo > 0);
+  const long Ml = (long)N * g.Ho * g.Wo;
+  CXRK_CHECK_ARG(Ml < (1L << 31));
+  const int M = (int)Ml, K = R * S * C;
+  if (!tile_span_ok((long)g.Ho * g.Wo, (long)H * W * C)) return CXRK_ERR_UNSUPPORTED;
+  EpiParams ep{};
+  ep.Cp = static_cast<unsigned short*>(y); ep.cplane = yplane; ep.ldc = Ko; ep.bias = shift; ep.ldr = Ko; ep.act = relu ? 1 : 0; ep.alpha = 1.f;
+  DenseKC<64>::P pb{w_scaled, (long)K, Ko, K, 0};
+  int rc;
+  if (presplit) {
+    ConvIm2colKC<256, PS4, false>::P pa{static_cast<const unsigned*>(x), g, M, K, 0};
+    rc = launch_gemm<ConvIm2colKC<256, PS4, false>, DenseKC<64>, 4, 1>(pa, pb, ep, M, Ko, K, 1, stream);
+  } else {
+    ConvIm2colKC<256, F32, false>::P pa{static_cast<const float*>(x), g, M, K, 0};
+    rc = launch_gemm<ConvIm2colKC<256, F32, false>, DenseKC<64>, 4, 1>(pa, pb, ep, M, Ko, K, 1, stream, false, true);
+  }
+  return rc < 0 ? rc : CXRK_OK;
+}
diff --git a/incremental_multimodal_medical_learning_ii_amd/csrc/conv_misc.hip b/incremental_multimodal_medical_learning_ii_amd/csrc/conv_misc.hip
--- a/incremental_multimodal_medical_learning_ii_amd/csrc/conv_misc.hip
+++ b/incremental_multimodal_medical_learning_ii_amd/csrc/conv_misc.hip
@@ -35,6 +35,16 @@
     const int wv = i / Cpad, c = i - wv * Cpad;
     y[(nh * W + wv) * Cpad + c] = c < C ? x[((n * C + c) * H + hh) * W + wv] : 0.f;
   }
+}
+__global__ __launch_bounds__(256) void nchw_to_nhwc4_split_kernel(const float* __restrict__ x, uint4* __restrict__ y, long HW, long total) {
+  const long p = (long)blockIdx.x * blockDim.x + threadIdx.x;
+  if (p >= total) return;
+  const long n = p / HW;
+  const float* src = x + n * 2 * HW + p;
+  uint4 o;
+  split2(src[0], src[HW], o.x, o.z);
+  split2(src[2 * HW], 0.f, o.y, o.w);
+  y[p] = o;
 }
 __global__ void nhwc_to_nchw_kernel(const float* __restrict__ x, float* __restrict__ y, int C, int H, int W) {
   const long nh = blockIdx.x;
@@ -180,16 +190,13 @@
   *reinterpret_cast<float4*>(dx + e) = make_float4(g[0], g[1], g[2], g[3]);
   *reinterpret_cast<float4*>(dx + e + 4) = make_float4(g[4], g[5], g[6], g[7]);
 }
-__global__ __launch_bounds__(256) void maxpool_bwd_pl_kernel(const unsigned short* __restrict__ dy, long dyplane, const unsigned char* __restrict__ idx,
-                                                             const unsigned short* __restrict__ pooled, float* __restrict__ dx, int N, int H,
-                                                             int W, int C, int Ho, int Wo) {
-  const long t = (long)blockIdx.x * blockDim.x + threadIdx.x;
+__device__ __forceinline__ void pool_bwd_item(long t, PoolWin& w00, const unsigned short* __restrict__ dy, long dyplane,
+                                              const unsigned char* __restrict__ idx, const unsigned short* __restrict__ pooled,
+                                              float* __restrict__ dx, int H, int W, int C, int Ho, int Wo) {
   const int C8 = C / 8, H2 = (H + 1) / 2, W2 = (W + 1) / 2;
-  const long total = (long)N * H2 * W2 * C8;
-  if (t >= total) return;
   const int c8 = (int)(t % C8); long p = t / C8;
   const int b = (int)(p % W2); p /= W2; const int a = (int)(p % H2); const long n = p / H2;
-  PoolWin w00, w01, w10, w11;
+  PoolWin w01, w10, w11;
   const bool va = a < Ho, va1 = a + 1 < Ho, vb = b < Wo, vb1 = b + 1 < Wo;
   const long o00 = (((n * Ho + a) * Wo + b) * C8 + c8) * 8;
   pool_win_load(w00, va && vb, dy, dyplane, idx, pooled, o00);
@@ -219,6 +226,40 @@
     pool_store(dx, e + (long)(W + 1) * C, g);
   }
 }
+__global__ __launch_bounds__(256) void maxpool_bwd_pl_kernel(const unsigned short* __restrict__ dy, long dyplane, const unsigned char* __restrict__ idx,
+                                                             const unsigned short* __restrict__ pooled, float* __restrict__ dx, int N, int H,
+                                                             int W, int C, int Ho, int Wo) {
+  const long t = (long)blockIdx.x * blockDim.x + threadIdx.x;
+  const long total = (long)N * ((H + 1) / 2) * ((W + 1) / 2) * (C / 8);
+  if (t >= total) return;
+  PoolWin w00;
+  pool_bwd_item(t, w00, dy, dyplane, idx, pooled, dx, H, W, C, Ho, Wo);
+}
+constexpr int POOL_SUMS_NT = 512;
+__global__ __launch_bounds__(POOL_SUMS_NT) void maxpool_bwd_pl_sums_kernel(const unsigned short* __restrict__ dy, long dyplane,
+                                                                           const unsigned char* __restrict__ idx,
+                                                                           const unsigned short* __restrict__ pooled, float* __restrict__ dx,
+                                                                           int N, int H, int W, int C, int Ho, int Wo, float* __restrict__ part) {
+  __shared__ float sh[POOL_SUMS_NT][9];
+  const long total = (long)N * ((H + 1) / 2) * ((W + 1) / 2) * (C / 8);
+  float s[8] = {0.f, 0.f, 0.f, 0.f, 0.f, 0.f, 0.f, 0.f};
+  for (long t = (long)blockIdx.x * POOL_SUMS_NT + threadIdx.x; t < total; t += (long)gridDim.x * POOL_SUMS_NT) {
+    PoolWin w00;
+    pool_bwd_item(t, w00, dy, dyplane, idx, pooled, dx, H, W, C, Ho, Wo);
+#pragma unroll
+    for (int q = 0; q < 8; ++q) s[q] += w00.tap[q] != 0xffu ? w00.d[q] : 0.f;
+  }
+#pragma unroll
+  for (int q = 0; q < 8; ++q) sh[threadIdx.x][q] = s[q];
+  __syncthreads();
+  const int C8 = C / 8;
+  for (int c = threadIdx.x; c < C; c += POOL_SUMS_NT) {
+    const int c8 = c >> 3, q = c & 7;
+    float a = 0.f;
+    for (int i = c8; i < POOL_SUMS_NT; i += C8) a += sh[i][q];
+    part[(long)blockIdx.x * C + c] = a;
+  }
+}
 __global__ void spatial_mean_bwd_pl_kernel(const float* __restrict__ dy, const float* __restrict__ add, unsigned short* __restrict__ dx,
                                            long dxplane, int P, int C) {
   const int n = blockIdx.x;
@@ -266,6 +307,15 @@
   CXRK_LAUNCH_CHECK();
   return CXRK_OK;
 }
+extern "C" int cxrk_nchw_to_nhwc4_split(const float* x, void* y, int N, int H, int W, hipStream_t stream) {
+  CXRK_CHECK_ARG(x && y && N > 0 && H > 0 && W > 0 && aligned16(y));
+  const long total = (long)N * H * W;
+  CXRK_CHECK_ARG((total + 255) / 256 < (1L << 31));
+  hipLaunchKernelGGL(nchw_to_nhwc4_split_kernel, dim3((unsigned)((total + 255) / 256)), dim3(256), 0, stream, x, static_cast<uint4*>(y),
+                     (long)H * W, total);
+  CXRK_LAUNCH_CHECK();
+  return CXRK_OK;
+}
 extern "C" int cxrk_nhwc_to_nchw(const float* x, float* y, int N, int C, int H, int W, hipStream_t stream) {
   CXRK_CHECK_ARG(x && y && N > 0 && C > 0);
   hipLaunchKernelGGL(nhwc_to_nchw_kernel, dim3((unsigned)((long)N * H)), dim3(256), 0, stream, x, y, C, H, W);
@@ -312,6 +362,20 @@
   return CXRK_OK;
 }
 
+extern "C" int cxrk_maxpool_bwd_pl_sums(const void* dy, long dyplane, const unsigned char* idx, const void* pooled, float* dx, float* sums,
+                                        int accumulate, int N, int H, int W, int C, float* partials, size_t partials_bytes,
+                                        hipStream_t stream) {
+  CXRK_CHECK_ARG(dy && idx && pooled && dx && sums && N > 0 && H > 0 && W > 0 && C > 0 && C % 8 == 0 && POOL_SUMS_NT % (C / 8) == 0);
+  CXRK_CHECK_ARG(aligned16(dy) && aligned16(pooled) && aligned16(dx) && (dyplane % 8) == 0 && (((uintptr_t)idx) & 7) == 0);
+  const int Ho = (H + 2 - 3) / 2 + 1, Wo = (W + 2 - 3) / 2 + 1;
+  const int nparts = colsum_parts((long)N * Ho * Wo);
+  CXRK_CHECK_WS(partials, partials_bytes, (size_t)nparts * C * sizeof(float));
+  hipLaunchKernelGGL(maxpool_bwd_pl_sums_kernel, dim3((unsigned)nparts), dim3(POOL_SUMS_NT), 0, stream, static_cast<const unsigned short*>(dy),
+                     dyplane, idx, static_cast<const unsigned short*>(pooled), dx, N, H, W, C, Ho, Wo, partials);
+  CXRK_LAUNCH_CHECK();
+  return colsum_finish(partials, nparts, C, sums, 1.f, accumulate, stream);
+}
+
 extern "C" int cxrk_spatial_mean_fwd(const float* x, float* y, int N, int P, int C, hipStream_t stream) {
   CXRK_CHECK_ARG(x && y && N > 0 && P > 0 && C > 0);
   hipLaunchKernelGGL(spatial_mean_fwd_kernel, dim3(N), dim3(128), 0, stream, x, y, P, C);
diff --git a/incremental_multimodal_medical_learning_ii_amd/csrc/conv_wgrad.hip b/incremental_multimodal_medical_learning_ii_amd/csrc/conv_wgrad.hip
--- a/incremental_multimodal_medical_learning_ii_amd/csrc/conv_wgrad.hip
+++ b/incremental_multimodal_medical_learning_ii_amd/csrc/conv_wgrad.hip
@@ -1,4 +1,5 @@
 #include "conv_common.h"
+#include <type_traits>
 
 using namespace cxrk;
 
@@ -82,11 +83,12 @@
   return ((size_t)sk * (size_t)Ko * (size_t)(R * S * C) + (size_t)Ko * wgrad_dot_parts(R * S * C)) * sizeof(float);
 }
 
-template <class FMT>
-static int conv_bwd_params_impl(const typename FMT::T* x, long xplane, const typename FMT::T* dy, long dyplane, const float* w,
+template <class FMT, class XF = FMT>
+static int conv_bwd_params_impl(const typename XF::T* x, long xplane, const typename FMT::T* dy, long dyplane, const float* w,
                                 const float* scale, const float* rstd, const float* rmean, const float* sumdy, float* dw,
                                 float* dgamma, float* dbeta, int accumulate, int N, int H, int W, int C, int Cpad, int Ko, int R,
-                                int S, int stride, int pad, float* ws, size_t ws_bytes, hipStream_t stream) {
+                                int S, int stride, int pad, float* ws, size_t ws_bytes, hipStream_t stream, bool force_split = false) {
+  constexpr bool same_fmt = std::is_same<FMT, XF>::value;
   CXRK_CHECK_ARG(x && dy && dw && N > 0 && Cpad % FMT::EPL == 0 && Ko % FMT::EPL == 0 && aligned16(x) && aligned16(dy));
   CXRK_CHECK_ARG(!(dgamma && !(w && rstd && rmean && sumdy && dbeta)));
   const ConvGeom g = make_geom(N, H, W, Cpad, Ko, R, S, stride, pad);
@@ -111,16 +113,16 @@
       DmaDenseMC<64, 4>::P pa{dy, (long)Ko, Ko, Kred, dyplane}; DmaConvIm2colMC<256, 4>::P pb{x, g, Nc, Kred, xplane};
       rc = launch_gemm_pw<Pw64x256, DmaDenseMC<64, 4>, DmaConvIm2colMC<256, 4>>(pa, pb, ep, Ko, Nc, Kred, sk, stream);
     } else {
-      typename DenseMC<64, FMT>::P pa{dy, (long)Ko, Ko, Kred, dyplane}; typename ConvIm2colMC<256, FMT>::P pb{x, g, Nc, Kred, xplane};
-      rc = launch_gemm<DenseMC<64, FMT>, ConvIm2colMC<256, FMT>, 1, 4>(pa, pb, ep, Ko, Nc, Kred, sk, stream, exact);
+      typename DenseMC<64, FMT>::P pa{dy, (long)Ko, Ko, Kred, dyplane}; typename ConvIm2colMC<256, XF>::P pb{x, g, Nc, Kred, xplane};
+      rc = launch_gemm<DenseMC<64, FMT>, ConvIm2colMC<256, XF>, 1, 4>(pa, pb, ep, Ko, Nc, Kred, sk, stream, exact, force_split);
     }
   } else if constexpr (FMT::PLANES) {
     DmaDenseMC<128, 4>::P pa{dy, (long)Ko, Ko, Kred, dyplane}; DmaConvIm2colMC<128, 4>::P pb{x, g, Nc, Kred, xplane};
     rc = launch_gemm_pw<Pw128, DmaDenseMC<128, 4>, DmaConvIm2colMC<128, 4>>(pa, pb, ep, Ko, Nc, Kred, sk, stream);
-  } else {
+  } else if constexpr (same_fmt) {
     typename DenseMC<128, FMT>::P pa{dy, (long)Ko, Ko, Kred, dyplane}; typename ConvIm2colMC<128, FMT>::P pb{x, g, Nc, Kred, xplane};
     rc = launch_gemm<DenseMC<128, FMT>, ConvIm2colMC<128, FMT>, 2, 2>(pa, pb, ep, Ko, Nc, Kred, sk, stream, exact);
-  }
+  } else return CXRK_ERR_UNSUPPORTED;
   if (rc < 0) return rc;
   const int sg_log2 = rc >= 64 ? 4 : (rc >= 8 ? 2 : 0);
   const int ny = ceil_div(Nc, 4 * (256 >> sg_log2));
@@ -153,3 +155,16 @@
                                   rstd, rmean, sumdy, dw, dgamma, dbeta, accumulate, N, H, W, C, C, Ko, R, S, stride, pad, ws, ws_bytes,
                                   stream);
 }
+
+extern "C" int cxrk_conv_bn_act_bwd_params_stem(const void* x, int presplit, const float* dy, const float* w, const float* scale,
+                                                const float* rstd, const float* rmean, const float* sumdy, float* dw, float* dgamma,
+                                                float* dbeta, int accumulate, int N, int H, int W, int C, int Ko, int R, int S,
+                                                int stride, int pad, float* slabs, size_t slabs_bytes, hipStream_t stream) {
+  CXRK_CHECK_ARG(C > 0 && C <= 4);
+  if (Ko > 64) return CXRK_ERR_UNSUPPORTED;
+  if (presplit)
+    return conv_bwd_params_impl<F32, PS4>(static_cast<const unsigned*>(x), 0, dy, 0, w, scale, rstd, rmean, sumdy, dw, dgamma, dbeta,
+                                          accumulate, N, H, W, C, 4, Ko, R, S, stride, pad, slabs, slabs_bytes, stream);
+  return conv_bwd_params_impl<F32>(static_cast<const float*>(x), 0, dy, 0, w, scale, rstd, rmean, sumdy, dw, dgamma, dbeta, accumulate,
+                                   N, H, W, C, 4, Ko, R, S, stride, pad, slabs, slabs_bytes, stream, true);
+}
diff --git a/incremental_multimodal_medical_learning_ii_amd/csrc/gemm_core.h b/incremental_multimodal_medical_learning_ii_amd/csrc/gemm_core.h
--- a/incremental_multimodal_medical_learning_ii_amd/csrc/gemm_core.h
+++ b/incremental_multimodal_medical_learning_ii_amd/csrc/gemm_core.h
@@ -369,6 +369,8 @@
 }
 
 int wgrad_splitk_policy(int M, int N, int K, bool planes);
+int colsum_parts(long rows);
+int colsum_finish(const float* part, int nparts, int cols, float* out, float alpha, int accumulate, hipStream_t stream);
 
 inline int& wide_mode_ref() { static int m = [] { const char* e = getenv("CXRK_WIDE"); return e ? atoi(e) : 1; }(); return m; }
 inline int wide_mode() { return wide_mode_ref(); }
@@ -419,7 +421,7 @@
 
 template <class LA, class LB, int WM, int WN>
 static int launch_gemm(const typename LA::P& pa, const typename LB::P& pb, const EpiParams& ep, int M, int N, int K,
-                       int splitk, hipStream_t stream, bool force_fp32 = false) {
+                       int splitk, hipStream_t stream, bool force_fp32 = false, bool force_split = false) {
   constexpr int BM = WM * 64, BN = WN * 64;
   if (M <= 0 || N <= 0 || K <= 0) return CXRK_ERR_ARG;
   const int nMt = ceil_div(M, BM), nNt = ceil_div(N, BN);
@@ -431,9 +433,11 @@
   if (!prep_epilogue(e, M, N, splitk)) return CXRK_ERR_ARG;
   if (e.rs2_on) return CXRK_ERR_UNSUPPORTED;
   constexpr bool planes_in = LA::FMT_PLANES || LB::FMT_PLANES;
-  const bool split = planes_in || (gemm_precision_mode() == 1 && !force_fp32 && 2.0 * M * N * (double)K >= 1073741824.0);
-  if constexpr (planes_in) {
-    static_assert(LA::FMT_PLANES && LB::FMT_PLANES, "both operands must share the storage format");
+  constexpr bool presplit_in = LA::FMT_PRESPLIT || LB::FMT_PRESPLIT;
+  const bool split = planes_in || presplit_in || force_split ||
+                     (gemm_precision_mode() == 1 && !force_fp32 && 2.0 * M * N * (double)K >= 1073741824.0);
+  if constexpr (planes_in || presplit_in) {
+    static_assert(!planes_in || (LA::FMT_PLANES && LB::FMT_PLANES), "planes operands must share the storage format");
     hipLaunchKernelGGL((gemm_x3_kernel<LA, LB, WM, WN>), grid, dim3(NTHREADS), 0, stream, pa, pb, e, M, N, K, nMt, nNt, splitk, kchunk);
   } else if (split)
     hipLaunchKernelGGL((gemm_x3_kernel<LA, LB, WM, WN>), grid, dim3(NTHREADS), 0, stream, pa, pb, e, M, N, K, nMt, nNt, splitk, kchunk);
diff --git a/incremental_multimodal_medical_learning_ii_amd/csrc/gemm_loaders.h b/incremental_multimodal_medical_learning_ii_amd/csrc/gemm_loaders.h
--- a/incremental_multimodal_medical_learning_ii_amd/csrc/gemm_loaders.h
+++ b/incremental_multimodal_medical_learning_ii_amd/csrc/gemm_loaders.h
@@ -4,16 +4,28 @@
 
 constexpr unsigned VOFF_OOB = 0x80000000u;
 
+struct PSV { uint2 hi, lo; };
 struct F32 {
   static constexpr bool PLANES = false;
+  static constexpr bool PRESPLIT = false;
   static constexpr int ESZ = 4;
   static constexpr int EPL = 4;
   static constexpr int NPL = 1;
   typedef float T;
   typedef float4 V;
 };
+struct PS4 {
+  static constexpr bool PLANES = false;
+  static constexpr bool PRESPLIT = true;
+  static constexpr int ESZ = 4;
+  static constexpr int EPL = 4;
+  static constexpr int NPL = 1;
+  typedef unsigned T;
+  typedef PSV V;
+};
 struct PL {
   static constexpr bool PLANES = true;
+  static constexpr bool PRESPLIT = false;
   static constexpr int ESZ = 2;
   static constexpr int EPL = 8;
   static constexpr int NPL = 2;
@@ -39,6 +51,10 @@
 template <class FMT> __device__ __forceinline__ typename FMT::V bloadv(__amdgpu_buffer_rsrc_t r, unsigned voff);
 template <> __device__ __forceinline__ float4 bloadv<F32>(__amdgpu_buffer_rsrc_t r, unsigned voff) { return bload4(r, voff); }
 template <> __device__ __forceinline__ uint4 bloadv<PL>(__amdgpu_buffer_rsrc_t r, unsigned voff) { return bloadu4(r, voff); }
+template <> __device__ __forceinline__ PSV bloadv<PS4>(__amdgpu_buffer_rsrc_t r, unsigned voff) {
+  const uint4 u = bloadu4(r, voff);
+  return PSV{make_uint2(u.x, u.y), make_uint2(u.z, u.w)};
+}
 
 __device__ __forceinline__ unsigned masked_off(unsigned off, unsigned inv, int t) {
   return (__builtin_amdgcn_ubfe(inv, (unsigned)t, 1u) << 31) | off;
@@ -72,6 +88,14 @@
   for (int j = 0; j < NV; ++j) store2_kc(hi, lo, r0 + j * RP, kq * 4, v[j]);
 }
 template <int NV, int RP>
+__device__ __forceinline__ void stage2_kc(unsigned short* hi, unsigned short* lo, int r0, int kq, const PSV (&v)[NV]) {
+#pragma unroll
+  for (int j = 0; j < NV; ++j) {
+    *reinterpret_cast<uint2*>(hi + (r0 + j * RP) * LDH + kq * 4) = v[j].hi;
+    *reinterpret_cast<uint2*>(lo + (r0 + j * RP) * LDH + kq * 4) = v[j].lo;
+  }
+}
+template <int NV, int RP>
 __device__ __forceinline__ void stage2_kc(unsigned short* hi, unsigned short* lo, int r0, int kq, const uint4 (&v)[NV]) {
 #pragma unroll
   for (int j = 0; j < NV / 2; ++j) {
@@ -88,6 +112,14 @@
 __device__ __forceinline__ void stage2_mc(unsigned short* hi, unsigned short* lo, int kr0, int cq, const float4 (&v)[NV]) {
 #pragma unroll
   for (int j = 0; j < NV; ++j) store2_mc<LDT>(hi, lo, cq * 4, kr0 + j * RPP, v[j]);
+}
+template <int NV, int LDT, int RPP>
+__device__ __forceinline__ void stage2_mc(unsigned short* hi, unsigned short* lo, int kr0, int cq, const PSV (&v)[NV]) {
+#pragma unroll
+  for (int j = 0; j < NV; ++j) {
+    *reinterpret_cast<uint2*>(hi + (kr0 + j * RPP) * LDT + cq * 4) = v[j].hi;
+    *reinterpret_cast<uint2*>(lo + (kr0 + j * RPP) * LDT + cq * 4) = v[j].lo;
+  }
 }
 template <int NV, int LDT, int RPP>
 __device__ __forceinline__ void stage2_mc(unsigned short* hi, unsigned short* lo, int kr0, int cq, const uint4 (&v)[NV]) {
@@ -102,6 +134,7 @@
 struct KCGeom {
   static constexpr bool KC = true;
   static constexpr bool FMT_PLANES = FMT::PLANES;
+  static constexpr bool FMT_PRESPLIT = FMT::PRESPLIT;
   static constexpr int PLANE = TILE * LDH;
   static constexpr int KQ = BK / FMT::EPL;
   static constexpr int RP = NT / KQ;
@@ -114,6 +147,7 @@
 struct MCGeom {
   static constexpr bool KC = false;
   static constexpr bool FMT_PLANES = FMT::PLANES;
+  static constexpr bool FMT_PRESPLIT = FMT::PRESPLIT;
   static constexpr int LDT = TILE + 32;
   static constexpr int PLANE = BK * LDT;
   static constexpr int LD = TILE + 4;
@@ -192,7 +226,8 @@
   typedef KCGeom<TILE, FMT, NT> G;
   typedef typename FMT::T T; typedef typename FMT::V V;
   using G::NV; using G::NVR; using G::RP; using G::KQ; using G::LD;
-  static_assert(TAPWISE || !FMT::PLANES, "the per-lane-tap gather exists for the fp32 stem only");
+  static_assert(TAPWISE || !FMT::PLANES, "the per-lane-tap gather exists for the stem only: fp32 or pre-split pixels");
+  static_assert(!(TAPWISE && FMT::PRESPLIT), "pre-split pixels have 4 channels: no K-tile lies inside one tap");
   struct P { const T* x; ConvGeom g; int rows; int K; long plane; };
   const T* bp; long plane;
   unsigned off[NVR];
diff --git a/incremental_multimodal_medical_learning_ii_amd/csrc/gemm_misc.hip b/incremental_multimodal_medical_learning_ii_amd/csrc/gemm_misc.hip
--- a/incremental_multimodal_medical_learning_ii_amd/csrc/gemm_misc.hip
+++ b/incremental_multimodal_medical_learning_ii_amd/csrc/gemm_misc.hip
@@ -164,11 +164,19 @@
   return splitk > 1 ? (size_t)splitk * (size_t)M * (size_t)N * sizeof(float) : 0;
 }
 
+int cxrk::colsum_parts(long rows) {
+  int nparts = (int)((rows + 511) / 512);
+  if (nparts > 512) nparts = 512;
+  if (nparts < 1) nparts = 1;
+  return nparts;
+}
 extern "C" size_t cxrk_colsum_ws_bytes(long rows, int cols) {
-  int nparts = (int)((rows + 511) / 512);
-  if (nparts > 512) nparts = 512;
-  if (nparts < 1) nparts = 1;
-  return (size_t)nparts * (size_t)cols * sizeof(float);
+  return (size_t)colsum_parts(rows) * (size_t)cols * sizeof(float);
+}
+int cxrk::colsum_finish(const float* part, int nparts, int cols, float* out, float alpha, int accumulate, hipStream_t stream) {
+  hipLaunchKernelGGL(colsum_final_kernel, dim3(ceil_div(cols, 256)), dim3(256), 0, stream, part, nparts, cols, out, alpha, accumulate);
+  CXRK_LAUNCH_CHECK();
+  return CXRK_OK;
 }
 
 extern "C" int cxrk_split_planes(const float* x, long n, void* out, long plane, hipStream_t stream) {
diff --git a/incremental_multimodal_medical_learning_ii_amd/image_encoder.py b/incremental_multimodal_medical_learning_ii_amd/image_encoder.py
--- a/incremental_multimodal_medical_learning_ii_amd/image_encoder.py
+++ b/incremental_multimodal_medical_learning_ii_amd/image_encoder.py
@@ -114,6 +114,18 @@
     return (H + 2 * s.pad - s.k) // s.stride + 1, (W + 2 * s.pad - s.k) // s.stride + 1
 
 
+def _is_presplit(x) -> bool:
+    return isinstance(x, torch.Tensor) and x.dtype == torch.bfloat16
+
+
+def _stem_image(specs, x: torch.Tensor, pl: bool):
+    N, _, H, W = x.shape
+    s = specs[0]
+    if pl and os.environ.get("CXRK_STEM_PRESPLIT", "1") != "0" and K.stem_presplit_applies(N, H, W, s.cout, s.k, s.k, s.stride, s.pad):
+        return K.nchw_to_nhwc4_split(x)
+    return K.nchw_to_nhwc(x, 4)
+
+
 def _conv(i, s, fold, x, residual, relu, N, H, W, pl, want_mask=True):
     Ho, Wo = _out_hw(s, H, W)
     dev = fold.vec.device
@@ -122,6 +134,9 @@
         K.conv_fwd(x, fold.ws(i, s), fold.shift(i, s), residual, y, N, H, W, s.cpad, s.cout, s.k, s.k, s.stride, s.pad, relu)
         return y, None
     y = Planes.empty(N, Ho, Wo, s.cout, device=dev)
+    if _is_presplit(x):
+        K.conv_stem_fwd_pl(x, True, fold.ws(i, s), fold.shift(i, s), y, N, H, W, s.cout, s.k, s.k, s.stride, s.pad, relu)
+        return y, None
     mask = torch.empty(N * Ho * Wo, s.cout // 8, dtype=torch.uint8, device=dev) if (relu and want_mask) else None
     K.conv_fwd_pl(x, fold.ws(i, s), fold.shift(i, s), residual, y, mask, N, H, W, s.cpad, s.cout, s.k, s.k, s.stride, s.pad, relu)
     return y, mask
@@ -171,7 +186,7 @@
             return _conv_bn_train(i, s, fold, p, bufs, x, residual, relu, N, H, W, pl, want_mask, bn_momentum)
         return _conv(i, s, fold, x, residual, relu, N, H, W, pl, want_mask)
 
-    x0 = K.nchw_to_nhwc(x, 4)
+    x0 = _stem_image(specs, x, pl and stages is None)
     stem, _ = unit(0, specs[0], fold, x0, None, True, N, H, W, pl, want_mask=False)
     Hs, Ws = stem.shape[1], stem.shape[2]
     pooled, idx = K.maxpool_fwd_pl(stem) if pl else K.maxpool_fwd(stem)
@@ -231,6 +246,8 @@
     args = (w, fold.scale(i, s), fold.rstd(i, s), bufs[2 * i], sumdy, dw, dg, db, acc, N, H, W)
     if pl and i > 0:
         K.conv_bwd_params_pl(x, dy, *args, s.cpad, s.cout, s.k, s.k, s.stride, s.pad)
+    elif _is_presplit(x):
+        K.conv_stem_bwd_params(x, True, dy, *args, s.cin, s.cout, s.k, s.k, s.stride, s.pad)
     else:
         K.conv_bwd_params(x, dy, *args, s.cin, s.cpad, s.cout, s.k, s.k, s.stride, s.pad)
 
@@ -366,12 +383,12 @@
             if all(r is None for r in sink.ret[3 * blk["c1"]:]):
                 report(stage)
     if pl:
-        ds = K.maxpool_bwd_pl(g, idx, pooled, Hs, Ws)
+        ds, sum_s = K.maxpool_bwd_pl_sums(g, idx, pooled, Hs, Ws)
     else:
         ds = K.maxpool_bwd(g, idx, stem, True)
+        sum_s = K.colsum(ds.view(-1, ds.shape[-1]), torch.empty(ds.shape[-1], dtype=torch.float32, device=dev))
     if _debug is not None:
         _debug["ds"], _debug["x0"] = ds, x0
-    sum_s = K.colsum(ds.view(-1, ds.shape[-1]), torch.empty(ds.shape[-1], dtype=torch.float32, device=dev))
     ds, sum_s = through_bn(0, specs[0], ds, sum_s)
     params_bwd(0, specs[0], x0, ds, sum_s, N, H, W, False)
     if on_grads_ready is not None and all(r is None for r in sink.ret):
diff --git a/incremental_multimodal_medical_learning_ii_amd/kernels.py b/incremental_multimodal_medical_learning_ii_amd/kernels.py
--- a/incremental_multimodal_medical_learning_ii_amd/kernels.py
+++ b/incremental_multimodal_medical_learning_ii_amd/kernels.py
@@ -701,6 +701,17 @@
     return dx
 
 
+def maxpool_bwd_pl_sums(dy: Planes, idx, pooled: Planes, H: int, W: int):
+    lib = _lib.load()
+    N, Ho, Wo, C = pooled.shape
+    dx = torch.empty(N, H, W, C, dtype=torch.float32, device=dy.device)
+    sums = torch.empty(C, dtype=torch.float32, device=dy.device)
+    ws = workspace(lib.cxrk_colsum_ws_bytes(N * Ho * Wo, C), dy.device)
+    check(lib.cxrk_maxpool_bwd_pl_sums(dy.ptr(), dy.plane, _p(idx), pooled.ptr(), _p(dx), _p(sums), 0, N, H, W, C, _p(ws), ws.numel() * 4,
+                                       _stream()), "cxrk_maxpool_bwd_pl_sums")
+    return dx, sums
+
+
 def spatial_mean_bwd_pl(dy: torch.Tensor, Pn: int, add: Optional[torch.Tensor] = None) -> Planes:
     lib = _lib.load()
     N, C = dy.shape
@@ -726,6 +737,61 @@
     y = torch.empty(N, H, W, cpad, dtype=torch.float32, device=x.device)
     check(lib.cxrk_nchw_to_nhwc(_p(x), _p(y), N, C, H, W, cpad, _stream()), "cxrk_nchw_to_nhwc")
     return y
+
+
+def nchw_to_nhwc4_split(x: torch.Tensor) -> torch.Tensor:
+    lib = _lib.load()
+    _chk(x, "nchw_to_nhwc4_split.x")
+    x = x.contiguous()
+    N, C, H, W = x.shape
+    if C != 3:
+        raise ValueError(f"nchw_to_nhwc4_split: expected 3 channels, got {C}")
+    y = torch.empty(N, H, W, 2, 4, dtype=torch.bfloat16, device=x.device)
+    check(lib.cxrk_nchw_to_nhwc4_split(_p(x), _p(y), N, H, W, _stream()), "cxrk_nchw_to_nhwc4_split")
+    return y
+
+
+def stem_presplit_applies(N, H, W, Ko, R, S, stride, pad) -> bool:
+    Ho, Wo = _conv_out(H, W, R, S, stride, pad)
+    return Ko <= 64 and _lib.get_precision() == "split_bf16" and 2.0 * N * Ho * Wo * Ko * R * S * 4 >= 1073741824.0
+
+
+def _stem_image(x, presplit: bool, N, H, W, name: str):
+    want = (torch.bfloat16, (N, H, W, 2, 4)) if presplit else (torch.float32, (N, H, W, 4))
+    if x.dtype != want[0] or tuple(x.shape) != want[1] or not x.is_contiguous() or not x.is_cuda:
+        raise ValueError(f"{name}: expected a contiguous {want[0]} GPU tensor {want[1]}, got {x.dtype} {tuple(x.shape)}")
+    return x.data_ptr()
+
+
+def conv_stem_fwd_pl(x, presplit: bool, w_scaled, shift, y: Planes, N, H, W, Ko, R, S, stride, pad, relu):
+    lib = _lib.load()
+    ev = None
+    if profiler.on:
+        Ho, Wo = _conv_out(H, W, R, S, stride, pad)
+        ev = profiler.bracket("gemm_x3_kernel<ConvIm2colKC,DenseKC,4,1>", 2.0 * N * Ho * Wo * Ko * R * S * 4,
+                              4.0 * (N * H * W * 4 + Ko * R * S * 4 + N * Ho * Wo * Ko))
+    rc = lib.cxrk_conv_bn_act_fwd_pl_stem(_stem_image(x, presplit, N, H, W, "conv_stem_fwd_pl.x"), int(presplit), _p(_chk(w_scaled, "conv.w")),
+                                          _p(shift), y.ptr(), y.plane, N, H, W, Ko, R, S, stride, pad, int(relu), _stream())
+    if ev is not None:
+        ev.record()
+    check(rc, f"cxrk_conv_bn_act_fwd_pl_stem(N={N},H={H},W={W},Ko={Ko},R={R},s={stride})")
+    return y
+
+
+def conv_stem_bwd_params(x, presplit: bool, dy, w, scale, rstd, rmean, sumdy, dw, dgamma, dbeta, accumulate, N, H, W, C, Ko, R, S, stride, pad):
+    lib = _lib.load()
+    ws = workspace(lib.cxrk_conv_wgrad_ws_bytes(N, H, W, 4, Ko, R, S, stride, pad), dy.device)
+    ev = None
+    if profiler.on:
+        Ho, Wo = _conv_out(H, W, R, S, stride, pad)
+        ev = profiler.bracket("gemm_x3_kernel<DenseMC,ConvIm2colMC,1,4>", 2.0 * N * Ho * Wo * Ko * R * S * 4,
+                              4.0 * (N * H * W * 4 + N * Ho * Wo * Ko + Ko * R * S * 4))
+    check(lib.cxrk_conv_bn_act_bwd_params_stem(_stem_image(x, presplit, N, H, W, "conv_stem_bwd_params.x"), int(presplit),
+                                               _p(_chk(dy, "conv.dy")), _p(w), _p(scale), _p(rstd), _p(rmean), _p(sumdy), _p(dw), _p(dgamma),
+                                               _p(dbeta), int(accumulate), N, H, W, C, Ko, R, S, stride, pad, _p(ws), ws.numel() * 4, _stream()),
+          f"cxrk_conv_bn_act_bwd_params_stem(N={N},H={H},W={W},C={C},Ko={Ko},R={R},s={stride})")
+    if ev is not None:
+        ev.record()
 
 
 def nhwc_to_nchw(x: torch.Tensor) -> torch.Tensor:
```
